# thobotics/geometry_rl

Hardware: NVIDIA B200
Metric: fwd+bwd+TRPL update samples/sec (policy fwd+bwd, TRPL projection, losses, critic, Adam) (higher is better)
Workload: dtype bf16

## Files before the change

### geometry_rl_b200/_lib.py

```python
import ctypes as C
import os

import torch

_HERE = os.path.dirname(os.path.abspath(__file__))
LIB_PATH = os.path.join(_HERE, "libgrl_b200.so")

GRL_OK = 0
BASIS_GRAD_FLOATS = 64 * 16 + 64 + 64 * 64 + 64
NODE_GRAD_FLOATS = 256 * 64 + 256 + 64 * 256 + 64 + 64 + 64 + 64 + 16 * 16 * 64
EDGE_GRAD_FLOATS = 64 * 64
FUSED_EDGE_GRAD_FLOATS = 64 * 64 + 64 * 16 + 64 * 64 + 64

_fp = C.c_void_p
_i32 = C.c_int32


class GrlEmbedDesc(C.Structure):
    _fields_ = [("n_nodes", _i32), ("n_scalars", _i32), ("n_vectors", _i32), ("dim", _i32),
                ("scalars", _fp), ("vectors", _fp), ("ori", _fp), ("weight", _fp), ("x", _fp),
                ("grad_x", _fp), ("grad_weight_partials", _fp), ("n_partials", _i32), ("node_ids", _fp)]


class GrlBasisDesc(C.Structure):
    _fields_ = [("n_edges", _i32), ("dim", _i32), ("edge_src", _fp), ("edge_dst", _fp), ("pos_src", _fp),
                ("pos_dst", _fp), ("ori", _fp), ("w1t", _fp), ("b1", _fp), ("w2t", _fp), ("b2", _fp), ("basis", _fp),
                ("w2", _fp), ("grad_basis", _fp), ("grad_partials", _fp), ("n_partials", _i32),
                ("basis_bf16", _fp), ("grad_basis_bf16", _fp)]


class GrlConvDesc(C.Structure):
    _fields_ = [("n_src", _i32), ("n_dst", _i32), ("n_edges", _i32),
                ("rowptr_dst", _fp), ("edge_src", _fp), ("edge_dst", _fp), ("rowptr_src", _fp), ("src_eid", _fp),
                ("x_src", _fp), ("x_dst", _fp), ("basis", _fp), ("fiber_kernel", _fp), ("wk_t", _fp), ("wk", _fp),
                ("bias", _fp), ("ln_g", _fp), ("ln_b", _fp), ("w1_t", _fp), ("w1", _fp), ("b1", _fp), ("w2_t", _fp),
                ("w2_c", _fp), ("b2", _fp), ("x1", _fp), ("out", _fp), ("accumulate_out", _i32),
                ("grad_out", _fp), ("grad_x1", _fp), ("grad_x_src", _fp), ("grad_x_src_init", _fp),
                ("grad_basis", _fp), ("accumulate_grad_basis", _i32), ("node_grad_partials", _fp),
                ("n_partials_node", _i32), ("edge_grad_partials", _fp), ("n_partials_edge", _i32), ("w2", _fp),
                ("basis_bf16", _fp), ("grad_basis_bf16", _fp), ("grad_x2", _fp), ("x2", _fp), ("grad_amax", _fp),
                ("basis_row", _fp), ("grad_basis_acc_mask", _fp)]


class GrlFusedEdgeDesc(C.Structure):
    _fields_ = [("n_key", _i32), ("n_edges", _i32), ("dim", _i32), ("n_partials", _i32),
                ("rowptr", _fp), ("e_src", _fp), ("e_dst", _fp), ("pos_src", _fp), ("pos_dst", _fp), ("ori", _fp),
                ("w1", _fp), ("b1", _fp), ("w2", _fp), ("b2", _fp), ("wk", _fp), ("x_src", _fp), ("x1", _fp),
                ("grad_x1", _fp), ("grad_x_src", _fp), ("grad_x_src_init", _fp), ("grad_partials", _fp), ("n_other", _i32)]


class GrlEncoderDesc(C.Structure):
    _fields_ = [("n_graphs", _i32), ("n_tokens", _i32), ("n_partials", _i32), ("x", _fp), ("in_proj_weight", _fp),
                ("in_proj_bias", _fp), ("out_proj_weight", _fp), ("out_proj_bias", _fp), ("linear1_weight", _fp),
                ("linear1_bias", _fp), ("linear2_weight", _fp), ("linear2_bias", _fp), ("norm1_weight", _fp),
                ("norm1_bias", _fp), ("norm2_weight", _fp), ("norm2_bias", _fp), ("out", _fp), ("grad_out", _fp),
                ("grad_x", _fp), ("grad_partials", _fp)]


ENCODER_MAX_TOKENS = 56
ENCODER_GRAD_FLOATS = 192 * 64 + 192 + 3 * (64 * 64 + 64) + 4 * 64


class GrlCriticDesc(C.Structure):
    _fields_ = [("n_graphs", _i32), ("n_tokens", _i32), ("n_feat", _i32), ("n_partials", _i32), ("eps", C.c_float),
                ("count", C.c_double), ("x", _fp), ("w1", _fp), ("b1", _fp), ("gamma", _fp), ("beta", _fp), ("stats", _fp),
                ("stat_partials", _fp), ("ysum", _fp), ("grad_ysum", _fp), ("bstats", _fp), ("grad_partials", _fp)]


CRITIC_GRAD_FLOATS = 3 * 64 + 64 * 16


class GrlProjDesc(C.Structure):
    _fields_ = [("batch", _i32), ("k", _i32), ("proj_type", _i32), ("eps_mean", C.c_float), ("eps_cov", C.c_float),
                ("mean", _fp), ("v", _fp), ("old_mean", _fp), ("old_v", _fp), ("proj_mean", _fp), ("proj_v", _fp),
                ("eta", _fp), ("grad_proj_mean", _fp), ("grad_proj_v", _fp), ("grad_mean", _fp), ("grad_v", _fp),
                ("grad_mean_add", _fp), ("grad_v_add", _fp)]


class GrlLossDesc(C.Structure):
    _fields_ = [("batch", _i32), ("k", _i32), ("proj_type", _i32), ("normalize_advantage", _i32),
                ("entropy_coef", C.c_float), ("trust_region_coeff", C.c_float),
                ("mean", _fp), ("v", _fp), ("proj_mean", _fp), ("proj_v", _fp), ("action", _fp), ("prev_log_prob", _fp),
                ("advantage", _fp), ("terms", _fp), ("stats", _fp), ("scalars", _fp), ("grad_losses", _fp),
                ("grad_proj_mean", _fp), ("grad_proj_v", _fp), ("grad_mean_direct", _fp), ("grad_v_direct", _fp),
                ("sums", _fp), ("stage", _i32)]


class GrlReadoutDesc(C.Structure):
    _fields_ = [("n_nodes", _i32), ("od", _i32), ("odv", _i32), ("dim", _i32), ("latent", _fp), ("weight", _fp),
                ("bias", _fp), ("ori", _fp), ("out", _fp), ("hidden", _fp), ("grad_out", _fp), ("grad_hidden", _fp),
                ("grad_latent", _fp), ("grad_partials", _fp), ("n_partials", _i32)]


class GrlActDesc(C.Structure):
    _fields_ = [("batch", _i32), ("num_rows", _i32), ("action_dim", _i32), ("hidden_dim", _i32), ("post_fc", _i32),
                ("contextual_std", _i32), ("use_tanh_mean", _i32), ("deterministic", _i32), ("rank", _i32),
                ("pre_shift", C.c_float), ("minimal_std", C.c_float), ("hidden", _fp), ("mean", _fp),
                ("mean_weight", _fp), ("mean_bias", _fp), ("std_weight", _fp), ("std_bias", _fp), ("state", _fp),
                ("loc", _fp), ("cov", _fp), ("action", _fp), ("log_prob", _fp), ("eps", _fp)]


ACT_MAX_K = 32
READOUT_MAX_OUT = 8
MAX_KNN = 8
LOSS_TERMS = 8
LOSS_SCALARS = 16
LOSS_STATS = 8
LOSS_SUMS = 16
LOSS_SCALAR_INDEX = {"loss_objective": 0, "loss_trust_region": 1, "loss_entropy": 2, "dist_entropy": 3, "ESS": 4, "kl": 5,
                     "constraint": 6, "mean_constraint": 7, "mean_constraint_max": 8, "cov_constraint": 9,
                     "cov_constraint_max": 10, "entropy": 11, "entropy_diff": 12}


SIGNATURES = {
    "grl_abi_version": (C.c_int, []),
    "grl_last_error": (C.c_char_p, []),
    "grl_sm_count": (C.c_int, []),
    "grl_reserve_sms": (C.c_int, [C.c_int]),
    "grl_knn_edge_ptr": (C.c_int, [_fp, C.c_int, C.c_int, C.c_int, _fp, _fp]),
    "grl_knn_graph": (C.c_int, [_fp, _fp, _fp, C.c_int, C.c_int, C.c_int, _fp, C.c_int64, _fp]),
    "grl_radius_neighbors": (C.c_int, [_fp, _fp, C.c_int, C.c_int, C.c_float, C.c_int, _fp, _fp, _fp]),
    "grl_radius_edge_ptr": (C.c_int, [_fp, C.c_int, C.c_int, C.c_int64, _fp, _fp]),
    "grl_radius_graph": (C.c_int, [_fp, _fp, _fp, C.c_int, C.c_int, C.c_int, _fp, C.c_int64, C.c_int64, _fp]),
    "grl_dense_edges": (C.c_int, [C.c_int, _fp, _fp, C.c_int, C.c_int, C.c_int, _fp, C.c_int64, _fp]),
    "grl_csr_build": (C.c_int, [_fp, C.c_int64, _fp, C.c_int, C.c_int, C.c_int, _fp, _fp, _fp, _fp]),
    "grl_embed_fwd": (C.c_int, [C.POINTER(GrlEmbedDesc), _fp]),
    "grl_embed_bwd": (C.c_int, [C.POINTER(GrlEmbedDesc), _fp]),
    "grl_edge_basis_fwd": (C.c_int, [C.POINTER(GrlBasisDesc), _fp]),
    "grl_edge_basis_bwd": (C.c_int, [C.POINTER(GrlBasisDesc), _fp]),
    "grl_fbconv_edge_fwd": (C.c_int, [C.POINTER(GrlConvDesc), _fp]),
    "grl_fbconv_node_fwd": (C.c_int, [C.POINTER(GrlConvDesc), _fp]),
    "grl_fbconv_node_bwd": (C.c_int, [C.POINTER(GrlConvDesc), _fp]),
    "grl_fbconv_edge_bwd": (C.c_int, [C.POINTER(GrlConvDesc), _fp]),
    "grl_fbconv_node_fwd_tc": (C.c_int, [C.POINTER(GrlConvDesc), _fp]),
    "grl_edge_basis_fwd_tc": (C.c_int, [C.POINTER(GrlBasisDesc), _fp]),
    "grl_fbconv_edge_fwd_tc": (C.c_int, [C.POINTER(GrlConvDesc), _fp]),
    "grl_fbconv_edge_bwd_tc": (C.c_int, [C.POINTER(GrlConvDesc), _fp]),
    "grl_edge_basis_bwd_tc": (C.c_int, [C.POINTER(GrlBasisDesc), _fp]),
    "grl_fbconv_node_bwd_tc": (C.c_int, [C.POINTER(GrlConvDesc), _fp]),
    "grl_fbconv_edge_fused_fwd": (C.c_int, [C.POINTER(GrlFusedEdgeDesc), _fp]),
    "grl_fbconv_edge_fused_bwd": (C.c_int, [C.POINTER(GrlFusedEdgeDesc), _fp]),
    "grl_critic_inner_stats": (C.c_int, [C.POINTER(GrlCriticDesc), _fp]),
    "grl_critic_inner_fwd": (C.c_int, [C.POINTER(GrlCriticDesc), _fp]),
    "grl_critic_inner_bwd_stats": (C.c_int, [C.POINTER(GrlCriticDesc), _fp]),
    "grl_critic_inner_bwd": (C.c_int, [C.POINTER(GrlCriticDesc), _fp]),
    "grl_encoder_layer_fwd": (C.c_int, [C.POINTER(GrlEncoderDesc), _fp]),
    "grl_encoder_layer_bwd": (C.c_int, [C.POINTER(GrlEncoderDesc), _fp]),
    "grl_readout_fwd": (C.c_int, [C.POINTER(GrlReadoutDesc), _fp]),
    "grl_readout_bwd": (C.c_int, [C.POINTER(GrlReadoutDesc), _fp]),
    "grl_trpl_loss_fwd": (C.c_int, [C.POINTER(GrlLossDesc), _fp]),
    "grl_trpl_loss_bwd": (C.c_int, [C.POINTER(GrlLossDesc), _fp]),
    "grl_dp_combine": (C.c_int, [_fp, C.c_int, C.c_int, C.c_int, _fp, _fp]),
    "grl_absmax": (C.c_int, [_fp, C.c_int64, _fp, _fp]),
    "grl_reduce_partials": (C.c_int, [_fp, C.c_int, C.c_int64, _fp, C.c_int, _fp]),
    "grl_gae_scan": (C.c_int, [_fp, _fp, _fp, _fp, C.c_float, C.c_float, C.c_int, C.c_int, _fp, _fp, _fp]),
    "grl_gaussian_act": (C.c_int, [C.POINTER(GrlActDesc), _fp]),
    "grl_act_advance": (C.c_int, [_fp, _fp]),
    "grl_trpl_fwd": (C.c_int, [C.POINTER(GrlProjDesc), _fp]),
    "grl_trpl_bwd": (C.c_int, [C.POINTER(GrlProjDesc), _fp]),
    "grl_tc_selftest_gemm": (C.c_int, [_fp, _fp, _fp, C.c_int, C.c_int, _fp]),
    "grl_tc_selftest_gemm_ts": (C.c_int, [_fp, _fp, _fp, C.c_int, _fp]),
    "grl_tc_debug_mma": (C.c_int, [_fp, C.c_int, _fp, C.c_int, _fp, C.c_int, C.c_int] + [C.c_uint32] * 8 + [_fp]),
    "grl_tc_latency_probe": (C.c_int, [_fp, _fp]),
}

_lib = None
launch_count = 0


def load():
    global _lib
    if _lib is None:
        if not os.path.exists(LIB_PATH):
            raise RuntimeError(
                f"{LIB_PATH} not found: build it with `python -c 'import __graft_entry__ as g; g.build()'` "
                "(geometry_rl_b200 has no CPU or eager fallback)")
        lib = C.CDLL(LIB_PATH)
        for name, (res, args) in SIGNATURES.items():
            fn = getattr(lib, name)
            fn.restype = res
            fn.argtypes = args
        _lib = lib
    return _lib


def last_error() -> str:
    return load().grl_last_error().decode()


def check(rc: int, what: str):
    if rc != GRL_OK:
        raise RuntimeError(f"{what} failed with code {rc}: {last_error()}")


def stream_ptr() -> int:
    return torch.cuda.current_stream().cuda_stream


def ptr(t):
    if t is None:
        return None
    if not t.is_cuda:
        raise RuntimeError("geometry_rl_b200 kernels need CUDA tensors (no CPU path exists)")
    if not t.is_contiguous():
        raise RuntimeError("geometry_rl_b200 kernels need contiguous tensors")
    return t.data_ptr()


def ptr_any(t):
    if t is None:
        return None
    if not t.is_cuda:
        raise RuntimeError("geometry_rl_b200 kernels need CUDA tensors (no CPU path exists)")
    return t.data_ptr()


_timing = None


def event_timing(enable: bool):
    global _timing
    if enable:
        _timing = {}
        return None
    rec, _timing = _timing, None
    torch.cuda.synchronize()
    return {k: [(a.elapsed_time(b),) + tuple(shape) for a, b, shape in v] for k, v in (rec or {}).items()}


def call(name: str, *args, shape=(0, 0, 0)):
    global launch_count
    lib = load()
    if _timing is not None:
        a, b = torch.cuda.Event(enable_timing=True), torch.cuda.Event(enable_timing=True)
        a.record()
        rc = getattr(lib, name)(*args, stream_ptr())
        b.record()
        _timing.setdefault(name, []).append((a, b, shape))
    else:
        rc = getattr(lib, name)(*args, stream_ptr())
    launch_count += 1
    check(rc, name)


_sm = None


def sm_count() -> int:
    global _sm
    if _sm is None:
        _sm = load().grl_sm_count()
    return _sm


def reserve_sms(n: int) -> None:
    global _sm
    check(load().grl_reserve_sms(int(n)), "grl_reserve_sms")
    _sm = None
```

### geometry_rl_b200/csrc/grl_common.cuh

```cuda
#pragma once
#include <cuda_runtime.h>
#include <stdint.h>

#include "../../include/grl_b200.h"

namespace grl {

constexpr int kO = GRL_NUM_ORI;
constexpr int kC = GRL_CHANNELS;
constexpr int kH = GRL_HIDDEN;
constexpr int kTE = 8;
constexpr int kTM = kTE * kO;
constexpr int kLDT = 68;
constexpr int kThreads = 256;
constexpr int kRow = kO * kC;
constexpr int kTileFloats = kTM * kLDT;
constexpr int kWFloats = kC * kC;

void set_error(const char* fmt, ...);
int check_launch(const char* what);
int sm_count();
int ensure_dynamic_smem(const void* func, int bytes);
int make_row_tensor_map(void* out_tensor_map_128B, const float* base, long long n_nodes, int box_rows = 16);

#define GRL_REQUIRE(cond, code, ...)  \
  do {                                \
    if (!(cond)) {                    \
      ::grl::set_error(__VA_ARGS__);  \
      return (code);                  \
    }                                 \
  } while (0)

__device__ __forceinline__ float gelu_f(float x) { return 0.5f * x * (1.0f + erff(x * 0.70710678118654752440f)); }
__device__ __forceinline__ float gelu_grad_f(float x) {
  const float cdf = 0.5f * (1.0f + erff(x * 0.70710678118654752440f));
  const float pdf = 0.39894228040143267794f * expf(-0.5f * x * x);
  return cdf + x * pdf;
}

__device__ __forceinline__ float tanh_approx(float x) {
  float y;
  asm("tanh.approx.f32 %0, %1;" : "=f"(y) : "f"(x));
  return y;
}
__device__ __forceinline__ void gelu_fast(float x, float& y, float& dy) {
#ifdef GRL_TC_EXACT_GELU
  const float u = __expf(-0.5f * x * x);
  const float t = __fdividef(1.0f, fmaf(0.23164189f, fabsf(x), 1.0f));
  float poly = fmaf(t, 1.061405429f, -1.453152027f);
  poly = fmaf(t, poly, 1.421413741f);
  poly = fmaf(t, poly, -0.284496736f);
  poly = fmaf(t, poly, 0.254829592f);
  const float tail = 0.5f * (poly * t) * u;
  const float cdf = x >= 0.f ? 1.0f - tail : tail;
  y = x * cdf;
  dy = fmaf(x * u, 0.39894228040143267794f, cdf);
#else
  constexpr float k = 0.7978845608028654f, kc = 0.7978845608028654f * 0.044715f;
  const float t2 = x * x;
  const float th = tanh_approx(x * fmaf(t2, kc, k));
  const float hx = 0.5f * x;
  y = fmaf(hx, th, hx);
  dy = fmaf(hx * fmaf(-th, th, 1.0f), fmaf(t2, 3.0f * kc, k), fmaf(th, 0.5f, 0.5f));
#endif
}
__device__ __forceinline__ float gelu_fast(float x) {
#ifdef GRL_TC_EXACT_GELU
  float y, dy;
  gelu_fast(x, y, dy);
  return y;
#else
  constexpr float k = 0.7978845608028654f, kc = 0.7978845608028654f * 0.044715f;
  const float hx = 0.5f * x;
  return fmaf(hx, tanh_approx(x * fmaf(x * x, kc, k)), hx);
#endif
}

__device__ __forceinline__ void cp_async16(float* smem_dst, const float* gmem_src) {
  const unsigned s = static_cast<unsigned>(__cvta_generic_to_shared(smem_dst));
  asm volatile("cp.async.cg.shared.global [%0], [%1], 16;\n" ::"r"(s), "l"(gmem_src) : "memory");
}
__device__ __forceinline__ void cp_async_commit() { asm volatile("cp.async.commit_group;\n" ::: "memory"); }
__device__ __forceinline__ void cp_async_wait_all() { asm volatile("cp.async.wait_group 0;\n" ::: "memory"); }
template <int N>
__device__ __forceinline__ void cp_async_wait() {
  asm volatile("cp.async.wait_group %0;\n" ::"n"(N) : "memory");
}

__device__ __forceinline__ void stage_w64(float* __restrict__ dst, const float* __restrict__ src) {
#pragma unroll
  for (int i = 0; i < 4; ++i) {
    const int f = threadIdx.x + kThreads * i;
    cp_async16(dst + 4 * f, src + 4 * f);
  }
}

__device__ __forceinline__ void stage_rows_contig(float* __restrict__ tile, const float* __restrict__ src, int cnt) {
#pragma unroll
  for (int i = 0; i < 8; ++i) {
    const int f = threadIdx.x + kThreads * i;
    const int row = f >> 4, c4 = f & 15;
    float* d = tile + row * kLDT + 4 * c4;
    if ((row >> 4) < cnt) {
      cp_async16(d, src + (size_t)row * kC + 4 * c4);
    } else {
      *reinterpret_cast<float4*>(d) = make_float4(0.f, 0.f, 0.f, 0.f);
    }
  }
}

__device__ __forceinline__ void stage_rows_gather(float* __restrict__ tile, const float* __restrict__ base,
                                                  const int* __restrict__ idx, int cnt) {
#pragma unroll
  for (int i = 0; i < 8; ++i) {
    const int f = threadIdx.x + kThreads * i;
    const int row = f >> 4, c4 = f & 15;
    const int j = row >> 4;
    float* d = tile + row * kLDT + 4 * c4;
    if (j < cnt) {
      cp_async16(d, base + (size_t)idx[j] * kRow + (row & 15) * kC + 4 * c4);
    } else {
      *reinterpret_cast<float4*>(d) = make_float4(0.f, 0.f, 0.f, 0.f);
    }
  }
}

template <int K>
__device__ __forceinline__ void gemm_tile(const float* __restrict__ As, int lda, const float* __restrict__ Bs, int o,
                                          int cg, float (&acc)[kTE][4]) {
  const float* a0 = As + o * lda;
  const float* b0 = Bs + 4 * cg;
#pragma unroll 2
  for (int k = 0; k < K; k += 4) {
    const float4 b_0 = *reinterpret_cast<const float4*>(b0 + (k + 0) * kC);
    const float4 b_1 = *reinterpret_cast<const float4*>(b0 + (k + 1) * kC);
    const float4 b_2 = *reinterpret_cast<const float4*>(b0 + (k + 2) * kC);
    const float4 b_3 = *reinterpret_cast<const float4*>(b0 + (k + 3) * kC);
#pragma unroll
    for (int j = 0; j < kTE; ++j) {
      const float4 a = *reinterpret_cast<const float4*>(a0 + j * 16 * lda + k);
      acc[j][0] = fmaf(a.x, b_0.x, acc[j][0]);
      acc[j][1] = fmaf(a.x, b_0.y, acc[j][1]);
      acc[j][2] = fmaf(a.x, b_0.z, acc[j][2]);
      acc[j][3] = fmaf(a.x, b_0.w, acc[j][3]);
      acc[j][0] = fmaf(a.y, b_1.x, acc[j][0]);
      acc[j][1] = fmaf(a.y, b_1.y, acc[j][1]);
      acc[j][2] = fmaf(a.y, b_1.z, acc[j][2]);
      acc[j][3] = fmaf(a.y, b_1.w, acc[j][3]);
      acc[j][0] = fmaf(a.z, b_2.x, acc[j][0]);
      acc[j][1] = fmaf(a.z, b_2.y, acc[j][1]);
      acc[j][2] = fmaf(a.z, b_2.z, acc[j][2]);
      acc[j][3] = fmaf(a.z, b_2.w, acc[j][3]);
      acc[j][0] = fmaf(a.w, b_3.x, acc[j][0]);
      acc[j][1] = fmaf(a.w, b_3.y, acc[j][1]);
      acc[j][2] = fmaf(a.w, b_3.z, acc[j][2]);
      acc[j][3] = fmaf(a.w, b_3.w, acc[j][3]);
    }
  }
}

__device__ __forceinline__ void zero_acc(float (&acc)[kTE][4]) {
#pragma unroll
  for (int j = 0; j < kTE; ++j) acc[j][0] = acc[j][1] = acc[j][2] = acc[j][3] = 0.f;
}

template <bool kColSum>
__device__ __forceinline__ void wgrad_tile(const float* __restrict__ As, int lda, const float* __restrict__ Bs, int ldb,
                                           int ni, int mi, float (&g)[4][4], float (&colsum)[4]) {
  const float* a0 = As + 4 * ni;
  const float* b0 = Bs + 4 * mi;
#pragma unroll 4
  for (int r = 0; r < kTM; ++r) {
    const float4 a = *reinterpret_cast<const float4*>(a0 + r * lda);
    const float4 b = *reinterpret_cast<const float4*>(b0 + r * ldb);
    g[0][0] = fmaf(a.x, b.x, g[0][0]); g[0][1] = fmaf(a.x, b.y, g[0][1]);
    g[0][2] = fmaf(a.x, b.z, g[0][2]); g[0][3] = fmaf(a.x, b.w, g[0][3]);
    g[1][0] = fmaf(a.y, b.x, g[1][0]); g[1][1] = fmaf(a.y, b.y, g[1][1]);
    g[1][2] = fmaf(a.y, b.z, g[1][2]); g[1][3] = fmaf(a.y, b.w, g[1][3]);
    g[2][0] = fmaf(a.z, b.x, g[2][0]); g[2][1] = fmaf(a.z, b.y, g[2][1]);
    g[2][2] = fmaf(a.z, b.z, g[2][2]); g[2][3] = fmaf(a.z, b.w, g[2][3]);
    g[3][0] = fmaf(a.w, b.x, g[3][0]); g[3][1] = fmaf(a.w, b.y, g[3][1]);
    g[3][2] = fmaf(a.w, b.z, g[3][2]); g[3][3] = fmaf(a.w, b.w, g[3][3]);
    if (kColSum && mi == 0) {
      colsum[0] += a.x; colsum[1] += a.y; colsum[2] += a.z; colsum[3] += a.w;
// ... 32 lines not shown
```

### geometry_rl_b200/csrc/grl_conv_node_bwd_tc.cu

```cuda
#include "grl_common.cuh"
#include "grl_tc.cuh"

namespace grl {

constexpr int kPGW1 = 0;
constexpr int kPGB1 = kPGW1 + kH * kC;
constexpr int kPGW2 = kPGB1 + kH;
constexpr int kPGB2 = kPGW2 + kC * kH;
constexpr int kPGLNG = kPGB2 + kC;
constexpr int kPGLNB = kPGLNG + kC;
constexpr int kPGBIAS = kPGLNB + kC;
constexpr int kPGFK = kPGBIAS + kC;
static_assert(kPGFK + kO * kO * kC == GRL_NODE_GRAD_FLOATS, "partial layout");

constexpr int kKb = 80;
constexpr int kLDX2 = 68;

__device__ __forceinline__ void warp_colsum16(float (&v)[16], int lane) {
#pragma unroll
  for (int step = 0; step < 4; ++step) {
    const int half = 8 >> step;
    const int bit = 16 >> step;
    const bool upper = (lane & bit) != 0;
#pragma unroll
    for (int i = 0; i < half; ++i) {
      const float keep = upper ? v[i + half] : v[i];
      const float send = upper ? v[i] : v[i + half];
      v[i] = keep + __shfl_xor_sync(0xffffffffu, send, bit);
    }
  }
  v[0] += __shfl_xor_sync(0xffffffffu, v[0], 1);
}

constexpr int kNB3Epi = 512;
constexpr int kNB3Threads = kNB3Epi + 32;
constexpr uint32_t kCol3D0 = 0, kCol3D1 = 64, kCol3GY = 128, kCol3DW1 = 192, kCol3DW2 = 352;

struct NodeBwd3Smem {
  __half W1h[kH * kKb];
  __half W2h[kC * kH];
  __half A1[kTM * kKb];
  __half GZh[kTM * kC];
  union {
    struct {
      float X2[kTM * kLDX2];
      float GZf[kTM * kLDX2];
    } in;
    struct {
      __half A2h[kTM * 128];
      __half AP[kTM * 128];
    } h;
  } u;
  float bias[kC], lng[kC], lnb[kC];
  float rs[2][4][kTM];
  float acc_gb2[4][kC], acc_glng[4][kC], acc_glnb[4][kC];
  uint64_t full[2], edone[2], lnready, gyfull, dwdone;
  uint32_t tmem_base;
};

__global__ void __launch_bounds__(kNB3Threads, 1) fbconv_node_bwd_tc3_kernel(const GrlConvDesc d) {
  extern __shared__ __align__(128) unsigned char smem_raw[];
  NodeBwd3Smem& s = *reinterpret_cast<NodeBwd3Smem*>(smem_raw);
  const int tid = threadIdx.x, warp = tid >> 5, lane = tid & 31;
  const bool is_epi = warp < 16;
  const int q = warp & 3, cg = (warp >> 2) & 3;
  const int row = 32 * q + lane;

  if (tid == 0) {
    tc::mbar_init(&s.full[0], 1);
    tc::mbar_init(&s.full[1], 1);
    tc::mbar_init(&s.edone[0], 16);
    tc::mbar_init(&s.edone[1], 16);
    tc::mbar_init(&s.lnready, 16);
    tc::mbar_init(&s.gyfull, 1);
    tc::mbar_init(&s.dwdone, 1);
    tc::fence_mbar_init();
  }
  if (warp == 16) tc::tmem_alloc(&s.tmem_base, 512);
  tc::stage_weight_f16(s.W1h, d.w1, kH, kC, kC);
  tc::stage_weight_f16(s.W2h, d.w2, kC, kH, kH);
  for (int n = tid; n < kH; n += kNB3Threads) {
    const float b = d.b1[n];
    const __half hi = __float2half_rn(b);
    const __half lo = __float2half_rn(b - __half2float(hi));
    const __half2 p0 = __halves2half2(hi, lo);
    *reinterpret_cast<uint4*>(s.W1h + ((size_t)8 * kH + n) * 8) = make_uint4(*reinterpret_cast<const uint32_t*>(&p0), 0u, 0u, 0u);
    *reinterpret_cast<uint4*>(s.W1h + ((size_t)9 * kH + n) * 8) = make_uint4(0u, 0u, 0u, 0u);
  }
  if (tid < kTM) {
    *reinterpret_cast<uint4*>(s.A1 + ((size_t)8 * kTM + tid) * 8) = make_uint4(0x3C003C00u, 0u, 0u, 0u);
    *reinterpret_cast<uint4*>(s.A1 + ((size_t)9 * kTM + tid) * 8) = make_uint4(0u, 0u, 0u, 0u);
  }
  if (tid < kC) { s.bias[tid] = d.bias[tid]; s.lng[tid] = d.ln_g[tid]; s.lnb[tid] = d.ln_b[tid]; }
  for (int i = tid; i < 4 * kC; i += kNB3Threads) {
    (&s.acc_gb2[0][0])[i] = 0.f; (&s.acc_glng[0][0])[i] = 0.f; (&s.acc_glnb[0][0])[i] = 0.f;
  }
  const float gscale = d.grad_amax ? tc::grad_scale_from_amax(__ldg(d.grad_amax)) : 1.0f;
  const float inv_gscale = 1.0f / gscale;
  const int n_tiles = (d.n_dst + kTE - 1) / kTE;
  int tile = blockIdx.x;
  auto stage_x2 = [&](int t) {
    const int cnt = min(kTE, d.n_dst - t * kTE);
    const float* src = d.x2 + (size_t)t * kTE * kRow;
    const float* gsrc = d.grad_out + (size_t)t * kTE * kRow;
#pragma unroll
    for (int i = 0; i < 4; ++i) {
      const int f = tid + kNB3Epi * i;
      const int so = (f >> 4) * kLDX2 + 4 * (f & 15);
      if ((f >> 8) < cnt) {
        cp_async16(s.u.in.X2 + so, src + 4 * f);
        cp_async16(s.u.in.GZf + so, gsrc + 4 * f);
      } else {
        *reinterpret_cast<float4*>(s.u.in.X2 + so) = make_float4(0.f, 0.f, 0.f, 0.f);
        *reinterpret_cast<float4*>(s.u.in.GZf + so) = make_float4(0.f, 0.f, 0.f, 0.f);
      }
    }
  };
  if (is_epi && tile < n_tiles) {
    stage_x2(tile);
    cp_async_commit();
  }
  tc::fence_async_smem();
  tc::tc_fence_before();
  __syncthreads();
  tc::tc_fence_after();
  const uint32_t tmem = s.tmem_base;
  const uint32_t lane_addr = tmem + ((uint32_t)(32 * q) << 16);
  const uint32_t a1 = tc::smem_u32(s.A1), gz = tc::smem_u32(s.GZh), a2 = tc::smem_u32(s.u.h.A2h), ap = tc::smem_u32(s.u.h.AP);
  const uint32_t w1 = tc::smem_u32(s.W1h), w2 = tc::smem_u32(s.W2h);
  bool first_tile = true;

  if (!is_epi) {
    uint32_t p_ln = 0, p_e0 = 0, p_e1 = 0;
    constexpr uint32_t id_pre = tc::idesc_f16_ex(128, 64, 0, 0, 0, 0);
    constexpr uint32_t id_gh = tc::idesc_f16_ex(128, 64, 0, 1, 0, 0);
    constexpr uint32_t id_dw2 = tc::idesc_f16_ex(128, 64, 1, 1, 0, 0);
    constexpr uint32_t id_dw1 = tc::idesc_f16_ex(128, kKb, 1, 1, 0, 0);
    const tc::Op a1_k = tc::op_k(a1, kTM), a1_mn = tc::op_mn(a1, kTM);
    const tc::Op gz_k = tc::op_k(gz, kTM), gz_mn = tc::op_mn(gz, kTM);
    const tc::Op a2_mn = tc::op_mn(a2, kTM), ap_k = tc::op_k(ap, kTM), ap_mn = tc::op_mn(ap, kTM);
    const tc::Op w1_k = tc::op_k(w1, kH), w1_mn = tc::op_mn(w1, kH), w2_mn = tc::op_mn(w2, kC);
    auto shifted = [](tc::Op o, uint32_t bytes) { o.lo += bytes >> 4; return o; };
    auto pre = [&](int qq, uint32_t col) { tc::issue_mma_fast<kKb / 16>(tmem + col, a1_k, shifted(w1_k, 64u * qq * 16u), id_pre, false); };
    auto gh = [&](int qq, uint32_t col) { tc::issue_mma_fast<kC / 16>(tmem + col, gz_k, shifted(w2_mn, 8u * qq * (kC * 16u)), id_gh, false); };
    for (; tile < n_tiles; tile += gridDim.x) {
      tc::mbar_wait(&s.lnready, p_ln);
      p_ln ^= 1u;
      tc::tc_fence_after();
      if (tc::elect_one()) {
        pre(0, kCol3D0);
        tc::mma_commit(&s.full[0]);
        pre(1, kCol3D1);
        tc::mma_commit(&s.full[1]);
      }
      __syncwarp();
#pragma unroll
      for (int hh = 0; hh < 2; ++hh) {
        tc::mbar_wait(&s.edone[0], p_e0);
        p_e0 ^= 1u;
        tc::tc_fence_after();
        if (tc::elect_one()) {
          gh(2 * hh, kCol3D0);
          tc::mma_commit(&s.full[0]);
        }
        __syncwarp();
        tc::mbar_wait(&s.edone[1], p_e1);
        p_e1 ^= 1u;
        tc::tc_fence_after();
        if (tc::elect_one()) {
          gh(2 * hh + 1, kCol3D1);
          tc::mma_commit(&s.full[1]);
          tc::issue_mma_fast<kTM / 16>(tmem + kCol3DW2 + 64 * hh, a2_mn, gz_mn, id_dw2, !first_tile);
        }
        __syncwarp();
        tc::mbar_wait(&s.edone[0], p_e0);
        p_e0 ^= 1u;
        tc::tc_fence_after();
        if (hh == 0) {
          if (tc::elect_one()) {
            pre(2, kCol3D0);
            tc::mma_commit(&s.full[0]);
          }
          __syncwarp();
        }
        tc::mbar_wait(&s.edone[1], p_e1);
        p_e1 ^= 1u;
        tc::tc_fence_after();
        if (tc::elect_one()) {
          if (hh == 0) {
            pre(3, kCol3D1);
            tc::mma_commit(&s.full[1]);
          }
          tc::issue_mma_fast<128 / 16>(tmem + kCol3GY, ap_k, shifted(w1_mn, 128u * hh * 16u), id_gh, hh > 0);
          if (hh == 1) tc::mma_commit(&s.gyfull);
          tc::issue_mma_fast<kTM / 16>(tmem + kCol3DW1 + kKb * hh, ap_mn, a1_mn, id_dw1, !first_tile);
          if (hh == 1) tc::mma_commit(&s.dwdone);
        }
        __syncwarp();
      }
      first_tile = false;
    }
  } else {
    uint32_t pf0 = 0, pf1 = 0, pgy = 0;
    for (; tile < n_tiles; tile += gridDim.x) {
      const int n0 = tile * kTE;
      const int node = n0 + (row >> 4);
      const bool live = node < d.n_dst;
      const size_t roff = (size_t)(live ? node : 0) * kRow + (row & 15) * kC + 16 * cg;
      if (tid == 0) {
        const int nt = tile + gridDim.x;
        if (nt < n_tiles) {
          const uint32_t bytes = (uint32_t)min(kTE, d.n_dst - nt * kTE) * kRow * 4u;
          tc::prefetch_l2(d.x2 + (size_t)nt * kTE * kRow, bytes);
          tc::prefetch_l2(d.grad_out + (size_t)nt * kTE * kRow, bytes);
        }
      }
      cp_async_wait_all();
      tc::group_sync(5, kNB3Epi);

      float xh[16];
      float rstd;
      {
        float sum = 0.f;
#pragma unroll
        for (int i = 0; i < 4; ++i) {
          const float4 v = ld4(s.u.in.X2 + row * kLDX2 + 16 * cg + 4 * i);
          xh[4 * i] = v.x; xh[4 * i + 1] = v.y; xh[4 * i + 2] = v.z; xh[4 * i + 3] = v.w;
          sum += (v.x + v.y) + (v.z + v.w);
        }
        float g16[16];
#pragma unroll
        for (int i = 0; i < 4; ++i) {
          const float4 gv = ld4(s.u.in.GZf + row * kLDX2 + 16 * cg + 4 * i);
          g16[4 * i] = gv.x; g16[4 * i + 1] = gv.y; g16[4 * i + 2] = gv.z; g16[4 * i + 3] = gv.w;
        }
        s.rs[0][cg][row] = sum;
        tc::group_sync(1 + q, 128);
        const float mean = ((s.rs[0][0][row] + s.rs[0][1][row]) + (s.rs[0][2][row] + s.rs[0][3][row])) * (1.0f / 64.0f);
        float sq = 0.f;
#pragma unroll
        for (int i = 0; i < 16; ++i) { xh[i] -= mean; sq = fmaf(xh[i], xh[i], sq); }
        s.rs[1][cg][row] = sq;
        {
          float gs[16];
#pragma unroll
          for (int i = 0; i < 16; ++i) gs[i] = g16[i] * gscale;
          *reinterpret_cast<uint4*>(s.GZh + ((size_t)(2 * cg) * kTM + row) * 8) = tc::pack8_h(gs);
          *reinterpret_cast<uint4*>(s.GZh + ((size_t)(2 * cg + 1) * kTM + row) * 8) = tc::pack8_h(gs + 8);
        }
        warp_colsum16(g16, lane);
        if ((lane & 1) == 0) s.acc_gb2[q][16 * cg + (lane >> 1)] += g16[0];
        tc::group_sync(1 + q, 128);
        rstd = rsqrtf(((s.rs[1][0][row] + s.rs[1][1][row]) + (s.rs[1][2][row] + s.rs[1][3][row])) * (1.0f / 64.0f) + 1e-5f);
#pragma unroll
        for (int i = 0; i < 2; ++i) {
          float y[8];
#pragma unroll
          for (int e = 0; e < 8; ++e) {
            const int c = 16 * cg + 8 * i + e;
            xh[8 * i + e] *= rstd;
            y[e] = xh[8 * i + e] * s.lng[c] + s.lnb[c];
          }
          *reinterpret_cast<uint4*>(s.A1 + ((size_t)(2 * cg + i) * kTM + row) * 8) = tc::pack8_h(y);
        }
      }
      tc::fence_async_smem();
      tc::tc_fence_before();
      __syncwarp();
      if (lane == 0) tc::mbar_arrive(&s.lnready);

      __half2 dG0[8], dG1[8];
      auto e1 = [&](uint32_t col, uint64_t* fullb, uint32_t& pf, uint64_t* doneb, __half2 (&dG)[8], int chunk) {
        tc::mbar_wait(fullb, pf);
        pf ^= 1u;
        tc::tc_fence_after();
        float v[16];
        tc::tmem_ld16(lane_addr + col + 16 * cg, v);
        __half2 h0[4], h1[4];
#pragma unroll
        for (int e = 0; e < 4; ++e) {
          tc::gelu_h2(__floats2half2_rn(v[2 * e], v[2 * e + 1]), h0[e], dG[e]);
          tc::gelu_h2(__floats2half2_rn(v[8 + 2 * e], v[8 + 2 * e + 1]), h1[e], dG[4 + e]);
        }
        *reinterpret_cast<uint4*>(s.u.h.A2h + ((size_t)chunk * kTM + row) * 8) = tc::pack_h8(h0);
        *reinterpret_cast<uint4*>(s.u.h.A2h + ((size_t)(chunk + 1) * kTM + row) * 8) = tc::pack_h8(h1);
        tc::fence_async_smem();
        tc::tc_fence_before();
        __syncwarp();
        if (lane == 0) tc::mbar_arrive(doneb);
      };
      auto e2 = [&](uint32_t col, uint64_t* fullb, uint32_t& pf, uint64_t* doneb, const __half2 (&dG)[8], int chunk) {
        tc::mbar_wait(fullb, pf);
        pf ^= 1u;
        tc::tc_fence_after();
        float v[16];
        tc::tmem_ld16(lane_addr + col + 16 * cg, v);
        __half2 p0[4], p1[4];
#pragma unroll
        for (int e = 0; e < 4; ++e) {
          p0[e] = __hmul2(__floats2half2_rn(v[2 * e], v[2 * e + 1]), dG[e]);
          p1[e] = __hmul2(__floats2half2_rn(v[8 + 2 * e], v[8 + 2 * e + 1]), dG[4 + e]);
        }
        *reinterpret_cast<uint4*>(s.u.h.AP + ((size_t)chunk * kTM + row) * 8) = tc::pack_h8(p0);
        *reinterpret_cast<uint4*>(s.u.h.AP + ((size_t)(chunk + 1) * kTM + row) * 8) = tc::pack_h8(p1);
        tc::fence_async_smem();
        tc::tc_fence_before();
        __syncwarp();
        if (lane == 0) tc::mbar_arrive(doneb);
      };
#pragma unroll 1
      for (int hh = 0; hh < 2; ++hh) {
        e1(kCol3D0, &s.full[0], pf0, &s.edone[0], dG0, 2 * cg);
        e1(kCol3D1, &s.full[1], pf1, &s.edone[1], dG1, 8 + 2 * cg);
        e2(kCol3D0, &s.full[0], pf0, &s.edone[0], dG0, 2 * cg);
        e2(kCol3D1, &s.full[1], pf1, &s.edone[1], dG1, 8 + 2 * cg);
      }
      tc::mbar_wait(&s.gyfull, pgy);
      tc::tc_fence_after();

      {
        float gy[32];
        {
          float v[16];
          tc::tmem_ld16(lane_addr + kCol3GY + 16 * cg, v);
#pragma unroll
          for (int e = 0; e < 16; ++e) gy[e] = v[e] * inv_gscale;
        }
        tc::mbar_wait(&s.dwdone, pgy);
        pgy ^= 1u;
        {
          const int nt = tile + gridDim.x;
          if (nt < n_tiles) {
            stage_x2(nt);
            cp_async_commit();
          }
        }
        float s1 = 0.f, s2 = 0.f;
#pragma unroll
        for (int i = 0; i < 16; ++i) {
          const float hx = gy[i] * s.lng[16 * cg + i];
          s1 += hx;
          s2 = fmaf(hx, xh[i], s2);
        }
        s.rs[0][cg][row] = s1;
        s.rs[1][cg][row] = s2;
        tc::group_sync(1 + q, 128);
        const float m1 = ((s.rs[0][0][row] + s.rs[0][1][row]) + (s.rs[0][2][row] + s.rs[0][3][row])) * (1.0f / 64.0f);
        const float m2 = ((s.rs[1][0][row] + s.rs[1][1][row]) + (s.rs[1][2][row] + s.rs[1][3][row])) * (1.0f / 64.0f);
        float* gdst = d.grad_x2 + roff;
#pragma unroll
        for (int i = 0; i < 4; ++i) {
          float o[4];
#pragma unroll
          for (int e = 0; e < 4; ++e) {
            const int c = 4 * i + e;
            const float hx = gy[c] * s.lng[16 * cg + c];
            o[e] = rstd * (hx - m1 - xh[c] * m2);
          }
          if (live) st4(gdst + 4 * i, make_float4(o[0], o[1], o[2], o[3]));
        }
#pragma unroll
        for (int i = 0; i < 16; ++i) gy[16 + i] = gy[i] * xh[i];
        tc::warp_colsum<32>(gy, lane);
        if (lane < 16) s.acc_glnb[q][16 * cg + lane] += gy[0];
        else s.acc_glng[q][16 * cg + lane - 16] += gy[0];
      }
      tc::tc_fence_before();
      first_tile = false;
    }
    cp_async_wait_all();
  }

  __syncthreads();
  tc::tc_fence_after();
  float* P = d.node_grad_partials + (size_t)blockIdx.x * GRL_NODE_GRAD_FLOATS;
  if (is_epi) {
#pragma unroll 1
    for (int h2 = 0; h2 < 2; ++h2) {
      const int c0 = 16 * cg;
      float v[16];
#pragma unroll
      for (int e = 0; e < 16; ++e) v[e] = 0.f;
      if (!first_tile) tc::tmem_ld16(lane_addr + kCol3DW1 + kKb * h2 + c0, v);
      float* p1 = P + kPGW1 + (size_t)(128 * h2 + row) * kC + c0;
#pragma unroll
      for (int e = 0; e < 16; e += 4)
        st4(p1 + e, make_float4(v[e] * inv_gscale, v[e + 1] * inv_gscale, v[e + 2] * inv_gscale, v[e + 3] * inv_gscale));
      if (cg == 0) {
        float b[16];
#pragma unroll
        for (int e = 0; e < 16; ++e) b[e] = 0.f;
        if (!first_tile) tc::tmem_ld16(lane_addr + kCol3DW1 + kKb * h2 + 64, b);
        P[kPGB1 + 128 * h2 + row] = b[0] * inv_gscale;
      }
      if (!first_tile) tc::tmem_ld16(lane_addr + kCol3DW2 + 64 * h2 + c0, v);
#pragma unroll
      for (int e = 0; e < 16; ++e) P[kPGW2 + (size_t)(c0 + e) * kH + 128 * h2 + row] = v[e] * inv_gscale;
    }
  }
  if (tid < kC) {
    P[kPGB2 + tid] = ((s.acc_gb2[0][tid] + s.acc_gb2[1][tid]) + s.acc_gb2[2][tid]) + s.acc_gb2[3][tid];
    P[kPGLNG + tid] = ((s.acc_glng[0][tid] + s.acc_glng[1][tid]) + s.acc_glng[2][tid]) + s.acc_glng[3][tid];
    P[kPGLNB + tid] = ((s.acc_glnb[0][tid] + s.acc_glnb[1][tid]) + s.acc_glnb[2][tid]) + s.acc_glnb[3][tid];
  }
  tc::tc_fence_before();
  __syncthreads();
  if (warp == 16) tc::tmem_dealloc(tmem, 512);
}

constexpr int kFiberThreads = 512;
constexpr int kFibTile = 4;
struct FiberBwdSmem {
  float G[2][kFibTile * kRow];
  float X[2][kFibTile * kRow];
};

__device__ __forceinline__ void fiber_stage(FiberBwdSmem& s, int buf, const GrlConvDesc& d, int tile) {
  const int n0 = tile * kFibTile;
#pragma unroll
  for (int i = 0; i < 4; ++i) {
    const int f = threadIdx.x + kFiberThreads * i;
    const int arr = f >> 10, idx = f & 1023, node = n0 + (idx >> 8);
    float* dst = (arr ? s.X[buf] : s.G[buf]) + 4 * idx;
    if (node < d.n_dst) cp_async16(dst, (arr ? d.x1 : d.grad_x2) + (size_t)n0 * kRow + 4 * idx);
    else *reinterpret_cast<float4*>(dst) = make_float4(0.f, 0.f, 0.f, 0.f);
  }
}

__global__ void __launch_bounds__(kFiberThreads, 1) fbconv_fiber_bwd_kernel(const GrlConvDesc d) {
  extern __shared__ __align__(128) unsigned char smem_raw[];
  FiberBwdSmem& s = *reinterpret_cast<FiberBwdSmem*>(smem_raw);
  const int tid = threadIdx.x, c = tid & 63, op = tid >> 6;
  unsigned long long fk2[kO], gfk2[kO];
#pragma unroll
  for (int p = 0; p < kO; ++p) {
    fk2[p] = pack2(__ldg(d.fiber_kernel + ((size_t)((2 * op) * kO + p)) * kC + c) * 0.0625f,
                   __ldg(d.fiber_kernel + ((size_t)((2 * op + 1) * kO + p)) * kC + c) * 0.0625f);
    gfk2[p] = pack2(0.f, 0.f);
  }
  float gbias = 0.f;
  const int n_tiles = (d.n_dst + kFibTile - 1) / kFibTile;
  int tile = blockIdx.x, buf = 0;
  if (tile < n_tiles) fiber_stage(s, 0, d, tile);
  cp_async_commit();
  for (; tile < n_tiles; tile += gridDim.x, buf ^= 1) {
    const int nt = tile + gridDim.x;
    if (nt < n_tiles) fiber_stage(s, buf ^ 1, d, nt);
    cp_async_commit();
    cp_async_wait<1>();
    __syncthreads();
#pragma unroll
    for (int j = 0; j < kFibTile; ++j) {
      const int node = tile * kFibTile + j;
      const float* G = s.G[buf] + j * kRow + c;
      const float* X = s.X[buf] + j * kRow + c;
      const unsigned long long xv = pack2(X[(2 * op) * kC], X[(2 * op + 1) * kC]);
      unsigned long long a2 = pack2(0.f, 0.f);
      float gsum = 0.f;
#pragma unroll
      for (int p = 0; p < kO; ++p) {
        const float g = G[p * kC];
        const unsigned long long gg = pack2(g, g);
        a2 = ffma2(gg, fk2[p], a2);
        gfk2[p] = ffma2(xv, gg, gfk2[p]);
        gsum += g;
      }
      if (node < d.n_dst) {
        float a0, a1;
        unpack2(a2, a0, a1);
        d.grad_x1[(size_t)node * kRow + (2 * op) * kC + c] = a0;
        d.grad_x1[(size_t)node * kRow + (2 * op + 1) * kC + c] = a1;
      }
      if (op == 0) gbias += gsum;
    }
    __syncthreads();
  }
  float* P = d.node_grad_partials + (size_t)blockIdx.x * GRL_NODE_GRAD_FLOATS;
#pragma unroll
  for (int p = 0; p < kO; ++p) {
    float g0, g1;
    unpack2(gfk2[p], g0, g1);
    P[kPGFK + ((size_t)((2 * op) * kO + p)) * kC + c] = g0 * 0.0625f;
    P[kPGFK + ((size_t)((2 * op + 1) * kO + p)) * kC + c] = g1 * 0.0625f;
  }
  if (op == 0) P[kPGBIAS + c] = gbias;
}

}

extern "C" int grl_fbconv_node_bwd_tc(const GrlConvDesc* d, grl_stream_t stream) {
  GRL_REQUIRE(d && d->n_dst > 0, GRL_EINVAL, "grl_fbconv_node_bwd_tc: bad descriptor");
  GRL_REQUIRE(d->x1 && d->fiber_kernel && d->bias && d->ln_g && d->ln_b && d->w1 && d->b1 && d->w2 && d->grad_out &&
                  d->grad_x1 && d->grad_x2 && d->node_grad_partials && d->n_partials_node > 0, GRL_EINVAL,
              "grl_fbconv_node_bwd_tc: null pointer");
  {
    GRL_REQUIRE(d->x2, GRL_EINVAL, "grl_fbconv_node_bwd_tc: x2 (saved by grl_fbconv_node_fwd_tc) is required");
    const int smem = (int)sizeof(grl::NodeBwd3Smem);
    if (grl::ensure_dynamic_smem((const void*)grl::fbconv_node_bwd_tc3_kernel, smem) != GRL_OK) return GRL_ECUDA;
    grl::fbconv_node_bwd_tc3_kernel<<<d->n_partials_node, grl::kNB3Threads, smem, (cudaStream_t)stream>>>(*d);
  }
  int rc = grl::check_launch("grl_fbconv_node_bwd_tc (mlp)");
  if (rc != GRL_OK) return rc;
  const int smem2 = (int)sizeof(grl::FiberBwdSmem);
  if (grl::ensure_dynamic_smem((const void*)grl::fbconv_fiber_bwd_kernel, smem2) != GRL_OK) return GRL_ECUDA;
  grl::fbconv_fiber_bwd_kernel<<<d->n_partials_node, grl::kFiberThreads, smem2, (cudaStream_t)stream>>>(*d);
  return grl::check_launch("grl_fbconv_node_bwd_tc (fibre)");
}
```

### geometry_rl_b200/csrc/grl_conv_node_tc.cu

```cuda
#include <cuda.h>

#include "grl_common.cuh"
#include "grl_tc.cuh"

namespace grl {

constexpr int kLDX = 72;

constexpr int kNF2Threads = 512;
constexpr int kK1 = 80;

struct NodeFwd2Group {
  union {
    struct {
      float X1[kTM * kC];
      float X2[kTM * kLDX];
    } x;
    __half A1[kTM * kK1];
  } u;
};

struct NodeFwd2Smem {
  __half W1h[kH * kK1];
  __half W2h[kC * kH];
  NodeFwd2Group g[2];
  float b2[kC], bias[kC], lng[kC], lnb[kC];
  uint64_t bar[2][2];
  uint64_t bar_x[2];
  uint64_t bar_d[2];
  uint32_t tmem_base;
};

__device__ __forceinline__ void stage_x1_dense(float* __restrict__ X1, const float* __restrict__ src, int cnt, int gt,
                                               uint64_t* bar) {
  if (gt == 0) {
    tc::mbar_expect_tx(bar, (uint32_t)cnt * kRow * 4u);
    tc::bulk_g2s(X1, src, (uint32_t)cnt * kRow * 4u, bar);
  }
  if (cnt < kTE) {
#pragma unroll
    for (int i = 0; i < 8; ++i) {
      const int f = gt + 256 * i;
      if ((f >> 8) >= cnt) *reinterpret_cast<float4*>(X1 + 4 * f) = make_float4(0.f, 0.f, 0.f, 0.f);
    }
  }
}

template <bool kAcc>
__global__ void __launch_bounds__(kNF2Threads, 1) fbconv_node_fwd_tc2_kernel(const GrlConvDesc d, const __grid_constant__ CUtensorMap tm_xd) {
  extern __shared__ unsigned char smem_raw[];
  NodeFwd2Smem& s = *reinterpret_cast<NodeFwd2Smem*>(
      smem_raw + ((1024u - (tc::smem_u32(smem_raw) & 1023u)) & 1023u));
  const int tid = threadIdx.x;
  const int grp = tid >> 8, gt = tid & 255, gw = gt >> 5, lane = tid & 31;
  NodeFwd2Group& G = s.g[grp];
  const int bar_id = 1 + grp;

  if (tid == 0) {
    tc::mbar_init(&s.bar[0][0], 1);
    tc::mbar_init(&s.bar[0][1], 1);
    tc::mbar_init(&s.bar[1][0], 1);
    tc::mbar_init(&s.bar[1][1], 1);
    tc::mbar_init(&s.bar_x[0], 1);
    tc::mbar_init(&s.bar_x[1], 1);
    tc::mbar_init(&s.bar_d[0], 1);
    tc::mbar_init(&s.bar_d[1], 1);
    tc::fence_mbar_init();
  }
  if (tid < 32) tc::tmem_alloc(&s.tmem_base, 512);
  tc::stage_weight_f16(s.W1h, d.w1, kH, kC, kC);
  tc::stage_weight_f16(s.W2h, d.w2, kC, kH, kH);
  for (int n = tid; n < kH; n += kNF2Threads) {
    const float b = d.b1[n];
    const __half hi = __float2half_rn(b);
    const __half lo = __float2half_rn(b - __half2float(hi));
    const __half z = __float2half_rn(0.f);
    const __half2 h[4] = {__halves2half2(hi, lo), __halves2half2(z, z), __halves2half2(z, z), __halves2half2(z, z)};
    *reinterpret_cast<uint4*>(s.W1h + ((size_t)8 * kH + n) * 8) = tc::pack_h8(h);
    *reinterpret_cast<uint4*>(s.W1h + ((size_t)9 * kH + n) * 8) = make_uint4(0u, 0u, 0u, 0u);
  }
  if (tid < kC) { s.b2[tid] = d.b2[tid]; s.bias[tid] = d.bias[tid]; s.lng[tid] = d.ln_g[tid]; s.lnb[tid] = d.ln_b[tid]; }
  const int fc = gt & 63, pq = gt >> 6;
  unsigned long long fk2[kO][2];
#pragma unroll
  for (int o = 0; o < kO; ++o)
#pragma unroll
    for (int pi = 0; pi < 2; ++pi)
      fk2[o][pi] = pack2(__ldg(d.fiber_kernel + ((size_t)(o * kO + 4 * pq + 2 * pi)) * kC + fc) * 0.0625f,
                         __ldg(d.fiber_kernel + ((size_t)(o * kO + 4 * pq + 2 * pi + 1)) * kC + fc) * 0.0625f);

  const int n_tiles = (d.n_dst + kTE - 1) / kTE;
  const int tile_stride = 2 * gridDim.x;
  int tile = 2 * blockIdx.x + grp;
  tc::fence_async_smem();
  tc::tc_fence_before();
  __syncthreads();
  tc::tc_fence_after();
  if (tile < n_tiles)
    stage_x1_dense(G.u.x.X1, d.x1 + (size_t)tile * kTE * kRow, min(kTE, d.n_dst - tile * kTE), gt, &s.bar_x[grp]);
  const uint32_t tmem = s.tmem_base + 256u * grp;
  const uint32_t a1_addr = tc::smem_u32(G.u.A1);
  const uint32_t w1_addr = tc::smem_u32(s.W1h), w2_addr = tc::smem_u32(s.W2h);
  const int q = gw & 3, hh = gw >> 2;
  const int row = 32 * q + lane;
  const uint32_t lane_addr = tmem + ((uint32_t)(32 * q) << 16);
  uint32_t parity = 0;

  for (; tile < n_tiles; tile += tile_stride) {
    const int n0 = tile * kTE;
    if (gt == 0) {
      tc::prefetch_l2(d.x_dst + (size_t)n0 * kRow, (uint32_t)min(kTE, d.n_dst - n0) * kRow * 4u);
      const int nt = tile + tile_stride;
      if (nt < n_tiles) tc::prefetch_l2(d.x1 + (size_t)nt * kTE * kRow, (uint32_t)min(kTE, d.n_dst - nt * kTE) * kRow * 4u);
    }
    tc::mbar_wait(&s.bar_x[grp], parity);
    tc::group_sync(bar_id, 256);

    {
      const float bias_c = s.bias[fc];
#pragma unroll 2
      for (int j = 0; j < kTE; ++j) {
        unsigned long long a01 = pack2(0.f, 0.f), a23 = a01;
#pragma unroll
        for (int o = 0; o < kO; ++o) {
          const float x = G.u.x.X1[(16 * j + o) * kC + fc];
          const unsigned long long xx = pack2(x, x);
          a01 = ffma2(xx, fk2[o][0], a01);
          a23 = ffma2(xx, fk2[o][1], a23);
        }
        float a0, a1, a2, a3;
        unpack2(a01, a0, a1);
        unpack2(a23, a2, a3);
        float* o2 = G.u.x.X2 + (16 * j + 4 * pq) * kLDX + fc;
        o2[0 * kLDX] = a0 + bias_c;
        o2[1 * kLDX] = a1 + bias_c;
        o2[2 * kLDX] = a2 + bias_c;
        o2[3 * kLDX] = a3 + bias_c;
      }
    }
    tc::group_sync(bar_id, 256);

    {
      const int r = gt >> 1, h = gt & 1;
      float4 v[8];
      float sum = 0.f;
#pragma unroll
      for (int i = 0; i < 8; ++i) {
        v[i] = ld4(G.u.x.X2 + r * kLDX + 4 * (2 * i + h));
        sum += (v[i].x + v[i].y) + (v[i].z + v[i].w);
      }
      if (d.x2 && n0 + (r >> 4) < d.n_dst) {
        float* xo = d.x2 + (size_t)(n0 + (r >> 4)) * kRow + (r & 15) * kC + 4 * h;
#pragma unroll
        for (int i = 0; i < 8; ++i) st4(xo + 8 * i, v[i]);
      }
      sum += __shfl_xor_sync(0xffffffffu, sum, 1);
      const float mean = sum * (1.0f / 64.0f);
      float sq = 0.f;
#pragma unroll
      for (int i = 0; i < 8; ++i) {
        v[i].x -= mean; v[i].y -= mean; v[i].z -= mean; v[i].w -= mean;
        sq += (v[i].x * v[i].x + v[i].y * v[i].y) + (v[i].z * v[i].z + v[i].w * v[i].w);
      }
      sq += __shfl_xor_sync(0xffffffffu, sq, 1);
      const float rstd = rsqrtf(sq * (1.0f / 64.0f) + 1e-5f);
#pragma unroll
      for (int i = 0; i < 8; ++i) {
        const int c = 4 * (2 * i + h);
        const float4 g = ld4(s.lng + c), b = ld4(s.lnb + c);
        const __half2 p0 = __floats2half2_rn(v[i].x * rstd * g.x + b.x, v[i].y * rstd * g.y + b.y);
        const __half2 p1 = __floats2half2_rn(v[i].z * rstd * g.z + b.z, v[i].w * rstd * g.w + b.w);
        uint2 pk;
        pk.x = *reinterpret_cast<const uint32_t*>(&p0);
        pk.y = *reinterpret_cast<const uint32_t*>(&p1);
        *reinterpret_cast<uint2*>(G.u.A1 + ((size_t)i * kTM + r) * 8 + 4 * h) = pk;
      }
      *reinterpret_cast<uint4*>(G.u.A1 + ((size_t)(8 + h) * kTM + r) * 8) = make_uint4(h == 0 ? 0x3C003C00u : 0u, 0u, 0u, 0u);
    }
    tc::fence_async_smem();
    tc::tc_fence_before();
    tc::group_sync(bar_id, 256);
    if (gt == 0) {
      tc::tc_fence_after();
      tc::issue_mma_rolled(tmem, tc::view_k(a1_addr, kTM), tc::view_k(w1_addr, kH), tc::idesc_f16_ex(128, kH, 0, 0, 0, 0), kK1 / 16, false);
      tc::mma_commit(&s.bar[grp][0]);
      tc::mbar_expect_tx(&s.bar_d[grp], 2u * kTM * 32u * 4u);
      tc::tma_load_2d(G.u.x.X2, &tm_xd, 0, n0 * kO, &s.bar_d[grp]);
      tc::tma_load_2d(G.u.x.X2 + kTM * 32, &tm_xd, 32, n0 * kO, &s.bar_d[grp]);
    }
    tc::mbar_wait(&s.bar[grp][0], parity);
    tc::tc_fence_after();
    {
      const int nt = tile + tile_stride;
      if (nt < n_tiles) {
        tc::fence_async_smem();
        stage_x1_dense(G.u.x.X1, d.x1 + (size_t)nt * kTE * kRow, min(kTE, d.n_dst - nt * kTE), gt, &s.bar_x[grp]);
      }
    }
    {
#pragma unroll 2
      for (int i = 0; i < 8; ++i) {
        const int c0 = 128 * hh + 16 * i;
        float v[16];
        tc::tmem_ld16(lane_addr + c0, v);
        uint32_t r[8];
#pragma unroll
        for (int e = 0; e < 4; ++e) {
          const __half2 a = tc::gelu_h2(__floats2half2_rn(v[2 * e], v[2 * e + 1]));
          const __half2 b = tc::gelu_h2(__floats2half2_rn(v[8 + 2 * e], v[8 + 2 * e + 1]));
          r[e] = *reinterpret_cast<const uint32_t*>(&a);
          r[4 + e] = *reinterpret_cast<const uint32_t*>(&b);
        }
        tc::tmem_st8(lane_addr + 128 * hh + 8 * i, r);
      }
      tc::tmem_st_wait();
    }
    tc::tc_fence_before();
    tc::group_sync(bar_id, 256);
    if (gt == 0) {
      tc::tc_fence_after();
      const tc::OpView w2v = tc::view_k(w2_addr, kC);
      tc::OpView w2hi = w2v;
      w2hi.addr += 8 * w2v.adv;
      tc::issue_mma_ts(tmem + 64, tmem, w2v, tc::idesc_f16_ex(128, kC, 0, 0, 0, 0), 8, false);
      tc::issue_mma_ts(tmem + 64, tmem + 128, w2hi, tc::idesc_f16_ex(128, kC, 0, 0, 0, 0), 8, true);
      tc::mma_commit(&s.bar[grp][1]);
    }
    const int node = n0 + (row >> 4);
    const bool live = node < d.n_dst;
    const size_t off = (size_t)(live ? node : 0) * kRow + (row & 15) * kC + 32 * hh;
    tc::mbar_wait(&s.bar[grp][1], parity);
    tc::tc_fence_after();
    tc::mbar_wait(&s.bar_d[grp], parity);
    const float* xrow = G.u.x.X2 + hh * (kTM * 32) + row * 32;
#pragma unroll
    for (int i = 0; i < 2; ++i) {
      float v[16];
      tc::tmem_ld16(lane_addr + 64 + 32 * hh + 16 * i, v);
      if (live) {
#pragma unroll
        for (int e = 0; e < 4; ++e) {
          const float4 bb = ld4(s.b2 + 32 * hh + 16 * i + 4 * e);
          float4 x = ld4(xrow + (((4 * i + e) ^ (row & 7)) << 2));
          if (kAcc) {
            const float4 old = ldg4(d.out + off + 16 * i + 4 * e);
            x.x += old.x; x.y += old.y; x.z += old.z; x.w += old.w;
          }
          st4(d.out + off + 16 * i + 4 * e, make_float4(x.x + (v[4 * e] + bb.x), x.y + (v[4 * e + 1] + bb.y),
                                                       x.z + (v[4 * e + 2] + bb.z), x.w + (v[4 * e + 3] + bb.w)));
        }
      }
    }
    tc::tc_fence_before();
    parity ^= 1u;
  }
  cp_async_wait_all();
  tc::tc_fence_before();
  __syncthreads();
  if (tid < 32) tc::tmem_dealloc(s.tmem_base, 512);
}

}

extern "C" int grl_fbconv_node_fwd_tc(const GrlConvDesc* d, grl_stream_t stream) {
  GRL_REQUIRE(d && d->n_dst > 0, GRL_EINVAL, "grl_fbconv_node_fwd_tc: bad descriptor");
  GRL_REQUIRE(d->x1 && d->fiber_kernel && d->bias && d->ln_g && d->ln_b && d->w1 && d->b1 && d->w2 && d->b2 && d->x_dst &&
                  d->out, GRL_EINVAL, "grl_fbconv_node_fwd_tc: null pointer");
  const int n_tiles = (d->n_dst + grl::kTE - 1) / grl::kTE;
  const int smem2 = (int)sizeof(grl::NodeFwd2Smem) + 1024;
  if (grl::ensure_dynamic_smem((const void*)grl::fbconv_node_fwd_tc2_kernel<false>, smem2) != GRL_OK) return GRL_ECUDA;
  if (grl::ensure_dynamic_smem((const void*)grl::fbconv_node_fwd_tc2_kernel<true>, smem2) != GRL_OK) return GRL_ECUDA;
  alignas(64) CUtensorMap tm_xd;
  if (grl::make_row_tensor_map(&tm_xd, d->x_dst, d->n_dst, grl::kTM) != GRL_OK) return GRL_ECUDA;
  int grid = grl::sm_count();
  if (2 * grid > n_tiles) grid = (n_tiles + 1) / 2;
  if (d->accumulate_out) grl::fbconv_node_fwd_tc2_kernel<true><<<grid, grl::kNF2Threads, smem2, (cudaStream_t)stream>>>(*d, tm_xd);
  else grl::fbconv_node_fwd_tc2_kernel<false><<<grid, grl::kNF2Threads, smem2, (cudaStream_t)stream>>>(*d, tm_xd);
  return grl::check_launch("grl_fbconv_node_fwd_tc");
}
```

### geometry_rl_b200/csrc/grl_critic.cu

```cuda
#include "grl_common.cuh"

namespace grl {

constexpr int kCrThreads = 256;
constexpr int kCrMaxTokens = 256;

struct CriticSmem {
  float x[kCrMaxTokens * 16];
  float w1[16 * kC];
  float red[16 * kC];
  double dred[kCrThreads / 32 * 4];
};

__device__ __forceinline__ void critic_stage_w1(float* __restrict__ w1s, const GrlCriticDesc& d) {
  for (int i = threadIdx.x; i < 16 * kC; i += kCrThreads) {
    const int f = i >> 6, c = i & 63;
    w1s[i] = f < d.n_feat ? __ldg(d.w1 + c * d.n_feat + f) : 0.f;
  }
}

__device__ __forceinline__ void critic_stage_x(float* __restrict__ xs, const GrlCriticDesc& d, int b, int t0, int cnt) {
  const float* src = d.x + ((size_t)b * d.n_tokens + t0) * d.n_feat;
  for (int i = threadIdx.x; i < cnt * 16; i += kCrThreads) {
    const int t = i >> 4, f = i & 15;
    xs[i] = f < d.n_feat ? __ldg(src + t * d.n_feat + f) : 0.f;
  }
}

__device__ __forceinline__ float4 critic_h(const float* __restrict__ xrow, const float* __restrict__ w1s, int cg, float4 b1) {
  float4 h = b1;
#pragma unroll
  for (int f = 0; f < 16; ++f) {
    const float xv = xrow[f];
    const float4 w = *reinterpret_cast<const float4*>(w1s + f * kC + 4 * cg);
    h.x = fmaf(xv, w.x, h.x); h.y = fmaf(xv, w.y, h.y); h.z = fmaf(xv, w.z, h.z); h.w = fmaf(xv, w.w, h.w);
  }
  return h;
}

template <int NV>
__device__ __forceinline__ void block_sum_d(double (&v)[NV], double* __restrict__ scratch) {
#pragma unroll
  for (int i = 0; i < NV; ++i) {
#pragma unroll
    for (int o = 16; o > 0; o >>= 1) v[i] += __shfl_xor_sync(0xffffffffu, v[i], o);
  }
  const int warp = threadIdx.x >> 5, lane = threadIdx.x & 31;
  __syncthreads();
  if (lane == 0) {
#pragma unroll
    for (int i = 0; i < NV; ++i) scratch[warp * 4 + i] = v[i];
  }
  __syncthreads();
  if (threadIdx.x == 0) {
#pragma unroll
    for (int i = 0; i < NV; ++i) {
      double s = 0.0;
      for (int w = 0; w < kCrThreads / 32; ++w) s += scratch[w * 4 + i];
      v[i] = s;
    }
  }
}

__device__ __forceinline__ void critic_range(const GrlCriticDesc& d, int& g_lo, int& g_hi) {
  g_lo = (int)((long long)d.n_graphs * blockIdx.x / gridDim.x);
  g_hi = (int)((long long)d.n_graphs * (blockIdx.x + 1) / gridDim.x);
}

__global__ void __launch_bounds__(kCrThreads) critic_stats_kernel(const GrlCriticDesc d) {
  extern __shared__ __align__(16) unsigned char smem_raw[];
  CriticSmem& s = *reinterpret_cast<CriticSmem*>(smem_raw);
  const int p = threadIdx.x >> 4, cg = threadIdx.x & 15;
  critic_stage_w1(s.w1, d);
  const float4 b1 = __ldg(reinterpret_cast<const float4*>(d.b1) + cg);
  int g_lo, g_hi;
  critic_range(d, g_lo, g_hi);
  double acc[2] = {0.0, 0.0};
  for (int b = g_lo; b < g_hi; ++b) {
    for (int t0 = 0; t0 < d.n_tokens; t0 += kCrMaxTokens) {
      const int cnt = min(kCrMaxTokens, d.n_tokens - t0);
      __syncthreads();
      critic_stage_x(s.x, d, b, t0, cnt);
      __syncthreads();
      float sm = 0.f, sq = 0.f;
      for (int t = p; t < cnt; t += 16) {
        const float4 h = critic_h(s.x + t * 16, s.w1, cg, b1);
        sm += (h.x + h.y) + (h.z + h.w);
        sq += (h.x * h.x + h.y * h.y) + (h.z * h.z + h.w * h.w);
      }
      acc[0] += (double)sm;
      acc[1] += (double)sq;
    }
  }
  block_sum_d<2>(acc, s.dred);
  if (threadIdx.x == 0) {
    d.stat_partials[2 * blockIdx.x] = acc[0];
    d.stat_partials[2 * blockIdx.x + 1] = acc[1];
  }
}

__global__ void critic_combine_kernel(const double* __restrict__ partials, int n_slots, int n, double* __restrict__ out) {
  const int i = threadIdx.x;
  if (i >= n) return;
  double s = 0.0;
  for (int k = 0; k < n_slots; ++k) s += partials[(size_t)k * n + i];
  out[i] = s;
}

struct CriticNorm {
  float mean, inv, r;
};
__device__ __forceinline__ CriticNorm critic_norm(const GrlCriticDesc& d) {
  const double n = d.count;
  const double mean = d.stats[0] / n;
  double var = d.stats[1] / n - mean * mean;
  var = var > 0.0 ? var : 0.0;
  const double sd = sqrt(var);
  CriticNorm c;
  c.mean = (float)mean;
  c.inv = (float)(1.0 / (sd + (double)d.eps));
  c.r = (float)(sd / (sd + (double)d.eps));
  return c;
}

__global__ void __launch_bounds__(kCrThreads) critic_fwd_kernel(const GrlCriticDesc d) {
  extern __shared__ __align__(16) unsigned char smem_raw[];
  CriticSmem& s = *reinterpret_cast<CriticSmem*>(smem_raw);
  const int p = threadIdx.x >> 4, cg = threadIdx.x & 15;
  critic_stage_w1(s.w1, d);
  const float4 b1 = __ldg(reinterpret_cast<const float4*>(d.b1) + cg);
  const float4 ga = __ldg(reinterpret_cast<const float4*>(d.gamma) + cg);
  const float4 be = __ldg(reinterpret_cast<const float4*>(d.beta) + cg);
  const CriticNorm nm = critic_norm(d);
  int g_lo, g_hi;
  critic_range(d, g_lo, g_hi);
  for (int b = g_lo; b < g_hi; ++b) {
    float4 ys = make_float4(0.f, 0.f, 0.f, 0.f);
    for (int t0 = 0; t0 < d.n_tokens; t0 += kCrMaxTokens) {
      const int cnt = min(kCrMaxTokens, d.n_tokens - t0);
      __syncthreads();
      critic_stage_x(s.x, d, b, t0, cnt);
      __syncthreads();
      for (int t = p; t < cnt; t += 16) {
        const float4 h = critic_h(s.x + t * 16, s.w1, cg, b1);
        ys.x += fmaxf(fmaf((h.x - nm.mean) * nm.inv, ga.x, be.x), 0.f);
        ys.y += fmaxf(fmaf((h.y - nm.mean) * nm.inv, ga.y, be.y), 0.f);
        ys.z += fmaxf(fmaf((h.z - nm.mean) * nm.inv, ga.z, be.z), 0.f);
        ys.w += fmaxf(fmaf((h.w - nm.mean) * nm.inv, ga.w, be.w), 0.f);
      }
    }
    __syncthreads();
    *reinterpret_cast<float4*>(s.red + p * kC + 4 * cg) = ys;
    __syncthreads();
    if (threadIdx.x < kC) {
      float a = 0.f;
#pragma unroll
      for (int k = 0; k < 16; ++k) a += s.red[k * kC + threadIdx.x];
      d.ysum[(size_t)b * kC + threadIdx.x] = a;
    }
  }
}

__global__ void __launch_bounds__(kCrThreads) critic_bwd_stats_kernel(const GrlCriticDesc d) {
  extern __shared__ __align__(16) unsigned char smem_raw[];
  CriticSmem& s = *reinterpret_cast<CriticSmem*>(smem_raw);
  const int p = threadIdx.x >> 4, cg = threadIdx.x & 15;
  critic_stage_w1(s.w1, d);
  const float4 b1 = __ldg(reinterpret_cast<const float4*>(d.b1) + cg);
  const float4 ga = __ldg(reinterpret_cast<const float4*>(d.gamma) + cg);
  const float4 be = __ldg(reinterpret_cast<const float4*>(d.beta) + cg);
  const CriticNorm nm = critic_norm(d);
  int g_lo, g_hi;
  critic_range(d, g_lo, g_hi);
  double acc[2] = {0.0, 0.0};
  float4 gg = make_float4(0.f, 0.f, 0.f, 0.f), gb = make_float4(0.f, 0.f, 0.f, 0.f);
  for (int b = g_lo; b < g_hi; ++b) {
    const float4 gy = __ldg(reinterpret_cast<const float4*>(d.grad_ysum + (size_t)b * kC) + cg);
    for (int t0 = 0; t0 < d.n_tokens; t0 += kCrMaxTokens) {
      const int cnt = min(kCrMaxTokens, d.n_tokens - t0);
      __syncthreads();
      critic_stage_x(s.x, d, b, t0, cnt);
      __syncthreads();
      float s1 = 0.f, s2 = 0.f;
      for (int t = p; t < cnt; t += 16) {
        const float4 h = critic_h(s.x + t * 16, s.w1, cg, b1);
        const float xh[4] = {(h.x - nm.mean) * nm.inv, (h.y - nm.mean) * nm.inv, (h.z - nm.mean) * nm.inv, (h.w - nm.mean) * nm.inv};
        const float g[4] = {gy.x, gy.y, gy.z, gy.w}, gam[4] = {ga.x, ga.y, ga.z, ga.w}, bet[4] = {be.x, be.y, be.z, be.w};
        float* ggp = &gg.x;
        float* gbp = &gb.x;
#pragma unroll
        for (int k = 0; k < 4; ++k) {
          const float go = fmaf(xh[k], gam[k], bet[k]) > 0.f ? g[k] : 0.f;
          ggp[k] += go * xh[k];
          gbp[k] += go;
          const float gx = go * gam[k];
          s1 += gx;
          s2 += gx * xh[k];
        }
      }
      acc[0] += (double)s1;
      acc[1] += (double)s2;
    }
  }
  block_sum_d<2>(acc, s.dred);
  if (threadIdx.x == 0) {
    d.stat_partials[2 * blockIdx.x] = acc[0];
    d.stat_partials[2 * blockIdx.x + 1] = acc[1];
  }
  float* P = d.grad_partials + (size_t)blockIdx.x * GRL_CRITIC_GRAD_FLOATS;
  __syncthreads();
  *reinterpret_cast<float4*>(s.red + p * kC + 4 * cg) = gg;
  __syncthreads();
  if (threadIdx.x < kC) {
    float a = 0.f;
#pragma unroll
    for (int k = 0; k < 16; ++k) a += s.red[k * kC + threadIdx.x];
    P[threadIdx.x] = a;
  }
  __syncthreads();
  *reinterpret_cast<float4*>(s.red + p * kC + 4 * cg) = gb;
  __syncthreads();
  if (threadIdx.x < kC) {
    float a = 0.f;
#pragma unroll
    for (int k = 0; k < 16; ++k) a += s.red[k * kC + threadIdx.x];
    P[kC + threadIdx.x] = a;
  }
}

__global__ void __launch_bounds__(kCrThreads) critic_bwd_kernel(const GrlCriticDesc d) {
  extern __shared__ __align__(16) unsigned char smem_raw[];
  CriticSmem& s = *reinterpret_cast<CriticSmem*>(smem_raw);
  const int p = threadIdx.x >> 4, cg = threadIdx.x & 15;
  critic_stage_w1(s.w1, d);
  const float4 b1 = __ldg(reinterpret_cast<const float4*>(d.b1) + cg);
  const float4 ga = __ldg(reinterpret_cast<const float4*>(d.gamma) + cg);
  const float4 be = __ldg(reinterpret_cast<const float4*>(d.beta) + cg);
  const CriticNorm nm = critic_norm(d);
  const float c1 = (float)(d.bstats[0] / d.count);
  const float c2 = (float)(d.bstats[1] / (d.count * (double)nm.r));
  int g_lo, g_hi;
  critic_range(d, g_lo, g_hi);
  float gw[4][16];
  float gb1[4] = {0.f, 0.f, 0.f, 0.f};
#pragma unroll
  for (int k = 0; k < 4; ++k)
#pragma unroll
    for (int f = 0; f < 16; ++f) gw[k][f] = 0.f;
  for (int b = g_lo; b < g_hi; ++b) {
    const float4 gy = __ldg(reinterpret_cast<const float4*>(d.grad_ysum + (size_t)b * kC) + cg);
    for (int t0 = 0; t0 < d.n_tokens; t0 += kCrMaxTokens) {
      const int cnt = min(kCrMaxTokens, d.n_tokens - t0);
      __syncthreads();
      critic_stage_x(s.x, d, b, t0, cnt);
      __syncthreads();
      for (int t = p; t < cnt; t += 16) {
        const float* xr = s.x + t * 16;
        const float4 h = critic_h(xr, s.w1, cg, b1);
        const float hv[4] = {h.x, h.y, h.z, h.w}, g[4] = {gy.x, gy.y, gy.z, gy.w};
        const float gam[4] = {ga.x, ga.y, ga.z, ga.w}, bet[4] = {be.x, be.y, be.z, be.w};
        float gh[4];
#pragma unroll
        for (int k = 0; k < 4; ++k) {
          const float xh = (hv[k] - nm.mean) * nm.inv;
          const float gx = fmaf(xh, gam[k], bet[k]) > 0.f ? g[k] * gam[k] : 0.f;
          gh[k] = nm.inv * (gx - c1 - xh * c2);
          gb1[k] += gh[k];
        }
#pragma unroll
        for (int f = 0; f < 16; ++f) {
          const float xv = xr[f];
#pragma unroll
          for (int k = 0; k < 4; ++k) gw[k][f] = fmaf(gh[k], xv, gw[k][f]);
        }
      }
    }
  }
  float* P = d.grad_partials + (size_t)blockIdx.x * GRL_CRITIC_GRAD_FLOATS;
  auto combine = [&](float v0, float v1, float v2, float v3, float* dst, int stride) {
    __syncthreads();
    *reinterpret_cast<float4*>(s.red + p * kC + 4 * cg) = make_float4(v0, v1, v2, v3);
    __syncthreads();
    if (threadIdx.x < kC) {
      float a = 0.f;
#pragma unroll
      for (int k = 0; k < 16; ++k) a += s.red[k * kC + threadIdx.x];
      dst[(size_t)threadIdx.x * stride] = a;
    }
  };
  combine(gb1[0], gb1[1], gb1[2], gb1[3], P + 2 * kC, 1);
#pragma unroll
  for (int f = 0; f < 16; ++f) combine(gw[0][f], gw[1][f], gw[2][f], gw[3][f], P + 3 * kC + f, 16);
}

}

extern "C" {

static int critic_check(const GrlCriticDesc* d, const char* who) {
  GRL_REQUIRE(d, GRL_EINVAL, "%s: null descriptor", who);
  GRL_REQUIRE(d->n_graphs > 0 && d->n_tokens > 0 && d->n_feat > 0 && d->n_feat <= 16, GRL_EINVAL,
              "%s: n_graphs=%d n_tokens=%d n_feat=%d (n_feat <= 16)", who, d->n_graphs, d->n_tokens, d->n_feat);
  GRL_REQUIRE(d->x && d->w1 && d->b1 && d->gamma && d->beta && d->stats && d->stat_partials, GRL_EINVAL, "%s: null pointer", who);
  GRL_REQUIRE(d->n_partials > 0 && d->n_partials <= d->n_graphs, GRL_EINVAL, "%s: n_partials=%d must be in [1, n_graphs]", who,
              d->n_partials);
  return GRL_OK;
}

static int critic_grid(const GrlCriticDesc* d) { return d->n_partials; }

int grl_critic_inner_stats(const GrlCriticDesc* d, grl_stream_t stream) {
  const int rc = critic_check(d, "grl_critic_inner_stats");
  if (rc != GRL_OK) return rc;
  const int smem = (int)sizeof(grl::CriticSmem);
  if (grl::ensure_dynamic_smem((const void*)grl::critic_stats_kernel, smem) != GRL_OK) return GRL_ECUDA;
  const int grid = critic_grid(d);
  grl::critic_stats_kernel<<<grid, grl::kCrThreads, smem, (cudaStream_t)stream>>>(*d);
  grl::critic_combine_kernel<<<1, 32, 0, (cudaStream_t)stream>>>(d->stat_partials, grid, 2, d->stats);
  return grl::check_launch("grl_critic_inner_stats");
}

int grl_critic_inner_fwd(const GrlCriticDesc* d, grl_stream_t stream) {
  const int rc = critic_check(d, "grl_critic_inner_fwd");
  if (rc != GRL_OK) return rc;
  GRL_REQUIRE(d->ysum && d->count > 0, GRL_EINVAL, "grl_critic_inner_fwd: ysum / count");
  const int smem = (int)sizeof(grl::CriticSmem);
  if (grl::ensure_dynamic_smem((const void*)grl::critic_fwd_kernel, smem) != GRL_OK) return GRL_ECUDA;
  grl::critic_fwd_kernel<<<critic_grid(d), grl::kCrThreads, smem, (cudaStream_t)stream>>>(*d);
  return grl::check_launch("grl_critic_inner_fwd");
}

int grl_critic_inner_bwd_stats(const GrlCriticDesc* d, grl_stream_t stream) {
  const int rc = critic_check(d, "grl_critic_inner_bwd_stats");
  if (rc != GRL_OK) return rc;
  GRL_REQUIRE(d->grad_ysum && d->bstats && d->grad_partials && d->count > 0, GRL_EINVAL, "grl_critic_inner_bwd_stats: null pointer");
  const int smem = (int)sizeof(grl::CriticSmem);
  if (grl::ensure_dynamic_smem((const void*)grl::critic_bwd_stats_kernel, smem) != GRL_OK) return GRL_ECUDA;
  const int grid = critic_grid(d);
  grl::critic_bwd_stats_kernel<<<grid, grl::kCrThreads, smem, (cudaStream_t)stream>>>(*d);
  grl::critic_combine_kernel<<<1, 32, 0, (cudaStream_t)stream>>>(d->stat_partials, grid, 2, d->bstats);
  return grl::check_launch("grl_critic_inner_bwd_stats");
}

int grl_critic_inner_bwd(const GrlCriticDesc* d, grl_stream_t stream) {
  const int rc = critic_check(d, "grl_critic_inner_bwd");
  if (rc != GRL_OK) return rc;
  GRL_REQUIRE(d->grad_ysum && d->bstats && d->grad_partials && d->count > 0, GRL_EINVAL, "grl_critic_inner_bwd: null pointer");
  const int smem = (int)sizeof(grl::CriticSmem);
  if (grl::ensure_dynamic_smem((const void*)grl::critic_bwd_kernel, smem) != GRL_OK) return GRL_ECUDA;
  grl::critic_bwd_kernel<<<critic_grid(d), grl::kCrThreads, smem, (cudaStream_t)stream>>>(*d);
  return grl::check_launch("grl_critic_inner_bwd");
}

}
```

### geometry_rl_b200/csrc/grl_edge_fused.cu

```cuda
#include <cuda.h>

#include <cstdlib>

#include "grl_common.cuh"
#include "grl_tc.cuh"

namespace grl {


__device__ __forceinline__ int fused_lower_bound(const int32_t* __restrict__ rowptr, int n_nodes, long long target) {
  int lo = 0, hi = n_nodes;
  while (lo < hi) {
    const int mid = (lo + hi) >> 1;
    if (8ll * __ldg(rowptr + mid) + mid < target) lo = mid + 1; else hi = mid;
  }
  return lo;
}

struct RowPos {
  float p[6];
  bool valid;
  __device__ __forceinline__ void load(const GrlFusedEdgeDesc& d, int es, int ed, bool v) {
    valid = v;
    if (v) {
      const float* ps = d.pos_src + 3 * (size_t)es;
      const float* pd = d.pos_dst + 3 * (size_t)ed;
      p[0] = __ldg(ps); p[1] = __ldg(ps + 1); p[2] = __ldg(ps + 2);
      p[3] = __ldg(pd); p[4] = __ldg(pd + 1); p[5] = __ldg(pd + 2);
    }
  }
  __device__ __forceinline__ void emit(const GrlFusedEdgeDesc& d, __nv_bfloat16* __restrict__ F, int r) const {
    const int o = r & 15;
    float f[16];
#pragma unroll
    for (int i = 0; i < 16; ++i) f[i] = 0.f;
    if (valid) {
      const float rx = p[0] - p[3], ry = p[1] - p[4], rz = (d.dim == 3) ? p[2] - p[5] : 0.f;
      const float ox = __ldg(d.ori + 3 * o), oy = __ldg(d.ori + 3 * o + 1), oz = (d.dim == 3) ? __ldg(d.ori + 3 * o + 2) : 0.f;
      const float i1 = (rx * ox + ry * oy) + rz * oz;
      const float tx = rx - i1 * ox, ty = ry - i1 * oy, tz = rz - i1 * oz;
      const float i2 = sqrtf((tx * tx + ty * ty) + tz * tz);
      f[0] = i1; f[1] = i2;
      f[2] = i1 * i1; f[3] = i1 * i2; f[4] = i2 * i1; f[5] = i2 * i2;
      f[6] = f[2] * i1; f[7] = f[2] * i2; f[8] = f[3] * i1; f[9] = f[3] * i2;
      f[10] = f[4] * i1; f[11] = f[4] * i2; f[12] = f[5] * i1; f[13] = f[5] * i2;
      f[14] = 1.0f; f[15] = 1.0f;
    }
    *reinterpret_cast<uint4*>(F + ((size_t)0 * kTM + r) * 8) = tc::pack8(f);
    *reinterpret_cast<uint4*>(F + ((size_t)1 * kTM + r) * 8) = tc::pack8(f + 8);
  }
};

__device__ __forceinline__ void stage_w1_bias(__nv_bfloat16* __restrict__ img, const float* __restrict__ w1,
                                              const float* __restrict__ b1) {
  for (int i = threadIdx.x; i < kC * 16; i += blockDim.x) {
    const int n = i >> 4, f = i & 15;
    float w;
    if (f < GRL_BASIS_FEATS) {
      w = __ldg(w1 + n * GRL_BASIS_FEATS + f);
    } else {
      const float b = __ldg(b1 + n);
      const float hi = __bfloat162float(__float2bfloat16_rn(b));
      w = f == GRL_BASIS_FEATS ? hi : b - hi;
    }
    img[tc::op_index(kC, n, f)] = __float2bfloat16_rn(w);
  }
}

__device__ __forceinline__ void stage_w1_b1_b2(__nv_bfloat16* __restrict__ img, const float* __restrict__ w1,
                                               const float* __restrict__ b1, const float* __restrict__ b2) {
  for (int i = threadIdx.x; i < 2 * kC * 16; i += blockDim.x) {
    const int n = i >> 4, f = i & 15;
    float w = 0.f;
    if (f < GRL_BASIS_FEATS) {
      if (n < kC) w = __ldg(w1 + n * GRL_BASIS_FEATS + f);
    } else {
      const float b = n < kC ? __ldg(b1 + n) : __ldg(b2 + n - kC);
      const float hi = __bfloat162float(__float2bfloat16_rn(b));
      w = f == GRL_BASIS_FEATS ? hi : b - hi;
    }
    img[tc::op_index(2 * kC, n, f)] = __float2bfloat16_rn(w);
  }
}

__device__ __forceinline__ int swz_off(int j, int half, int o, int k) {
  return (((j * 2 + half) * kO + o) << 5) + ((k ^ (o & 7)) << 2);
}

struct FusedFwdSmem {
  __nv_bfloat16 F[kTM * 16];
  __half HB[kTM * kC];
  float XS[kTM * kC];
  __nv_bfloat16 W1b[2 * kC * 16];
  __half W2h[kC * kC];
  __half Wkh[kC * kC];
  int src[4][kTE], dst[4][kTE];
  uint64_t bar[3];
  uint64_t bar_x;
  uint32_t tmem_base;
};

__global__ void __launch_bounds__(kThreads, 3) edge_fused_fwd_kernel(const GrlFusedEdgeDesc d, const __grid_constant__ CUtensorMap tm_xs) {
  extern __shared__ unsigned char smem_raw[];
  FusedFwdSmem& s = *reinterpret_cast<FusedFwdSmem*>(
      smem_raw + ((1024u - (tc::smem_u32(smem_raw) & 1023u)) & 1023u));
  const int tid = threadIdx.x, warp = tid >> 5, lane = tid & 31;
  const int q = warp & 3, ch = warp >> 2, row = 32 * q + lane;
  const int o = tid >> 4, cg = tid & 15;
  if (tid == 0) {
    tc::mbar_init(&s.bar[0], 1);
    tc::mbar_init(&s.bar[1], 1);
    tc::mbar_init(&s.bar[2], 1);
    tc::mbar_init(&s.bar_x, 1);
    tc::fence_mbar_init();
  }
  if (warp == 0) tc::tmem_alloc(&s.tmem_base, 128);
  stage_w1_b1_b2(s.W1b, d.w1, d.b1, d.b2);
  tc::stage_weight_f16(s.W2h, d.w2, kC, kC, kC);
  tc::stage_weight_f16(s.Wkh, d.wk, kC, kC, kC);
  const long long W = 8ll * __ldg(d.rowptr + d.n_key) + d.n_key;
  const int n_lo = blockIdx.x == 0 ? 0 : fused_lower_bound(d.rowptr, d.n_key, W * blockIdx.x / gridDim.x);
  const int n_hi = blockIdx.x + 1 == gridDim.x ? d.n_key : fused_lower_bound(d.rowptr, d.n_key, W * (blockIdx.x + 1) / gridDim.x);
  const int p0 = d.rowptr[n_lo], p1 = d.rowptr[n_hi];
  const int n_tiles = (p1 - p0 + kTE - 1) / kTE;

  auto load_idx = [&](int t, int& es, int& ed) {
    es = 0; ed = 0;
    const int e = p0 + t * kTE + tid;
    if (tid < kTE && t < n_tiles && e < p1) { es = __ldg(d.e_src + e); ed = __ldg(d.e_dst + e); }
  };
  int es_a, ed_a, es_b, ed_b;
  load_idx(0, es_a, ed_a);
  if (tid < kTE) { s.src[0][tid] = es_a; s.dst[0][tid] = ed_a; }
  load_idx(1, es_a, ed_a);
  if (tid < kTE) { s.src[1][tid] = es_a; s.dst[1][tid] = ed_a; }
  load_idx(2, es_a, ed_a);
  load_idx(3, es_b, ed_b);
  tc::fence_async_smem();
  tc::tc_fence_before();
  __syncthreads();
  tc::tc_fence_after();
  const uint32_t tmem = s.tmem_base, lane_addr = tmem + ((uint32_t)(32 * q) << 16);
  const uint32_t fa = tc::smem_u32(s.F), hb = tc::smem_u32(s.HB);
  const uint32_t w1 = tc::smem_u32(s.W1b), w2 = tc::smem_u32(s.W2h), wk = tc::smem_u32(s.Wkh);
  constexpr uint32_t kIdF16 = tc::idesc_f16_ex(128, kC, 0, 0, 0, 0);

  RowPos pos;
  pos.valid = false;
  if (tid < kTM && n_tiles > 0) {
    const int j = tid >> 4;
    pos.load(d, s.src[0][j], s.dst[0][j], p0 + j < p1);
  }

  int cur = n_lo;
  float4 sum = make_float4(0.f, 0.f, 0.f, 0.f);
  for (int t = 0; t < n_tiles; ++t) {
    const int slot = t & 3;
    const uint32_t par = (uint32_t)t & 1u;
    const int cnt = min(kTE, p1 - (p0 + t * kTE));
    if (tid < kTE) { s.src[(t + 2) & 3][tid] = es_a; s.dst[(t + 2) & 3][tid] = ed_a; }
    es_a = es_b; ed_a = ed_b;
    load_idx(t + 4, es_b, ed_b);
    tc::fence_async_smem();
    __syncthreads();
    if (tid >= kTM && tid < kTM + kTE) {
      const int j = tid - kTM;
      if (j < cnt) {
        const int srow = s.src[slot][j] * kO;
        tc::tma_load_2d(s.XS + (j * 2 + 0) * 512, &tm_xs, 0, srow, &s.bar_x);
        tc::tma_load_2d(s.XS + (j * 2 + 1) * 512, &tm_xs, 32, srow, &s.bar_x);
      }
      if (j == 0) tc::mbar_expect_tx(&s.bar_x, (uint32_t)cnt * kO * kC * 4u);
    }
    if (cnt < kTE) {
      for (int i = tid; i < (kTE - cnt) * kRow / 4; i += kThreads)
        reinterpret_cast<float4*>(s.XS + cnt * kRow)[i] = make_float4(0.f, 0.f, 0.f, 0.f);
    }
    if (tid < kTM) {
      const int j = tid >> 4;
      pos.emit(d, s.F, tid);
      const int nb = p0 + (t + 1) * kTE + j;
      pos.load(d, s.src[(t + 1) & 3][j], s.dst[(t + 1) & 3][j], t + 1 < n_tiles && nb < p1);
    }
    if (tid >= kTM && tid < kTM + kTE && t + 1 < n_tiles) {
      const int j = tid - kTM;
      if (p0 + (t + 1) * kTE + j < p1) tc::prefetch_l2(d.x_src + (size_t)s.src[(t + 1) & 3][j] * kRow, kRow * 4u);
    }
    tc::fence_async_smem();
    tc::tc_fence_before();
    __syncthreads();
    if (tid == 0) {
      tc::tc_fence_after();
      tc::issue_mma(tmem, tc::view_k(fa, kTM), tc::view_k(w1, 2 * kC), tc::idesc_bf16(128, 2 * kC), 1, false);
      tc::mma_commit(&s.bar[0]);
    }
    tc::mbar_wait(&s.bar[0], par);
    tc::tc_fence_after();
#pragma unroll
    for (int i = 0; i < 2; ++i) {
      const int c0 = 32 * ch + 16 * i;
      float v[16];
      tc::tmem_ld16(lane_addr + c0, v);
      __half2 h0[4], h1[4];
#pragma unroll
      for (int e = 0; e < 4; ++e) {
        h0[e] = tc::gelu_h2(__floats2half2_rn(v[2 * e], v[2 * e + 1]));
        h1[e] = tc::gelu_h2(__floats2half2_rn(v[8 + 2 * e], v[8 + 2 * e + 1]));
      }
      *reinterpret_cast<uint4*>(s.HB + ((size_t)(c0 >> 3) * kTM + row) * 8) = tc::pack_h8(h0);
      *reinterpret_cast<uint4*>(s.HB + ((size_t)((c0 >> 3) + 1) * kTM + row) * 8) = tc::pack_h8(h1);
    }
    tc::fence_async_smem();
    tc::tc_fence_before();
    __syncthreads();
    if (tid == 0) {
      tc::tc_fence_after();
      tc::issue_mma(tmem + kC, tc::view_k(hb, kTM), tc::view_k(w2, kC), kIdF16, kC / 16, true);
      tc::mma_commit(&s.bar[1]);
    }
    tc::mbar_wait(&s.bar[1], par);
    tc::tc_fence_after();
#pragma unroll
    for (int i = 0; i < 2; ++i) {
      const int c0 = 32 * ch + 16 * i;
      float v[16];
      tc::tmem_ld16(lane_addr + kC + c0, v);
      __half2 h0[4], h1[4];
#pragma unroll
      for (int e = 0; e < 4; ++e) {
        h0[e] = tc::gelu_h2(__floats2half2_rn(v[2 * e], v[2 * e + 1]));
        h1[e] = tc::gelu_h2(__floats2half2_rn(v[8 + 2 * e], v[8 + 2 * e + 1]));
      }
      *reinterpret_cast<uint4*>(s.HB + ((size_t)(c0 >> 3) * kTM + row) * 8) = tc::pack_h8(h0);
      *reinterpret_cast<uint4*>(s.HB + ((size_t)((c0 >> 3) + 1) * kTM + row) * 8) = tc::pack_h8(h1);
    }
    tc::fence_async_smem();
    tc::tc_fence_before();
    __syncthreads();
    if (tid == 0) {
      tc::tc_fence_after();
      tc::issue_mma(tmem, tc::view_k(hb, kTM), tc::view_k(wk, kC), kIdF16, kC / 16, false);
      tc::mma_commit(&s.bar[2]);
    }
    tc::mbar_wait(&s.bar_x, par);
    tc::mbar_wait(&s.bar[2], par);
    tc::tc_fence_after();
#pragma unroll
    for (int i = 0; i < 2; ++i) {
      const int c0 = 32 * ch + 16 * i;
      float v[16];
      tc::tmem_ld16(lane_addr + c0, v);
      float* xs = s.XS + ((((row >> 4) * 2 + ch) * kO + (row & 15)) << 5);
#pragma unroll
      for (int e4 = 0; e4 < 4; ++e4) {
        float* px = xs + (((4 * i + e4) ^ (row & 7)) << 2);
        const int e = 4 * e4;
        float4 x = ld4(px);
        x.x *= v[e]; x.y *= v[e + 1]; x.z *= v[e + 2]; x.w *= v[e + 3];
        st4(px, x);
      }
    }
    tc::tc_fence_before();
    __syncthreads();
#pragma unroll
    for (int j = 0; j < kTE; ++j) {
      if (j < cnt) {
        const int dn = s.dst[slot][j];
        while (cur < dn) {
          st4(d.x1 + (size_t)cur * kRow + o * kC + 4 * cg, sum);
          sum = make_float4(0.f, 0.f, 0.f, 0.f);
          ++cur;
        }
        const float4 m = ld4(s.XS + swz_off(j, cg >> 3, o, cg & 7));
        sum.x += m.x; sum.y += m.y; sum.z += m.z; sum.w += m.w;
      }
    }
  }
  while (cur < n_hi) {
    st4(d.x1 + (size_t)cur * kRow + o * kC + 4 * cg, sum);
    sum = make_float4(0.f, 0.f, 0.f, 0.f);
    ++cur;
  }
  tc::tc_fence_before();
  __syncthreads();
  if (warp == 0) tc::tmem_dealloc(tmem, 128);
}

__device__ __forceinline__ void warp_colsum16(float (&v)[16], int lane) {
#pragma unroll
  for (int step = 0; step < 4; ++step) {
    const int half = 8 >> step;
    const int bit = 16 >> step;
    const bool upper = (lane & bit) != 0;
#pragma unroll
    for (int i = 0; i < half; ++i) {
      const float keep = upper ? v[i + half] : v[i];
      const float send = upper ? v[i] : v[i + half];
      v[i] = keep + __shfl_xor_sync(0xffffffffu, send, bit);
    }
  }
  v[0] += __shfl_xor_sync(0xffffffffu, v[0], 1);
}


constexpr int kWs3Threads = 800;

struct FusedBwdWs3Smem {
  float GX[kTM * kC];
  float XS[kTM * kC];
  float IN[kTM * kC];
  __nv_bfloat16 F[2][kTM * 16];
  __nv_bfloat16 H1[2][kTM * kC];
  __nv_bfloat16 BZ[2][kTM * kC];
  __nv_bfloat16 W1b[kC * 16];
  __nv_bfloat16 Wkb[kC * kC];
  __nv_bfloat16 W2b[kC * kC];
  __nv_bfloat16 G[2][kTM * kC];
  float b2[kC];
  float acc_gb2[4][kC];
  int src[4][kTE], dst[4][kTE], lead[4][kTE];
  int adv[4][kTE];
  uint64_t bar_r[2], bar_c[3], full[2], empty[2];
  uint64_t bar_g, xs_free, gx_free, b2_free;
  uint32_t tmem_base;
};

__global__ void __launch_bounds__(kWs3Threads, 1)
edge_fused_bwd_ws3_kernel(const GrlFusedEdgeDesc d, const __grid_constant__ CUtensorMap tm_gx, const __grid_constant__ CUtensorMap tm_xs,
                          const __grid_constant__ CUtensorMap tm_in) {
  extern __shared__ unsigned char smem_dyn[];
  FusedBwdWs3Smem& s = *reinterpret_cast<FusedBwdWs3Smem*>(
      smem_dyn + ((1024u - (tc::smem_u32(smem_dyn) & 1023u)) & 1023u));
  const int tid = threadIdx.x, warp = tid >> 5, lane = tid & 31;
  const int role = warp < 8 ? 0 : (warp < 16 ? 1 : (warp < 24 ? 2 : 3));
  const int rw = warp & 7;
  const int rt = rw * 32 + lane;
  const int q = rw & 3, ch = rw >> 2, row = 32 * q + lane;
  if (tid == 0) {
    tc::mbar_init(&s.bar_r[0], 1);
    tc::mbar_init(&s.bar_r[1], 1);
    for (int i = 0; i < 3; ++i) tc::mbar_init(&s.bar_c[i], 1);
    tc::mbar_init(&s.full[0], 256);
    tc::mbar_init(&s.full[1], 256);
    tc::mbar_init(&s.empty[0], 1);
    tc::mbar_init(&s.empty[1], 1);
    tc::mbar_init(&s.bar_g, 1);
    tc::mbar_init(&s.xs_free, 256);
    tc::mbar_init(&s.gx_free, 256);
    tc::mbar_init(&s.b2_free, 1);
    tc::fence_mbar_init();
  }
  if (warp == 0) tc::tmem_alloc(&s.tmem_base, 512);
  stage_w1_bias(s.W1b, d.w1, d.b1);
  tc::stage_weight_bf16(s.W2b, d.w2, kC, kC, kC);
  tc::stage_weight_bf16(s.Wkb, d.wk, kC, kC, kC);
  if (tid < kC) s.b2[tid] = __ldg(d.b2 + tid);
  if (tid < 4 * kC) (&s.acc_gb2[0][0])[tid] = 0.f;
  const long long W = 8ll * __ldg(d.rowptr + d.n_key) + d.n_key;
  const int n_lo = blockIdx.x == 0 ? 0 : fused_lower_bound(d.rowptr, d.n_key, W * blockIdx.x / gridDim.x);
  const int n_hi = blockIdx.x + 1 == gridDim.x ? d.n_key : fused_lower_bound(d.rowptr, d.n_key, W * (blockIdx.x + 1) / gridDim.x);
  const int p0 = d.rowptr[n_lo], p1 = d.rowptr[n_hi];
  const int n_tiles = (p1 - p0 + kTE - 1) / kTE;
  tc::fence_async_smem();
  tc::tc_fence_before();
  __syncthreads();
  tc::tc_fence_after();
  const uint32_t tmem = s.tmem_base, lane_addr = tmem + ((uint32_t)(32 * q) << 16);
  const uint32_t w1 = tc::smem_u32(s.W1b), w2 = tc::smem_u32(s.W2b), wk = tc::smem_u32(s.Wkb);
  constexpr uint32_t kScr = 0, kKern = 192, kGB = 256, kGWk = 320, kGW2 = 384, kGW1 = 448;

  if (role == 3) {
    if (lane == 0) {
      tc::tma_prefetch_desc(&tm_gx);
      tc::tma_prefetch_desc(&tm_xs);
    }
    if (lane == 0) tc::tma_prefetch_desc(&tm_in);
    int es = 0, ed = 0, es_n = 0, ed_n = 0;
    int last_key = n_lo;
    auto load_idx = [&](int t_, int& a, int& b_) {
      a = 0; b_ = 0;
      const int e = p0 + t_ * kTE + lane;
      if (lane < kTE && t_ < n_tiles && e < p1) { a = __ldg(d.e_src + e); b_ = __ldg(d.e_dst + e); }
    };
    load_idx(0, es, ed);
    for (int t = 0; t < n_tiles; ++t) {
      const int slot = t & 3;
      const int cnt = min(kTE, p1 - (p0 + t * kTE));
      load_idx(t + 1, es_n, ed_n);
      int prev = __shfl_up_sync(0xffffffffu, es, 1);
      const bool valid = lane < cnt;
      const bool starts = lane == 0 || !valid || es != prev;
      const unsigned heads = __ballot_sync(0xffffffffu, starts);
      const int ld = 31 - __clz(heads & ((2u << lane) - 1u));
      const unsigned leaders = __ballot_sync(0xffffffffu, valid && ld == lane);
      if (lane == 0) prev = last_key;
      const int adv = valid ? es - prev : 0;
      const unsigned run_starts = d.grad_x_src_init ? __ballot_sync(0xffffffffu, adv > 0) : 0u;
      last_key = __shfl_sync(0xffffffffu, es, cnt - 1);
      if (lane < kTE) { s.src[slot][lane] = es; s.dst[slot][lane] = ed; s.lead[slot][lane] = ld; s.adv[slot][lane] = adv; }
      if (lane < kTE && t + 1 < n_tiles && p0 + (t + 1) * kTE + lane < p1) {
        tc::prefetch_l2(d.grad_x1 + (size_t)ed_n * kRow, kRow * 4u);
        tc::prefetch_l2(d.x_src + (size_t)es_n * kRow, kRow * 4u);
        if (d.grad_x_src_init) tc::prefetch_l2(d.grad_x_src_init + (size_t)es_n * kRow, kRow * 4u);
      }
      if (t > 0) tc::mbar_wait(&s.xs_free, (uint32_t)(t - 1) & 1u);
      if (cnt < kTE) {
        for (int i = lane; i < (kTE - cnt) * kRow / 4; i += 32) {
          reinterpret_cast<float4*>(s.XS + cnt * kRow)[i] = make_float4(0.f, 0.f, 0.f, 0.f);
        }
      }
      if (valid && ld == lane) {
        tc::tma_load_2d(s.XS + (lane * 2 + 0) * 512, &tm_xs, 0, es * kO, &s.bar_g);
        tc::tma_load_2d(s.XS + (lane * 2 + 1) * 512, &tm_xs, 32, es * kO, &s.bar_g);
      }
      if (t > 0) tc::mbar_wait(&s.gx_free, (uint32_t)(t - 1) & 1u);
      if (cnt < kTE) {
        for (int i = lane; i < (kTE - cnt) * kRow / 4; i += 32) {
          reinterpret_cast<float4*>(s.GX + cnt * kRow)[i] = make_float4(0.f, 0.f, 0.f, 0.f);
        }
      }
      if (valid) {
        tc::tma_load_2d(s.GX + (lane * 2 + 0) * 512, &tm_gx, 0, ed * kO, &s.bar_g);
        tc::tma_load_2d(s.GX + (lane * 2 + 1) * 512, &tm_gx, 32, ed * kO, &s.bar_g);
      }
      if ((run_starts >> lane) & 1u) {
        tc::tma_load_2d(s.IN + (lane * 2 + 0) * 512, &tm_in, 0, es * kO, &s.bar_g);
        tc::tma_load_2d(s.IN + (lane * 2 + 1) * 512, &tm_in, 32, es * kO, &s.bar_g);
      }
      __syncwarp();
      if (lane == 0) tc::mbar_expect_tx(&s.bar_g, (uint32_t)(cnt + __popc(leaders) + __popc(run_starts)) * kRow * 4u);
      es = es_n; ed = ed_n;
    }
  } else if (role == 0) {
    RowPos pos;
    int es_n = 0, ed_n = 0;
    bool v_n = false;
    auto load_ids = [&](int t_) {
      const int e = p0 + t_ * kTE + (rt >> 4);
      v_n = rt < kTM && t_ < n_tiles && e < p1;
      if (v_n) { es_n = __ldg(d.e_src + e); ed_n = __ldg(d.e_dst + e); }
    };
    pos.valid = false;
    load_ids(0);
    pos.load(d, es_n, ed_n, v_n);
    load_ids(1);
    for (int t = 0; t < n_tiles; ++t) {
      const int b = t & 1;
      const uint32_t par = (uint32_t)t & 1u, parb = (uint32_t)(t >> 1) & 1u;
      const uint32_t fa = tc::smem_u32(s.F[b]), ha = tc::smem_u32(s.H1[b]);
      const uint32_t kSet = 64u + 64u * b;
      tc::mbar_wait(&s.empty[b], parb ^ 1u);
      tc::tc_fence_after();
      if (rt < kTM) {
        pos.emit(d, s.F[b], rt);
        pos.load(d, es_n, ed_n, v_n);
        load_ids(t + 2);
      }
      tc::fence_async_smem();
      tc::tc_fence_before();
      tc::group_sync(1, 256);
      if (rt == 0) {
        tc::tc_fence_after();
        tc::issue_mma(tmem + kScr, tc::view_k(fa, kTM), tc::view_k(w1, kC), tc::idesc_bf16(128, kC), 1, false);
        tc::mma_commit(&s.bar_r[0]);
      }
      tc::mbar_wait(&s.bar_r[0], par);
      tc::tc_fence_after();
#pragma unroll
      for (int layer = 0; layer < 2; ++layer) {
        __nv_bfloat16* img = layer == 0 ? s.H1[b] : s.BZ[b];
        if (layer == 1) {
          tc::fence_async_smem();
          tc::tc_fence_before();
          tc::group_sync(1, 256);
          if (rt == 0) {
            tc::tc_fence_after();
            tc::issue_mma(tmem + kScr, tc::view_k(ha, kTM), tc::view_k(w2, kC), tc::idesc_bf16(128, kC), kC / 16, false);
            tc::mma_commit(&s.bar_r[1]);
          }
          tc::mbar_wait(&s.bar_r[1], par);
          tc::tc_fence_after();
        }
        uint32_t dpk[16];
#pragma unroll
        for (int i = 0; i < 2; ++i) {
          const int c0 = 32 * ch + 16 * i;
          float v[16];
          tc::tmem_ld16(lane_addr + kScr + c0, v);
#pragma unroll
          for (int e = 0; e < 8; ++e) {
            float x0 = v[2 * e], x1 = v[2 * e + 1];
            if (layer == 1) { x0 += s.b2[c0 + 2 * e]; x1 += s.b2[c0 + 2 * e + 1]; }
            __half2 y, dy;
            tc::gelu_h2(__floats2half2_rn(x0, x1), y, dy);
            const float2 yf = __half22float2(y);
            v[2 * e] = yf.x; v[2 * e + 1] = yf.y;
            dpk[8 * i + e] = *reinterpret_cast<const uint32_t*>(&dy);
          }
          *reinterpret_cast<uint4*>(img + ((size_t)(c0 >> 3) * kTM + row) * 8) = tc::pack8(v);
          *reinterpret_cast<uint4*>(img + ((size_t)((c0 >> 3) + 1) * kTM + row) * 8) = tc::pack8(v + 8);
        }
        tc::tmem_st16(lane_addr + kSet + 32 * layer + 16 * ch, dpk);
      }
      tc::tmem_st_wait();
      tc::fence_async_smem();
      tc::tc_fence_before();
      tc::mbar_arrive(&s.full[b]);
    }
  } else if (role == 1) {
    const int o = rt >> 4, cg = rt & 15;
    int cur = n_lo;
    const size_t toff = (size_t)o * kC + 4 * cg;
    const bool has_init = d.grad_x_src_init != nullptr;
    float4 sum = make_float4(0.f, 0.f, 0.f, 0.f);
    float4 init = has_init && cur < n_hi ? ldg4(d.grad_x_src_init + (size_t)cur * kRow + toff) : make_float4(0.f, 0.f, 0.f, 0.f);
    auto fill_gap = [&](int lo, int hi) {
      for (int n = lo; n < hi; ++n)
        st4(d.grad_x_src + (size_t)n * kRow + toff,
            has_init ? ldg4(d.grad_x_src_init + (size_t)n * kRow + toff) : make_float4(0.f, 0.f, 0.f, 0.f));
    };
    const int rj = row >> 4, ro = row & 15;

    for (int t = 0; t < n_tiles; ++t) {
      const int slot = t & 3, b = t & 1;
      const uint32_t par = (uint32_t)t & 1u, parb = (uint32_t)(t >> 1) & 1u;
      const int cnt = min(kTE, p1 - (p0 + t * kTE));
      const bool acc = t > 0;
      const uint32_t bz = tc::smem_u32(s.BZ[b]);
      const uint32_t ga = tc::smem_u32(s.G[b]), xa = ga - kTM * kC * 2;
      __nv_bfloat16* G = s.G[b];
      if (t >= 2) {
        tc::mbar_wait(&s.empty[b], parb ^ 1u);
        tc::tc_fence_after();
      }
      tc::mbar_wait(&s.full[b], parb);
      tc::tc_fence_after();
      if (rt == 0) {
        tc::issue_mma(tmem + kKern, tc::view_k(bz, kTM), tc::view_k(wk, kC), tc::idesc_bf16(128, kC), kC / 16, false);
// ... 54 lines not shown
      }
      tc::fence_async_smem();
      tc::mbar_arrive(&s.gx_free);
    }
    if (cur < n_hi) {
      st4(d.grad_x_src + (size_t)cur * kRow + toff, make_float4(sum.x + init.x, sum.y + init.y, sum.z + init.z, sum.w + init.w));
      fill_gap(cur + 1, n_hi);
    }
  } else {
    for (int t = 0; t < n_tiles; ++t) {
      const int b = t & 1;
      const uint32_t par = (uint32_t)t & 1u, parb = (uint32_t)(t >> 1) & 1u;
      const bool acc = t > 0;
      const uint32_t fa = tc::smem_u32(s.F[b]), ha = tc::smem_u32(s.H1[b]);
      const uint32_t ga = tc::smem_u32(s.G[b]), xa = ga - kTM * kC * 2;
      __nv_bfloat16* G = s.G[b];
      const uint32_t kSet = 64u + 64u * b;
      tc::mbar_wait(&s.full[b], parb);
      tc::mbar_wait(&s.bar_c[1], par);
      tc::tc_fence_after();
      {
        const int h = ch;
        uint32_t dpk[16];
        tc::tmem_ld16_raw(lane_addr + kSet + 32 + 16 * h, dpk);
        float gp2[32];
#pragma unroll
        for (int i = 0; i < 2; ++i) {
          const int c0 = 32 * h + 16 * i;
          float v[16];
          tc::tmem_ld16(lane_addr + kGB + c0, v);
#pragma unroll
          for (int e = 0; e < 8; ++e) {
            const float2 dg = __half22float2(*reinterpret_cast<const __half2*>(&dpk[8 * i + e]));
            gp2[16 * i + 2 * e] = v[2 * e] * dg.x;
            gp2[16 * i + 2 * e + 1] = v[2 * e + 1] * dg.y;
          }
          *reinterpret_cast<uint4*>(G + ((size_t)(c0 >> 3) * kTM + row) * 8) = tc::pack8(gp2 + 16 * i);
          *reinterpret_cast<uint4*>(G + ((size_t)((c0 >> 3) + 1) * kTM + row) * 8) = tc::pack8(gp2 + 16 * i + 8);
        }
        tc::warp_colsum<32>(gp2, lane);
        s.acc_gb2[q][32 * h + lane] += gp2[0];
      }
      tc::fence_async_smem();
      tc::tc_fence_before();
      tc::group_sync(3, 256);
      if (rt == 0) {
        tc::tc_fence_after();
        tc::issue_mma(tmem + kGB, tc::view_k(ga, kTM), tc::view_mn(w2, kC), tc::idesc_bf16_ex(128, 64, 0, 1), kC / 16, false);
        tc::issue_mma(tmem + kGW2, tc::view_mn(xa, kTM), tc::view_mn(ha, kTM), tc::idesc_bf16_ex(128, 64, 1, 1), kTM / 16, acc);
        tc::mma_commit(&s.bar_c[2]);
      }
      tc::mbar_wait(&s.bar_c[2], par);
      tc::tc_fence_after();
      {
        const int h = ch;
        uint32_t dpk[16];
        tc::tmem_ld16_raw(lane_addr + kSet + 16 * h, dpk);
#pragma unroll
        for (int i = 0; i < 2; ++i) {
          const int c0 = 32 * h + 16 * i;
          float v[16];
          tc::tmem_ld16(lane_addr + kGB + c0, v);
#pragma unroll
          for (int e = 0; e < 8; ++e) {
            const float2 dg = __half22float2(*reinterpret_cast<const __half2*>(&dpk[8 * i + e]));
            v[2 * e] *= dg.x;
            v[2 * e + 1] *= dg.y;
          }
          *reinterpret_cast<uint4*>(G + ((size_t)(c0 >> 3) * kTM + row) * 8) = tc::pack8(v);
          *reinterpret_cast<uint4*>(G + ((size_t)((c0 >> 3) + 1) * kTM + row) * 8) = tc::pack8(v + 8);
        }
      }
      tc::fence_async_smem();
      tc::tc_fence_before();
      tc::group_sync(3, 256);
      if (rt == 0) {
        tc::mbar_arrive(&s.b2_free);
        tc::tc_fence_after();
        tc::issue_mma(tmem + kGW1, tc::view_mn(xa, kTM), tc::view_mn(fa, kTM), tc::idesc_bf16_ex(128, 16, 1, 1), kTM / 16, acc);
        tc::mma_commit(&s.empty[b]);
      }
    }
    for (int t = max(0, n_tiles - 2); t < n_tiles; ++t) {
      tc::mbar_wait(&s.empty[t & 1], (uint32_t)(t >> 1) & 1u);
    }
    tc::tc_fence_after();
  }
  tc::tc_fence_before();
  __syncthreads();
  tc::tc_fence_after();
  float* P = d.grad_partials + (size_t)blockIdx.x * GRL_FUSED_EDGE_GRAD_FLOATS;
  if (warp < 16) {
    const int q4 = warp & 3, cq = warp >> 2, row4 = 32 * q4 + lane, c0 = 16 * cq;
    const uint32_t la = tmem + ((uint32_t)(32 * q4) << 16);
    float v[16];
    auto read = [&](uint32_t col) {
      if (n_tiles > 0) {
        tc::tmem_ld16(la + col, v);
      } else {
#pragma unroll
        for (int e = 0; e < 16; ++e) v[e] = 0.f;
      }
    };
    read(kGWk + c0);
    if (row4 >= 64) {
      float* p = P + (size_t)(row4 - 64) * kC + c0;
#pragma unroll
      for (int e = 0; e < 16; e += 4) st4(p + e, make_float4(v[e], v[e + 1], v[e + 2], v[e + 3]));
    }
    read(kGW2 + c0);
    if (row4 >= 64) {
      float* p = P + kWFloats + 64 * 16 + (size_t)(row4 - 64) * kC + c0;
#pragma unroll
      for (int e = 0; e < 16; e += 4) st4(p + e, make_float4(v[e], v[e + 1], v[e + 2], v[e + 3]));
    }
    read(kGW1);
    if (row4 >= 64 && cq == 0) {
      float* p = P + kWFloats + (size_t)(row4 - 64) * 16;
#pragma unroll
      for (int e = 0; e < 16; e += 4) st4(p + e, make_float4(v[e], v[e + 1], v[e + 2], v[e + 3]));
    }
  }
  if (tid < kC)
    P[2 * kWFloats + 64 * 16 + tid] = ((s.acc_gb2[0][tid] + s.acc_gb2[1][tid]) + s.acc_gb2[2][tid]) + s.acc_gb2[3][tid];
  tc::tc_fence_before();
  __syncthreads();
  if (warp == 0) tc::tmem_dealloc(tmem, 512);
}

}

extern "C" {

static int fused_check(const GrlFusedEdgeDesc* d, const char* what) {
  GRL_REQUIRE(d, GRL_EINVAL, "%s: null descriptor", what);
  GRL_REQUIRE(d->n_key > 0 && d->n_edges >= 0 && (d->dim == 2 || d->dim == 3), GRL_EINVAL, "%s: n_key=%d n_edges=%d dim=%d",
              what, d->n_key, d->n_edges, d->dim);
  GRL_REQUIRE(d->rowptr && d->pos_src && d->pos_dst && d->ori && d->w1 && d->b1 && d->w2 && d->b2 && d->wk && d->x_src &&
                  (d->n_edges == 0 || (d->e_src && d->e_dst)), GRL_EINVAL, "%s: null pointer", what);
  return GRL_OK;
}

int grl_fbconv_edge_fused_fwd(const GrlFusedEdgeDesc* d, grl_stream_t stream) {
  const int rc = fused_check(d, "grl_fbconv_edge_fused_fwd");
  if (rc != GRL_OK) return rc;
  GRL_REQUIRE(d->x1, GRL_EINVAL, "grl_fbconv_edge_fused_fwd: x1 is null");
  GRL_REQUIRE(d->n_other > 0, GRL_EINVAL, "grl_fbconv_edge_fused_fwd: n_other=%d (rows of x_src) must be set", d->n_other);
  alignas(64) CUtensorMap tm_xs;
  if (grl::make_row_tensor_map(&tm_xs, d->x_src, d->n_other) != GRL_OK) return GRL_ECUDA;
  const int smem = (int)sizeof(grl::FusedFwdSmem) + 1024;
  if (grl::ensure_dynamic_smem((const void*)grl::edge_fused_fwd_kernel, smem) != GRL_OK) return GRL_ECUDA;
  int grid = 3 * grl::sm_count();
  if (grid > d->n_key) grid = d->n_key;
  grl::edge_fused_fwd_kernel<<<grid, grl::kThreads, smem, (cudaStream_t)stream>>>(*d, tm_xs);
  return grl::check_launch("grl_fbconv_edge_fused_fwd");
}

int grl_fbconv_edge_fused_bwd(const GrlFusedEdgeDesc* d, grl_stream_t stream) {
  const int rc = fused_check(d, "grl_fbconv_edge_fused_bwd");
  if (rc != GRL_OK) return rc;
  GRL_REQUIRE(d->grad_x1 && d->grad_x_src && d->grad_partials, GRL_EINVAL, "grl_fbconv_edge_fused_bwd: null pointer");
  GRL_REQUIRE(d->n_partials > 0 && d->n_partials <= d->n_key, GRL_EINVAL,
              "grl_fbconv_edge_fused_bwd: n_partials=%d must be in [1, n_key]", d->n_partials);
  GRL_REQUIRE(d->n_other > 0, GRL_EINVAL, "grl_fbconv_edge_fused_bwd: n_other=%d (rows of grad_x1) must be set", d->n_other);
  alignas(64) CUtensorMap tm_gx, tm_xs, tm_in;
  if (grl::make_row_tensor_map(&tm_gx, d->grad_x1, d->n_other) != GRL_OK) return GRL_ECUDA;
  if (grl::make_row_tensor_map(&tm_xs, d->x_src, d->n_key) != GRL_OK) return GRL_ECUDA;
  if (grl::make_row_tensor_map(&tm_in, d->grad_x_src_init ? d->grad_x_src_init : d->x_src, d->n_key) != GRL_OK) return GRL_ECUDA;
  const int smem = (int)sizeof(grl::FusedBwdWs3Smem) + 1024;
  if (grl::ensure_dynamic_smem((const void*)grl::edge_fused_bwd_ws3_kernel, smem) != GRL_OK) return GRL_ECUDA;
  grl::edge_fused_bwd_ws3_kernel<<<d->n_partials, grl::kWs3Threads, smem, (cudaStream_t)stream>>>(*d, tm_gx, tm_xs, tm_in);
  return grl::check_launch("grl_fbconv_edge_fused_bwd");
}

}
```

### geometry_rl_b200/csrc/grl_embed.cu

```cuda
#include "grl_common.cuh"

namespace grl {

constexpr int kMaxF = 16;

constexpr int kEmbTile = 16;

__device__ __forceinline__ void embed_stage(const GrlEmbedDesc& d, int n0, int cnt, float* __restrict__ sc, float* __restrict__ vc) {
  const int S = d.n_scalars, V3 = 3 * d.n_vectors;
  if (d.node_ids == nullptr) {
    for (int i = threadIdx.x; i < cnt * S; i += kThreads) sc[i] = d.scalars[(size_t)n0 * S + i];
    for (int i = threadIdx.x; i < cnt * V3; i += kThreads) vc[i] = d.vectors[(size_t)n0 * V3 + i];
  } else {
    for (int i = threadIdx.x; i < cnt * S; i += kThreads) sc[i] = d.scalars[(size_t)__ldg(d.node_ids + n0 + i / S) * S + i % S];
    for (int i = threadIdx.x; i < cnt * V3; i += kThreads) vc[i] = d.vectors[(size_t)__ldg(d.node_ids + n0 + i / V3) * V3 + i % V3];
  }
}

__device__ __forceinline__ void embed_features(const GrlEmbedDesc& d, const float* __restrict__ sc, const float* __restrict__ vc,
                                               int cnt, float* __restrict__ feat) {
  const int S = d.n_scalars, V = d.n_vectors;
  const int j = threadIdx.x >> 4, o = threadIdx.x & 15;
  const float ox = d.ori[3 * o], oy = d.ori[3 * o + 1], oz = (d.dim == 3) ? d.ori[3 * o + 2] : 0.f;
  float f[kMaxF];
#pragma unroll
  for (int i = 0; i < kMaxF; ++i) {
    float v = 0.f;
    if (j < cnt) {
      if (i < S) {
        v = sc[j * S + i];
      } else if (i < S + V) {
        const float* p = vc + (j * V + (i - S)) * 3;
        v = (p[0] * ox + p[1] * oy) + ((d.dim == 3) ? p[2] * oz : 0.f);
      }
    }
    f[i] = v;
  }
  float* dst = feat + (j * kO + o) * kMaxF;
#pragma unroll
  for (int i = 0; i < kMaxF; i += 4) st4(dst + i, make_float4(f[i], f[i + 1], f[i + 2], f[i + 3]));
}

template <int FQ>
__global__ void __launch_bounds__(kThreads, FQ <= 2 ? 4 : 2) embed_fwd_kernel(const GrlEmbedDesc d) {
  __shared__ __align__(16) float feat[kEmbTile * kO * kMaxF];
  __shared__ float sc[kEmbTile * kMaxF], vc[kEmbTile * kMaxF * 3];
  const int tid = threadIdx.x, o = tid >> 4, cg = tid & 15;
  const int F = d.n_scalars + d.n_vectors;
  unsigned long long w01[4 * FQ], w23[4 * FQ];
#pragma unroll
  for (int f = 0; f < 4 * FQ; ++f) {
    float w[4];
#pragma unroll
    for (int i = 0; i < 4; ++i) w[i] = (f < F) ? __ldg(d.weight + (size_t)(4 * cg + i) * F + f) : 0.f;
    w01[f] = pack2(w[0], w[1]);
    w23[f] = pack2(w[2], w[3]);
  }
  const int n_tiles = (d.n_nodes + kEmbTile - 1) / kEmbTile;
  for (int t = blockIdx.x; t < n_tiles; t += gridDim.x) {
    const int n0 = t * kEmbTile, cnt = min(kEmbTile, d.n_nodes - n0);
    __syncthreads();
    embed_stage(d, n0, cnt, sc, vc);
    __syncthreads();
    embed_features(d, sc, vc, cnt, feat);
    __syncthreads();
#pragma unroll 4
    for (int j = 0; j < cnt; ++j) {
      const float* fr = feat + (j * kO + o) * kMaxF;
      unsigned long long a01 = pack2(0.f, 0.f), a23 = a01;
#pragma unroll
      for (int qd = 0; qd < FQ; ++qd) {
        const float4 fv = ld4(fr + 4 * qd);
        const float fe[4] = {fv.x, fv.y, fv.z, fv.w};
#pragma unroll
        for (int e = 0; e < 4; ++e) {
          const unsigned long long ff = pack2(fe[e], fe[e]);
          a01 = ffma2(ff, w01[4 * qd + e], a01);
          a23 = ffma2(ff, w23[4 * qd + e], a23);
        }
      }
      float4 a;
      unpack2(a01, a.x, a.y);
      unpack2(a23, a.z, a.w);
      st4(d.x + (size_t)(n0 + j) * kRow + o * kC + 4 * cg, a);
    }
  }
}

template <int FQ>
__global__ void __launch_bounds__(kThreads, FQ <= 2 ? 4 : 2) embed_bwd_kernel(const GrlEmbedDesc d) {
  __shared__ __align__(16) float feat[kEmbTile * kO * kMaxF];
  __shared__ float sc[kEmbTile * kMaxF], vc[kEmbTile * kMaxF * 3];
  const int tid = threadIdx.x, o = tid >> 4, cg = tid & 15;
  const int F = d.n_scalars + d.n_vectors;
  unsigned long long g01[4 * FQ], g23[4 * FQ];
#pragma unroll
  for (int f = 0; f < 4 * FQ; ++f) g01[f] = g23[f] = pack2(0.f, 0.f);
  const int n_tiles = (d.n_nodes + kEmbTile - 1) / kEmbTile;
  for (int t = blockIdx.x; t < n_tiles; t += gridDim.x) {
    const int n0 = t * kEmbTile, cnt = min(kEmbTile, d.n_nodes - n0);
    __syncthreads();
    embed_stage(d, n0, cnt, sc, vc);
    __syncthreads();
    embed_features(d, sc, vc, cnt, feat);
    __syncthreads();
#pragma unroll 8
    for (int j = 0; j < cnt; ++j) {
      const float4 gx = ldg4(d.grad_x + (size_t)(n0 + j) * kRow + o * kC + 4 * cg);
      const unsigned long long gx01 = pack2(gx.x, gx.y), gx23 = pack2(gx.z, gx.w);
      const float* fr = feat + (j * kO + o) * kMaxF;
#pragma unroll
      for (int qd = 0; qd < FQ; ++qd) {
        const float4 fv = ld4(fr + 4 * qd);
        const float fe[4] = {fv.x, fv.y, fv.z, fv.w};
#pragma unroll
        for (int e = 0; e < 4; ++e) {
          const unsigned long long ff = pack2(fe[e], fe[e]);
          g01[4 * qd + e] = ffma2(gx01, ff, g01[4 * qd + e]);
          g23[4 * qd + e] = ffma2(gx23, ff, g23[4 * qd + e]);
        }
      }
    }
  }
  float* P = d.grad_weight_partials + (size_t)blockIdx.x * kC * F;
  float* red = feat;
#pragma unroll
  for (int f = 0; f < 4 * FQ; ++f) {
    if (f < F) {
      float4 g;
      unpack2(g01[f], g.x, g.y);
      unpack2(g23[f], g.z, g.w);
      __syncthreads();
      st4(red + o * kC + 4 * cg, g);
      __syncthreads();
      if (tid < kC) {
        float t = 0.f;
#pragma unroll
        for (int oo = 0; oo < kO; ++oo) t += red[oo * kC + tid];
        P[tid * F + f] = t;
      }
    }
  }
}

}

extern "C" {

static int check_embed(const GrlEmbedDesc* d, const char* who) {
  GRL_REQUIRE(d, GRL_EINVAL, "%s: null descriptor", who);
  GRL_REQUIRE(d->n_nodes > 0 && (d->dim == 2 || d->dim == 3), GRL_EINVAL, "%s: n_nodes=%d dim=%d", who, d->n_nodes, d->dim);
  GRL_REQUIRE(d->n_scalars >= 0 && d->n_vectors >= 0 && d->n_scalars + d->n_vectors >= 1 &&
                  d->n_scalars + d->n_vectors <= grl::kMaxF, GRL_EUNSUPPORTED, "%s: S+V=%d not in [1,16]", who,
              d->n_scalars + d->n_vectors);
  GRL_REQUIRE((d->n_scalars == 0 || d->scalars) && (d->n_vectors == 0 || d->vectors) && d->ori, GRL_EINVAL,
              "%s: null pointer", who);
  return GRL_OK;
}

int grl_embed_fwd(const GrlEmbedDesc* d, grl_stream_t stream) {
  const int rc = check_embed(d, "grl_embed_fwd");
  if (rc != GRL_OK) return rc;
  GRL_REQUIRE(d->weight && d->x, GRL_EINVAL, "grl_embed_fwd: null pointer");
  const int n_tiles = (d->n_nodes + grl::kEmbTile - 1) / grl::kEmbTile;
  const int fq = (d->n_scalars + d->n_vectors + 3) / 4;
  int grid = (fq <= 2 ? 8 : 6) * grl::sm_count();
  if (grid > n_tiles) grid = n_tiles;
  cudaStream_t st = (cudaStream_t)stream;
  if (fq == 1) grl::embed_fwd_kernel<1><<<grid, grl::kThreads, 0, st>>>(*d);
  else if (fq == 2) grl::embed_fwd_kernel<2><<<grid, grl::kThreads, 0, st>>>(*d);
  else if (fq == 3) grl::embed_fwd_kernel<3><<<grid, grl::kThreads, 0, st>>>(*d);
  else grl::embed_fwd_kernel<4><<<grid, grl::kThreads, 0, st>>>(*d);
  return grl::check_launch("grl_embed_fwd");
}

int grl_embed_bwd(const GrlEmbedDesc* d, grl_stream_t stream) {
  const int rc = check_embed(d, "grl_embed_bwd");
  if (rc != GRL_OK) return rc;
  GRL_REQUIRE(d->grad_x && d->grad_weight_partials && d->n_partials > 0, GRL_EINVAL, "grl_embed_bwd: null pointer");
  const int fq = (d->n_scalars + d->n_vectors + 3) / 4;
  cudaStream_t st = (cudaStream_t)stream;
  if (fq == 1) grl::embed_bwd_kernel<1><<<d->n_partials, grl::kThreads, 0, st>>>(*d);
  else if (fq == 2) grl::embed_bwd_kernel<2><<<d->n_partials, grl::kThreads, 0, st>>>(*d);
  else if (fq == 3) grl::embed_bwd_kernel<3><<<d->n_partials, grl::kThreads, 0, st>>>(*d);
  else grl::embed_bwd_kernel<4><<<d->n_partials, grl::kThreads, 0, st>>>(*d);
  return grl::check_launch("grl_embed_bwd");
}

}
```

### geometry_rl_b200/csrc/grl_readout.cu

```cuda
#include "grl_common.cuh"

namespace grl {

constexpr int kMaxJ = GRL_READOUT_MAX_OUT;

__device__ __forceinline__ float warp_sum(float v) {
#pragma unroll
  for (int o = 16; o > 0; o >>= 1) v += __shfl_xor_sync(0xffffffffu, v, o);
  return v;
}

struct ReadoutRow {
  float2 hid;
  float2 V[3];
};

__device__ __forceinline__ ReadoutRow reduce_row(const float* __restrict__ row, const float (&ori)[kO][3], int lane) {
  ReadoutRow r;
  r.hid = make_float2(0.f, 0.f);
  r.V[0] = r.V[1] = r.V[2] = make_float2(0.f, 0.f);
#pragma unroll
  for (int o = 0; o < kO; ++o) {
    const float2 x = __ldg(reinterpret_cast<const float2*>(row + o * kC) + lane);
    r.hid.x += x.x; r.hid.y += x.y;
#pragma unroll
    for (int dd = 0; dd < 3; ++dd) { r.V[dd].x = fmaf(x.x, ori[o][dd], r.V[dd].x); r.V[dd].y = fmaf(x.y, ori[o][dd], r.V[dd].y); }
  }
  const float s = 1.0f / kO;
  r.hid.x *= s; r.hid.y *= s;
#pragma unroll
  for (int dd = 0; dd < 3; ++dd) { r.V[dd].x *= s; r.V[dd].y *= s; }
  return r;
}

__global__ void __launch_bounds__(256) readout_fwd_kernel(const GrlReadoutDesc d) {
  __shared__ float s_ori[kO][3];
  __shared__ float s_obar[3];
  if (threadIdx.x < kO * 3) s_ori[threadIdx.x / 3][threadIdx.x % 3] = d.ori[threadIdx.x];
  __syncthreads();
  if (threadIdx.x < 3) {
    float a = 0.f;
    for (int o = 0; o < kO; ++o) a += s_ori[o][threadIdx.x];
    s_obar[threadIdx.x] = a / kO;
  }
  __syncthreads();
  float ori[kO][3];
#pragma unroll
  for (int o = 0; o < kO; ++o) { ori[o][0] = s_ori[o][0]; ori[o][1] = s_ori[o][1]; ori[o][2] = s_ori[o][2]; }
  const int lane = threadIdx.x & 31, od = d.od, odv = d.odv;
  const int warps_per_grid = gridDim.x * (blockDim.x >> 5);
  for (int n = blockIdx.x * (blockDim.x >> 5) + (threadIdx.x >> 5); n < d.n_nodes; n += warps_per_grid) {
    const ReadoutRow r = reduce_row(d.latent + (size_t)n * kRow, ori, lane);
    reinterpret_cast<float2*>(d.hidden + (size_t)n * kC)[lane] = r.hid;
    float os[kMaxJ];
#pragma unroll
    for (int s = 0; s < kMaxJ; ++s) {
      os[s] = 0.f;
      if (s < od) {
        const float2 w = __ldg(reinterpret_cast<const float2*>(d.weight + s * kC) + lane);
        os[s] = warp_sum(w.x * r.hid.x + w.y * r.hid.y) + __ldg(d.bias + s);
      }
    }
#pragma unroll
    for (int v = 0; v < kMaxJ; ++v) {
      if (v < odv) {
        const float2 w = __ldg(reinterpret_cast<const float2*>(d.weight + (od + v) * kC) + lane);
        const float bj = __ldg(d.bias + od + v);
        const float gate = os[od == 1 ? 0 : v];
#pragma unroll
        for (int dd = 0; dd < 3; ++dd) {
          const float ov = warp_sum(w.x * r.V[dd].x + w.y * r.V[dd].y) + bj * s_obar[dd];
          if (lane == 0) d.out[((size_t)n * odv + v) * 3 + dd] = dd < d.dim ? ov * gate : 0.f;
        }
      }
    }
  }
}

__global__ void __launch_bounds__(256) readout_bwd_kernel(const GrlReadoutDesc d) {
  __shared__ float s_ori[kO][3];
  __shared__ float s_obar[3];
  __shared__ float s_gw[8][kMaxJ * kC + kMaxJ];
  if (threadIdx.x < kO * 3) s_ori[threadIdx.x / 3][threadIdx.x % 3] = d.ori[threadIdx.x];
  for (int i = threadIdx.x; i < 8 * (kMaxJ * kC + kMaxJ); i += blockDim.x) (&s_gw[0][0])[i] = 0.f;
  __syncthreads();
  if (threadIdx.x < 3) {
    float a = 0.f;
    for (int o = 0; o < kO; ++o) a += s_ori[o][threadIdx.x];
    s_obar[threadIdx.x] = a / kO;
  }
  __syncthreads();
  float ori[kO][3];
#pragma unroll
  for (int o = 0; o < kO; ++o) { ori[o][0] = s_ori[o][0]; ori[o][1] = s_ori[o][1]; ori[o][2] = s_ori[o][2]; }
  const int lane = threadIdx.x & 31, warp = threadIdx.x >> 5, od = d.od, odv = d.odv, J = od + odv;
  float* gw = s_gw[warp];
  const int warps_per_grid = gridDim.x * (blockDim.x >> 5);
  for (int n = blockIdx.x * (blockDim.x >> 5) + warp; n < d.n_nodes; n += warps_per_grid) {
    const ReadoutRow r = reduce_row(d.latent + (size_t)n * kRow, ori, lane);
    float os[kMaxJ], g_os[kMaxJ];
#pragma unroll
    for (int s = 0; s < kMaxJ; ++s) {
      os[s] = 0.f; g_os[s] = 0.f;
      if (s < od) {
        const float2 w = __ldg(reinterpret_cast<const float2*>(d.weight + s * kC) + lane);
        os[s] = warp_sum(w.x * r.hid.x + w.y * r.hid.y) + __ldg(d.bias + s);
      }
    }
    float2 g_hid = d.grad_hidden ? reinterpret_cast<const float2*>(d.grad_hidden + (size_t)n * kC)[lane] : make_float2(0.f, 0.f);
    float2 gV[3] = {make_float2(0.f, 0.f), make_float2(0.f, 0.f), make_float2(0.f, 0.f)};
#pragma unroll
    for (int v = 0; v < kMaxJ; ++v) {
      if (v < odv) {
        const int j = od + v, sidx = od == 1 ? 0 : v;
        const float2 w = __ldg(reinterpret_cast<const float2*>(d.weight + j * kC) + lane);
        const float bj = __ldg(d.bias + j);
        float gb = 0.f;
        float2 gwj = make_float2(0.f, 0.f);
#pragma unroll
        for (int dd = 0; dd < 3; ++dd) {
          if (dd < d.dim) {
            const float go = __ldg(d.grad_out + ((size_t)n * odv + v) * 3 + dd);
            const float ov = warp_sum(w.x * r.V[dd].x + w.y * r.V[dd].y) + bj * s_obar[dd];
            const float g_ov = go * os[sidx];
            g_os[sidx] += go * ov;
            gV[dd].x = fmaf(g_ov, w.x, gV[dd].x); gV[dd].y = fmaf(g_ov, w.y, gV[dd].y);
            gwj.x = fmaf(g_ov, r.V[dd].x, gwj.x); gwj.y = fmaf(g_ov, r.V[dd].y, gwj.y);
            gb = fmaf(g_ov, s_obar[dd], gb);
          }
        }
        gw[j * kC + 2 * lane] += gwj.x;
        gw[j * kC + 2 * lane + 1] += gwj.y;
        if (lane == 0) gw[J * kC + j] += gb;
      }
    }
#pragma unroll
    for (int s = 0; s < kMaxJ; ++s) {
      if (s < od) {
        const float2 w = __ldg(reinterpret_cast<const float2*>(d.weight + s * kC) + lane);
        g_hid.x = fmaf(g_os[s], w.x, g_hid.x); g_hid.y = fmaf(g_os[s], w.y, g_hid.y);
        gw[s * kC + 2 * lane] += g_os[s] * r.hid.x;
        gw[s * kC + 2 * lane + 1] += g_os[s] * r.hid.y;
        if (lane == 0) gw[J * kC + s] += g_os[s];
      }
    }
    const float sc = 1.0f / kO;
    float* gl = d.grad_latent + (size_t)n * kRow;
#pragma unroll
    for (int o = 0; o < kO; ++o) {
      float2 g;
      g.x = sc * (g_hid.x + gV[0].x * ori[o][0] + gV[1].x * ori[o][1] + gV[2].x * ori[o][2]);
      g.y = sc * (g_hid.y + gV[0].y * ori[o][0] + gV[1].y * ori[o][1] + gV[2].y * ori[o][2]);
      reinterpret_cast<float2*>(gl + o * kC)[lane] = g;
    }
  }
  __syncthreads();
  float* P = d.grad_partials + (size_t)blockIdx.x * (J * kC + J);
  for (int i = threadIdx.x; i < J * kC + J; i += blockDim.x) {
    float a = 0.f;
#pragma unroll
    for (int w = 0; w < 8; ++w) a += s_gw[w][i];
    P[i] = a;
  }
}

}

extern "C" {

static int check_readout(const GrlReadoutDesc* d, const char* who, bool bwd) {
  GRL_REQUIRE(d, GRL_EINVAL, "%s: null descriptor", who);
  GRL_REQUIRE(d->n_nodes > 0 && (d->dim == 2 || d->dim == 3), GRL_EINVAL, "%s: n_nodes=%d dim=%d", who, d->n_nodes, d->dim);
  GRL_REQUIRE(d->od >= 1 && d->odv >= 1 && d->od + d->odv <= GRL_READOUT_MAX_OUT && (d->od == d->odv || d->od == 1),
              GRL_EUNSUPPORTED, "%s: od=%d odv=%d (need od == odv or od == 1, od + odv <= %d)", who, d->od, d->odv,
              GRL_READOUT_MAX_OUT);
  GRL_REQUIRE(d->latent && d->weight && d->bias && d->ori, GRL_EINVAL, "%s: null pointer", who);
  if (bwd) GRL_REQUIRE(d->grad_out && d->grad_latent && d->grad_partials && d->n_partials > 0, GRL_EINVAL, "%s: null grad pointer", who);
  else GRL_REQUIRE(d->out && d->hidden, GRL_EINVAL, "%s: null output pointer", who);
  return GRL_OK;
}

int grl_readout_fwd(const GrlReadoutDesc* d, grl_stream_t stream) {
  const int rc = check_readout(d, "grl_readout_fwd", false);
  if (rc != GRL_OK) return rc;
  int grid = (d->n_nodes + 7) / 8;
  const int cap = 4 * grl::sm_count();
  if (grid > cap) grid = cap;
  grl::readout_fwd_kernel<<<grid, 256, 0, (cudaStream_t)stream>>>(*d);
  return grl::check_launch("grl_readout_fwd");
}

int grl_readout_bwd(const GrlReadoutDesc* d, grl_stream_t stream) {
  const int rc = check_readout(d, "grl_readout_bwd", true);
  if (rc != GRL_OK) return rc;
  grl::readout_bwd_kernel<<<d->n_partials, 256, 0, (cudaStream_t)stream>>>(*d);
  return grl::check_launch("grl_readout_bwd");
}

}
```

### geometry_rl_b200/csrc/grl_trpl.cu

```cuda
#include "grl_common.cuh"

namespace grl {

constexpr int kMaxK = GRL_MAX_ACTION_DIM;

struct KlEval {
  double kl, dkl;
};

struct KlInv {
  double io[kMaxK], ic[kMaxK], lo[kMaxK];
};
__device__ __forceinline__ KlEval kl_eval(const KlInv& q, int k, double eta) {
  KlEval r{0.0, 0.0};
  const double e1 = eta + 1.0, ie1 = 1.0 / e1;
#pragma unroll
  for (int i = 0; i < kMaxK; ++i) {
    if (i < k) {
      const double D = fma(eta, q.io[i], q.ic[i]);
      const double rD = 1.0 / D;
      const double ct = e1 * rD;
      r.kl += fma(ct, q.io[i], -1.0) + q.lo[i] - log(ct);
      const double dct = (q.ic[i] - q.io[i]) * rD * rD;
      r.dkl += (q.io[i] - D * ie1) * dct;
    }
  }
  r.kl *= 0.5;
  r.dkl *= 0.5;
  return r;
}

__global__ void __launch_bounds__(128) trpl_fwd_kernel(const GrlProjDesc d) {
  const int b = blockIdx.x * blockDim.x + threadIdx.x;
  if (b >= d.batch) return;
  const int k = d.k;
  float m[kMaxK], v[kMaxK], mo[kMaxK], vo[kMaxK];
#pragma unroll
  for (int i = 0; i < kMaxK; ++i) {
    if (i < k) {
      m[i] = d.mean[(size_t)b * k + i];
      v[i] = d.v[(size_t)b * k + i];
      mo[i] = d.old_mean[(size_t)b * k + i];
      vo[i] = d.old_v[(size_t)b * k + i];
    } else {
      m[i] = mo[i] = 0.f;
      v[i] = vo[i] = 1.f;
    }
  }
  float maha = 0.f;
#pragma unroll
  for (int i = 0; i < kMaxK; ++i)
    if (i < k) { const float t = (m[i] - mo[i]) / vo[i]; maha += t * t; }
  const float mean_part = d.proj_type == 0 ? 0.5f * maha : maha;
  float omega = 0.f;
  const bool mean_active = mean_part > d.eps_mean;
  if (mean_active) omega = fabsf(sqrtf(mean_part / d.eps_mean) - 1.0f);
#pragma unroll
  for (int i = 0; i < kMaxK; ++i)
    if (i < k) d.proj_mean[(size_t)b * k + i] = mean_active ? (m[i] + omega * mo[i]) / (1.0f + omega + 1e-16f) : m[i];

  d.eta[2 * (size_t)b + 1] = mean_active ? (double)omega : 0.0;

  if (d.proj_type == 0) {
    double c[kMaxK], o[kMaxK];
    KlInv q;
#pragma unroll
    for (int i = 0; i < kMaxK; ++i) {
      c[i] = (double)(v[i] * v[i]);
      o[i] = (double)(vo[i] * vo[i]);
      q.io[i] = 1.0 / o[i];
      q.ic[i] = 1.0 / c[i];
      q.lo[i] = i < k ? log(o[i]) : 0.0;
    }
    const double eps = (double)d.eps_cov;
    double eta = 0.0;
    KlEval f = kl_eval(q, k, 0.0);
    if (f.kl > eps) {
      double lo = 0.0, hi = 1.0;
      for (int it = 0; it < 200; ++it) {
        if (kl_eval(q, k, hi).kl <= eps) break;
        lo = hi;
        hi *= 2.0;
      }
      eta = 0.5 * (lo + hi);
      for (int it = 0; it < 100; ++it) {
        f = kl_eval(q, k, eta);
        const double res = f.kl - eps;
        if (res > 0.0) lo = eta; else hi = eta;
        if (fabs(res) <= 1e-14 * eps || (hi - lo) <= 1e-15 * hi) break;
        double nxt = eta - res / f.dkl;
        if (!(nxt > lo && nxt < hi)) nxt = 0.5 * (lo + hi);
        eta = nxt;
      }
    }
    d.eta[2 * (size_t)b] = eta;
#pragma unroll
    for (int i = 0; i < kMaxK; ++i) {
      if (i < k) {
        const float ct = eta > 0.0 ? (float)((eta + 1.0) / (eta / o[i] + 1.0 / c[i])) : v[i] * v[i];
        d.proj_v[(size_t)b * k + i] = sqrtf(ct);
      }
    }
  } else {
    float cov_part = 0.f;
#pragma unroll
    for (int i = 0; i < kMaxK; ++i)
      if (i < k) { const float inv = 1.0f / vo[i]; cov_part += 1.0f + inv * (v[i] * v[i]) * inv - 2.0f * inv * v[i]; }
    float eta = 0.f;
    const bool active = cov_part > d.eps_cov;
    if (active) eta = fabsf(sqrtf(cov_part / d.eps_cov) - 1.0f);
    d.eta[2 * (size_t)b] = active ? (double)eta : 0.0;
#pragma unroll
    for (int i = 0; i < kMaxK; ++i)
      if (i < k) d.proj_v[(size_t)b * k + i] = active ? (v[i] + eta * vo[i]) / (1.0f + eta + 1e-16f) : v[i];
  }
}

__global__ void __launch_bounds__(128) trpl_bwd_kernel(const GrlProjDesc d) {
  const int b = blockIdx.x * blockDim.x + threadIdx.x;
  if (b >= d.batch) return;
  const int k = d.k;
  double m[kMaxK], v[kMaxK], mo[kMaxK], vo[kMaxK], gm[kMaxK], gv[kMaxK];
  double am[kMaxK], av[kMaxK];
#pragma unroll
  for (int i = 0; i < kMaxK; ++i) {
    am[i] = (i < k && d.grad_mean_add) ? (double)d.grad_mean_add[(size_t)b * k + i] : 0.0;
    av[i] = (i < k && d.grad_v_add) ? (double)d.grad_v_add[(size_t)b * k + i] : 0.0;
  }
#pragma unroll
  for (int i = 0; i < kMaxK; ++i) {
    if (i < k) {
      m[i] = d.mean[(size_t)b * k + i];
      v[i] = d.v[(size_t)b * k + i];
      mo[i] = d.old_mean[(size_t)b * k + i];
      vo[i] = d.old_v[(size_t)b * k + i];
      gm[i] = d.grad_proj_mean[(size_t)b * k + i];
      gv[i] = d.grad_proj_v[(size_t)b * k + i];
    } else {
      m[i] = mo[i] = gm[i] = gv[i] = 0.0;
      v[i] = vo[i] = 1.0;
    }
  }
  const double scale = d.proj_type == 0 ? 0.5 : 1.0;
  double M = 0.0;
#pragma unroll
  for (int i = 0; i < kMaxK; ++i)
    if (i < k) { const double t = (m[i] - mo[i]) / vo[i]; M += t * t; }
  M *= scale;
  const double eps_m = (double)d.eps_mean;
  if (d.eta[2 * (size_t)b + 1] > 0.0) {
    const double w = sqrt(M / eps_m) - 1.0;
    double dot = 0.0;
#pragma unroll
    for (int i = 0; i < kMaxK; ++i)
      if (i < k) dot += gm[i] * (mo[i] - m[i]) / ((1.0 + w) * (1.0 + w));
    const double dw_dM = 1.0 / (2.0 * eps_m * (1.0 + w));
#pragma unroll
    for (int i = 0; i < kMaxK; ++i)
      if (i < k)
        d.grad_mean[(size_t)b * k + i] =
            (float)(gm[i] / (1.0 + w) + dot * dw_dM * scale * 2.0 * (m[i] - mo[i]) / (vo[i] * vo[i]) + am[i]);
  } else {
#pragma unroll
    for (int i = 0; i < kMaxK; ++i)
      if (i < k) d.grad_mean[(size_t)b * k + i] = (float)(gm[i] + am[i]);
  }
  const double eta = d.eta[2 * (size_t)b];
  if (d.proj_type == 0) {
    if (eta > 0.0) {
      double num = 0.0, den = 0.0;
      double gct[kMaxK], dct_dc[kMaxK], dkl_dct[kMaxK];
#pragma unroll
      for (int i = 0; i < kMaxK; ++i) {
        gct[i] = dct_dc[i] = dkl_dct[i] = 0.0;
        if (i < k) {
          const double c = v[i] * v[i], o = vo[i] * vo[i];
          const double D = eta / o + 1.0 / c;
          const double ct = (eta + 1.0) / D;
          gct[i] = gv[i] / (2.0 * sqrt(ct));
          dct_dc[i] = (eta + 1.0) / (D * D * c * c);
          const double dct_deta = (1.0 / c - 1.0 / o) / (D * D);
          dkl_dct[i] = 0.5 * (1.0 / o - 1.0 / ct);
          num += gct[i] * dct_deta;
          den += dkl_dct[i] * dct_deta;
        }
      }
#pragma unroll
      for (int i = 0; i < kMaxK; ++i)
        if (i < k) {
          const double gc = gct[i] * dct_dc[i] - num * (dkl_dct[i] * dct_dc[i]) / den;
          d.grad_v[(size_t)b * k + i] = (float)(gc * 2.0 * v[i] + av[i]);
        }
    } else {
#pragma unroll
      for (int i = 0; i < kMaxK; ++i)
        if (i < k) d.grad_v[(size_t)b * k + i] = (float)(gv[i] + av[i]);
    }
  } else {
    if (eta > 0.0) {
      double dot = 0.0;
#pragma unroll
      for (int i = 0; i < kMaxK; ++i)
        if (i < k) dot += gv[i] * (vo[i] - v[i]) / ((1.0 + eta) * (1.0 + eta));
      const double deta_dS = 1.0 / (2.0 * (double)d.eps_cov * (1.0 + eta));
#pragma unroll
      for (int i = 0; i < kMaxK; ++i)
        if (i < k)
          d.grad_v[(size_t)b * k + i] =
              (float)(gv[i] / (1.0 + eta) + dot * deta_dS * 2.0 * (v[i] / vo[i] - 1.0) / vo[i] + av[i]);
    } else {
#pragma unroll
      for (int i = 0; i < kMaxK; ++i)
        if (i < k) d.grad_v[(size_t)b * k + i] = (float)(gv[i] + av[i]);
    }
  }
}


constexpr double kLog2Pi = 1.8378770664093454835606594728112;

__global__ void __launch_bounds__(128) trpl_loss_terms_kernel(const GrlLossDesc d) {
  const int b = blockIdx.x * blockDim.x + threadIdx.x;
  if (b >= d.batch) return;
  const int k = d.k;
  double maha_a = 0.0, logdet_pv = 0.0, log_pv = 0.0, log_v = 0.0, maha_m = 0.0, trace = 0.0, w2_cov = 0.0;
#pragma unroll
  for (int i = 0; i < kMaxK; ++i) {
    if (i < k) {
      const size_t j = (size_t)b * k + i;
      const double m = d.mean[j], v = d.v[j], pm = d.proj_mean[j], pv = d.proj_v[j], a = d.action[j];
      maha_a += (a - pm) * (a - pm) / pv;
      logdet_pv += log(pv);
      log_pv += log(pv);
      log_v += log(v);
      const double t = (m - pm) / pv;
      maha_m += t * t;
      trace += (v / pv) * (v / pv);
      w2_cov += 1.0 + v * v / (pv * pv) - 2.0 * v / pv;
    }
  }
  const double log_prob = -0.5 * (maha_a + k * kLog2Pi + logdet_pv);
  const double kl_mean = 0.5 * maha_m;
  const double kl_cov = 0.5 * (trace - k + 2.0 * log_pv - 2.0 * log_v);
  const double tr_mean = d.proj_type == 0 ? kl_mean : maha_m;
  const double tr_cov = d.proj_type == 0 ? kl_cov : w2_cov;
  double* T = d.terms + (size_t)b * GRL_LOSS_TERMS;
  T[0] = log_prob - (double)d.prev_log_prob[b];
  T[1] = tr_mean;
  T[2] = tr_cov;
  T[3] = kl_mean + kl_cov;
  T[4] = 0.5 * (k * (1.0 + kLog2Pi) + logdet_pv);
  T[5] = 0.5 * (k * (1.0 + kLog2Pi) + 2.0 * log_v);
  T[6] = 0.5 * (k * (1.0 + kLog2Pi) + 2.0 * log_pv);
  T[7] = (double)d.advantage[b];
}

constexpr int kLossThreads = 1024;

__device__ __forceinline__ double block_sum(double x, double* sh) {
#pragma unroll
  for (int o = 16; o > 0; o >>= 1) x += __shfl_xor_sync(0xffffffffu, x, o);
  __syncthreads();
  if ((threadIdx.x & 31) == 0) sh[threadIdx.x >> 5] = x;
  __syncthreads();
  x = sh[threadIdx.x & 31];
#pragma unroll
  for (int o = 16; o > 0; o >>= 1) x += __shfl_xor_sync(0xffffffffu, x, o);
  return x;
}
__device__ __forceinline__ double block_max(double x, double* sh) {
#pragma unroll
  for (int o = 16; o > 0; o >>= 1) x = fmax(x, __shfl_xor_sync(0xffffffffu, x, o));
  __syncthreads();
  if ((threadIdx.x & 31) == 0) sh[threadIdx.x >> 5] = x;
  __syncthreads();
  x = sh[threadIdx.x & 31];
#pragma unroll
  for (int o = 16; o > 0; o >>= 1) x = fmax(x, __shfl_xor_sync(0xffffffffu, x, o));
  return x;
}

__global__ void dp_combine_kernel(const double* __restrict__ gathered, int world, int n, int n_sum, double* __restrict__ out) {
  const int i = threadIdx.x;
  if (i >= n) return;
  double acc = gathered[i];
  for (int r = 1; r < world; ++r) {
    const double v = gathered[(size_t)r * n + i];
    acc = i < n_sum ? acc + v : fmax(acc, v);
  }
  out[i] = acc;
}

__global__ void __launch_bounds__(kLossThreads) trpl_loss_stats_kernel(const GrlLossDesc d) {
  __shared__ double sh[32];
  const int B = d.batch, tid = threadIdx.x;
  const double* T = d.terms;
  double s = 0.0, q = 0.0, mx = -1e300;
  for (int b = tid; b < B; b += kLossThreads) {
    const double a = T[(size_t)b * GRL_LOSS_TERMS + 7];
    s += a;
    q += a * a;
    mx = fmax(mx, T[(size_t)b * GRL_LOSS_TERMS]);
  }
  s = block_sum(s, sh);
  q = block_sum(q, sh);
  mx = block_max(mx, sh);
  if (tid == 0) { d.stats[0] = s; d.stats[1] = q; d.stats[2] = (double)B; d.stats[3] = mx; }
}

__global__ void __launch_bounds__(kLossThreads) trpl_loss_sums_kernel(const GrlLossDesc d) {
  __shared__ double sh[32];
  const int B = d.batch, tid = threadIdx.x;
  const double* T = d.terms;
  const double n = d.stats[2];
  double loc = 0.0, inv_scale = 1.0;
  if (d.normalize_advantage && n > 1.0) {
    loc = d.stats[0] / n;
    const double var = fmax((d.stats[1] - n * loc * loc) / (n - 1.0), 0.0);
    inv_scale = 1.0 / fmax(sqrt(var), 1e-6);
  }
  const double mx = d.stats[3];
  double s_obj = 0.0, s_e1 = 0.0, s_e2 = 0.0, s_trm = 0.0, s_trc = 0.0, s_kl = 0.0, s_hd = 0.0, s_hp = 0.0, s_hq = 0.0;
  double m_trm = -1e300, m_trc = -1e300;
  for (int b = tid; b < B; b += kLossThreads) {
    const double* t = T + (size_t)b * GRL_LOSS_TERMS;
    const double lw = t[0];
    s_obj += exp(lw) * ((t[7] - loc) * inv_scale);
    const double e = exp(lw - mx);
    s_e1 += e;
    s_e2 += e * e;
    s_trm += t[1]; s_trc += t[2]; s_kl += t[3]; s_hd += t[4]; s_hp += t[5]; s_hq += t[6];
    m_trm = fmax(m_trm, t[1]);
    m_trc = fmax(m_trc, t[2]);
  }
  s_obj = block_sum(s_obj, sh); s_e1 = block_sum(s_e1, sh); s_e2 = block_sum(s_e2, sh);
  s_trm = block_sum(s_trm, sh); s_trc = block_sum(s_trc, sh); s_kl = block_sum(s_kl, sh);
  s_hd = block_sum(s_hd, sh); s_hp = block_sum(s_hp, sh); s_hq = block_sum(s_hq, sh);
  m_trm = block_max(m_trm, sh); m_trc = block_max(m_trc, sh);
  if (tid == 0) {
    double* S = d.sums;
    S[0] = s_obj; S[1] = s_trm + s_trc; S[2] = s_hd;
    S[3] = s_e1; S[4] = s_e2; S[5] = s_trm; S[6] = s_trc; S[7] = s_kl; S[8] = s_hp; S[9] = s_hq - s_hp;
    S[10] = m_trm; S[11] = m_trc;
    d.stats[4] = loc;
    d.stats[5] = inv_scale;
  }
}

__global__ void trpl_loss_finalize_kernel(const GrlLossDesc d) {
  if (threadIdx.x != 0 || blockIdx.x != 0) return;
  const double n = d.stats[2];
  const double* G = d.sums;
  float* S = d.scalars;
  S[GRL_LS_LOSS_OBJECTIVE] = (float)(-G[0] / n);
  S[GRL_LS_LOSS_TRUST_REGION] = (float)(G[1] / n * (double)d.trust_region_coeff);
  S[GRL_LS_LOSS_ENTROPY] = (float)(-(double)d.entropy_coef * G[2] / n);
  S[GRL_LS_DIST_ENTROPY] = (float)(G[2] / n);
  S[GRL_LS_ESS] = (float)(G[3] * G[3] / G[4] / n);
  S[GRL_LS_KL] = (float)(G[7] / n);
  S[GRL_LS_CONSTRAINT] = (float)((G[5] + G[6]) / n);
  S[GRL_LS_MEAN_CONSTRAINT] = (float)(G[5] / n);
  S[GRL_LS_MEAN_CONSTRAINT_MAX] = (float)G[10];
  S[GRL_LS_COV_CONSTRAINT] = (float)(G[6] / n);
  S[GRL_LS_COV_CONSTRAINT_MAX] = (float)G[11];
  S[GRL_LS_ENTROPY] = (float)(G[8] / n);
  S[GRL_LS_ENTROPY_DIFF] = (float)(G[9] / n);
  for (int i = GRL_LS_ENTROPY_DIFF + 1; i < GRL_LOSS_SCALARS; ++i) S[i] = 0.f;
}

__global__ void __launch_bounds__(128) trpl_loss_bwd_kernel(const GrlLossDesc d) {
  const int b = blockIdx.x * blockDim.x + threadIdx.x;
  if (b >= d.batch) return;
  const int k = d.k;
  const double n = d.stats[2];
  const double g_obj = d.grad_losses[0], g_tr = d.grad_losses[1], g_ent = d.grad_losses[2];
  const double* T = d.terms + (size_t)b * GRL_LOSS_TERMS;
  const double adv = (T[7] - d.stats[4]) * d.stats[5];
  const double g_lw = -g_obj / n * exp(T[0]) * adv;
  const double c_ent = -g_ent * (double)d.entropy_coef / n;
  const double c_tr = g_tr * (double)d.trust_region_coeff / n;
#pragma unroll
  for (int i = 0; i < kMaxK; ++i) {
    if (i < k) {
      const size_t j = (size_t)b * k + i;
      const double m = d.mean[j], v = d.v[j], pm = d.proj_mean[j], pv = d.proj_v[j], a = d.action[j];
      const double r = a - pm;
      d.grad_proj_mean[j] = (float)(g_lw * r / pv);
      d.grad_proj_v[j] = (float)(g_lw * 0.5 * (r * r / (pv * pv) - 1.0 / pv) + c_ent * 0.5 / pv);
      double gm, gv;
      if (d.proj_type == 0) {
        gm = (m - pm) / (pv * pv);
        gv = v / (pv * pv) - 1.0 / v;
      } else {
        gm = 2.0 * (m - pm) / (pv * pv);
        gv = 2.0 * v / (pv * pv) - 2.0 / pv;
      }
      d.grad_mean_direct[j] = (float)(c_tr * gm);
      d.grad_v_direct[j] = (float)(c_tr * gv);
    }
  }
}

}

extern "C" {

static int check_proj(const GrlProjDesc* d, const char* who, bool bwd) {
  GRL_REQUIRE(d, GRL_EINVAL, "%s: null descriptor", who);
  GRL_REQUIRE(d->batch > 0 && d->k > 0, GRL_EINVAL, "%s: batch=%d k=%d", who, d->batch, d->k);
  GRL_REQUIRE(d->k <= GRL_MAX_ACTION_DIM, GRL_EUNSUPPORTED, "%s: k=%d > %d", who, d->k, GRL_MAX_ACTION_DIM);
  GRL_REQUIRE(d->proj_type == 0 || d->proj_type == 1, GRL_EUNSUPPORTED, "%s: proj_type=%d", who, d->proj_type);
  GRL_REQUIRE(d->eps_mean > 0.f && d->eps_cov > 0.f, GRL_EINVAL, "%s: bounds must be positive", who);
  GRL_REQUIRE(d->mean && d->v && d->old_mean && d->old_v && d->eta, GRL_EINVAL, "%s: null pointer", who);
  if (bwd) GRL_REQUIRE(d->grad_proj_mean && d->grad_proj_v && d->grad_mean && d->grad_v, GRL_EINVAL, "%s: null grad pointer", who);
  else GRL_REQUIRE(d->proj_mean && d->proj_v, GRL_EINVAL, "%s: null output pointer", who);
  return GRL_OK;
}

int grl_trpl_fwd(const GrlProjDesc* d, grl_stream_t stream) {
  const int rc = check_proj(d, "grl_trpl_fwd", false);
  if (rc != GRL_OK) return rc;
  grl::trpl_fwd_kernel<<<(d->batch + 127) / 128, 128, 0, (cudaStream_t)stream>>>(*d);
  return grl::check_launch("grl_trpl_fwd");
}

int grl_trpl_bwd(const GrlProjDesc* d, grl_stream_t stream) {
  const int rc = check_proj(d, "grl_trpl_bwd", true);
  if (rc != GRL_OK) return rc;
  grl::trpl_bwd_kernel<<<(d->batch + 127) / 128, 128, 0, (cudaStream_t)stream>>>(*d);
  return grl::check_launch("grl_trpl_bwd");
}

static int check_loss(const GrlLossDesc* d, const char* who, bool bwd) {
  GRL_REQUIRE(d, GRL_EINVAL, "%s: null descriptor", who);
  GRL_REQUIRE(d->batch > 0 && d->k > 0, GRL_EINVAL, "%s: batch=%d k=%d", who, d->batch, d->k);
  GRL_REQUIRE(d->k <= GRL_MAX_ACTION_DIM, GRL_EUNSUPPORTED, "%s: k=%d > %d", who, d->k, GRL_MAX_ACTION_DIM);
  GRL_REQUIRE(d->proj_type == 0 || d->proj_type == 1, GRL_EUNSUPPORTED, "%s: proj_type=%d", who, d->proj_type);
  GRL_REQUIRE(d->mean && d->v && d->proj_mean && d->proj_v && d->action && d->terms && d->stats, GRL_EINVAL,
              "%s: null pointer", who);
  if (bwd) GRL_REQUIRE(d->grad_losses && d->grad_proj_mean && d->grad_proj_v && d->grad_mean_direct && d->grad_v_direct,
                       GRL_EINVAL, "%s: null grad pointer", who);
  else GRL_REQUIRE(d->prev_log_prob && d->advantage && d->scalars && d->sums, GRL_EINVAL, "%s: null input / output pointer", who);
  return GRL_OK;
}

int grl_trpl_loss_fwd(const GrlLossDesc* d, grl_stream_t stream) {
  const int rc = check_loss(d, "grl_trpl_loss_fwd", false);
  if (rc != GRL_OK) return rc;
  GRL_REQUIRE(d->stage >= 0 && d->stage <= 3, GRL_EINVAL, "grl_trpl_loss_fwd: stage=%d", d->stage);
  cudaStream_t st = (cudaStream_t)stream;
  if (d->stage == 0 || d->stage == 1) {
    grl::trpl_loss_terms_kernel<<<(d->batch + 127) / 128, 128, 0, st>>>(*d);
    grl::trpl_loss_stats_kernel<<<1, grl::kLossThreads, 0, st>>>(*d);
  }
  if (d->stage == 0 || d->stage == 2) grl::trpl_loss_sums_kernel<<<1, grl::kLossThreads, 0, st>>>(*d);
  if (d->stage == 0 || d->stage == 3) grl::trpl_loss_finalize_kernel<<<1, 32, 0, st>>>(*d);
  return grl::check_launch("grl_trpl_loss_fwd");
}

int grl_dp_combine(const double* gathered, int world, int n, int n_sum, double* out, grl_stream_t stream) {
  GRL_REQUIRE(gathered && out && world > 0 && n > 0 && n <= 32 && n_sum >= 0 && n_sum <= n, GRL_EINVAL,
              "grl_dp_combine: world=%d n=%d n_sum=%d", world, n, n_sum);
  grl::dp_combine_kernel<<<1, 32, 0, (cudaStream_t)stream>>>(gathered, world, n, n_sum, out);
  return grl::check_launch("grl_dp_combine");
}

int grl_trpl_loss_bwd(const GrlLossDesc* d, grl_stream_t stream) {
  const int rc = check_loss(d, "grl_trpl_loss_bwd", true);
  if (rc != GRL_OK) return rc;
  grl::trpl_loss_bwd_kernel<<<(d->batch + 127) / 128, 128, 0, (cudaStream_t)stream>>>(*d);
  return grl::check_launch("grl_trpl_loss_bwd");
}

}
```

### geometry_rl_b200/csrc/grl_util.cu

```cuda
#include <cstdarg>
#include <cstdio>
#include <atomic>
#include <mutex>
#include <utility>
#include <vector>

#include <cuda.h>

#include "grl_common.cuh"

namespace grl {

typedef CUresult (*EncodeTiledFn)(CUtensorMap*, CUtensorMapDataType, cuuint32_t, void*, const cuuint64_t*, const cuuint64_t*,
                                  const cuuint32_t*, const cuuint32_t*, CUtensorMapInterleave, CUtensorMapSwizzle,
                                  CUtensorMapL2promotion, CUtensorMapFloatOOBfill);

static EncodeTiledFn encode_tiled_fn() {
  static EncodeTiledFn fn = [] {
    void* p = nullptr;
    cudaDriverEntryPointQueryResult q;
    if (cudaGetDriverEntryPoint("cuTensorMapEncodeTiled", &p, cudaEnableDefault, &q) != cudaSuccess ||
        q != cudaDriverEntryPointSuccess)
      p = nullptr;
    return reinterpret_cast<EncodeTiledFn>(p);
  }();
  return fn;
}

int make_row_tensor_map(void* out, const float* base, long long n_nodes, int box_rows) {
  EncodeTiledFn fn = encode_tiled_fn();
  if (!fn) {
    set_error("cuTensorMapEncodeTiled is not available from this driver");
    return GRL_ECUDA;
  }
  const cuuint64_t gdim[2] = {(cuuint64_t)kC, (cuuint64_t)n_nodes * kO};
  const cuuint64_t gstride[1] = {(cuuint64_t)kC * sizeof(float)};
  const cuuint32_t box[2] = {32u, (cuuint32_t)box_rows};
  const cuuint32_t estr[2] = {1u, 1u};
  const CUresult r = fn(reinterpret_cast<CUtensorMap*>(out), CU_TENSOR_MAP_DATA_TYPE_FLOAT32, 2, const_cast<float*>(base), gdim,
                        gstride, box, estr, CU_TENSOR_MAP_INTERLEAVE_NONE, CU_TENSOR_MAP_SWIZZLE_128B,
                        CU_TENSOR_MAP_L2_PROMOTION_L2_256B, CU_TENSOR_MAP_FLOAT_OOB_FILL_NONE);
  if (r != CUDA_SUCCESS) {
    set_error("cuTensorMapEncodeTiled failed with CUresult %d (base %p, %lld nodes)", (int)r, (const void*)base, n_nodes);
    return GRL_ECUDA;
  }
  return GRL_OK;
}

static thread_local char g_err[512] = "";

void set_error(const char* fmt, ...) {
  va_list ap;
  va_start(ap, fmt);
  vsnprintf(g_err, sizeof(g_err), fmt, ap);
  va_end(ap);
}

int check_launch(const char* what) {
  const cudaError_t e = cudaGetLastError();
  if (e != cudaSuccess) {
    set_error("%s: %s", what, cudaGetErrorString(e));
    return GRL_ECUDA;
  }
  return GRL_OK;
}

static std::atomic<int> g_reserved_sms{0};

int sm_count() {
  static int cached[64] = {0};
  int dev = 0;
  if (cudaGetDevice(&dev) != cudaSuccess || dev < 0 || dev >= 64) return 148 - g_reserved_sms.load(std::memory_order_relaxed);
  if (cached[dev] == 0) {
    int n = 0;
    if (cudaDeviceGetAttribute(&n, cudaDevAttrMultiProcessorCount, dev) != cudaSuccess || n <= 0) n = 148;
    cached[dev] = n;
  }
  const int usable = cached[dev] - g_reserved_sms.load(std::memory_order_relaxed);
  return usable > 1 ? usable : 1;
}

int ensure_dynamic_smem(const void* func, int bytes) {
  static std::mutex mu;
  static std::vector<std::pair<const void*, int>> done;
  int dev = 0;
  if (cudaGetDevice(&dev) != cudaSuccess) {
    set_error("cudaGetDevice failed");
    return GRL_ECUDA;
  }
  std::lock_guard<std::mutex> lock(mu);
  for (const auto& e : done)
    if (e.first == func && e.second == dev) return GRL_OK;
  const cudaError_t err = cudaFuncSetAttribute(func, cudaFuncAttributeMaxDynamicSharedMemorySize, bytes);
  if (err != cudaSuccess) {
    set_error("cudaFuncSetAttribute(MaxDynamicSharedMemorySize=%d): %s", bytes, cudaGetErrorString(err));
    return GRL_ECUDA;
  }
  done.emplace_back(func, dev);
  return GRL_OK;
}

__global__ void __launch_bounds__(256) reduce_partials_kernel(const float* __restrict__ partials, int n_partials, int64_t n,
                                                              float* __restrict__ out, int accumulate) {
  __shared__ float seg_sum[8][32];
  const int lane = threadIdx.x & 31, seg = threadIdx.x >> 5;
  const int per = (n_partials + 7) / 8;
  const int p0 = seg * per, p1 = min(n_partials, p0 + per);
  for (int64_t base = (int64_t)blockIdx.x * 32; base < n; base += (int64_t)gridDim.x * 32) {
    const int64_t i = base + lane;
    float a0 = 0.f, a1 = 0.f, a2 = 0.f, a3 = 0.f;
    if (i < n) {
      int p = p0;
      for (; p + 3 < p1; p += 4) {
        a0 += partials[(int64_t)p * n + i];
        a1 += partials[(int64_t)(p + 1) * n + i];
        a2 += partials[(int64_t)(p + 2) * n + i];
        a3 += partials[(int64_t)(p + 3) * n + i];
      }
      for (; p < p1; ++p) a0 += partials[(int64_t)p * n + i];
    }
    seg_sum[seg][lane] = (a0 + a1) + (a2 + a3);
    __syncthreads();
    if (seg == 0 && i < n) {
      float s = seg_sum[0][lane];
#pragma unroll
      for (int k = 1; k < 8; ++k) s += seg_sum[k][lane];
      out[i] = accumulate ? out[i] + s : s;
    }
    __syncthreads();
  }
}

__global__ void __launch_bounds__(256) absmax_kernel(const float4* __restrict__ x, int64_t n4, const float* __restrict__ tail,
                                                     int n_tail, unsigned int* __restrict__ out_bits) {
  unsigned int m = 0u;
  for (int64_t i = blockIdx.x * (int64_t)blockDim.x + threadIdx.x; i < n4; i += (int64_t)gridDim.x * blockDim.x) {
    const float4 v = __ldg(x + i);
    const float a = fmaxf(fmaxf(fabsf(v.x), fabsf(v.y)), fmaxf(fabsf(v.z), fabsf(v.w)));
    m = max(m, __float_as_uint(a));
  }
  if (blockIdx.x == 0 && (int)threadIdx.x < n_tail) m = max(m, __float_as_uint(fabsf(tail[threadIdx.x])));
#pragma unroll
  for (int o = 16; o > 0; o >>= 1) m = max(m, __shfl_xor_sync(0xffffffffu, m, o));
  __shared__ unsigned int wm[8];
  if ((threadIdx.x & 31) == 0) wm[threadIdx.x >> 5] = m;
  __syncthreads();
  if (threadIdx.x == 0) {
#pragma unroll
    for (int w = 1; w < 8; ++w) m = max(m, wm[w]);
    atomicMax(out_bits, m);
  }
}

}

extern "C" {

int grl_abi_version(void) { return 1; }
const char* grl_last_error(void) { return grl::g_err; }
int grl_sm_count(void) { return grl::sm_count(); }
int grl_reserve_sms(int n) {
  GRL_REQUIRE(n >= 0 && n <= 64, GRL_EINVAL, "grl_reserve_sms: n=%d outside [0, 64]", n);
  grl::g_reserved_sms.store(n, std::memory_order_relaxed);
  return GRL_OK;
}

int grl_reduce_partials(const float* partials, int n_partials, int64_t n_floats, float* out, int accumulate,
                        grl_stream_t stream) {
  GRL_REQUIRE(partials && out && n_partials > 0 && n_floats > 0, GRL_EINVAL, "grl_reduce_partials: bad arguments");
  int64_t blocks = (n_floats + 31) / 32;
  if (blocks > 16 * grl::sm_count()) blocks = 16 * grl::sm_count();
  grl::reduce_partials_kernel<<<(int)blocks, 256, 0, (cudaStream_t)stream>>>(partials, n_partials, n_floats, out, accumulate);
  return grl::check_launch("grl_reduce_partials");
}

int grl_absmax(const float* x, int64_t n, uint32_t* out_bits, grl_stream_t stream) {
  GRL_REQUIRE(x && out_bits && n > 0, GRL_EINVAL, "grl_absmax: bad arguments");
  GRL_REQUIRE((reinterpret_cast<uintptr_t>(x) & 15) == 0, GRL_EINVAL, "grl_absmax: x must be 16-byte aligned");
  cudaStream_t s = (cudaStream_t)stream;
  if (cudaMemsetAsync(out_bits, 0, sizeof(uint32_t), s) != cudaSuccess) return grl::check_launch("grl_absmax (memset)");
  const int64_t n4 = n / 4;
  int64_t blocks = (n4 + 255) / 256;
  if (blocks > 8 * grl::sm_count()) blocks = 8 * grl::sm_count();
  if (blocks < 1) blocks = 1;
  grl::absmax_kernel<<<(int)blocks, 256, 0, s>>>(reinterpret_cast<const float4*>(x), n4, x + 4 * n4, (int)(n - 4 * n4), out_bits);
  return grl::check_launch("grl_absmax");
}

}
```

### include/grl_b200.h

```cpp
#ifndef GRL_B200_H_
#define GRL_B200_H_

#include <stdint.h>

#ifdef __cplusplus
extern "C" {
#endif

#define GRL_OK 0
#define GRL_EINVAL (-1)
#define GRL_EUNSUPPORTED (-2)
#define GRL_ECUDA (-3)

#define GRL_NUM_ORI 16
#define GRL_CHANNELS 64
#define GRL_HIDDEN 256
#define GRL_BASIS_FEATS 14
#define GRL_MAX_ACTION_DIM 16
#define GRL_MAX_KNN 8

typedef void* grl_stream_t;

int grl_abi_version(void);
const char* grl_last_error(void);
int grl_sm_count(void);
int grl_reserve_sms(int n);


int grl_knn_edge_ptr(const int32_t* num_valid, int B, int P, int k, int64_t* edge_ptr, grl_stream_t stream);

int grl_knn_graph(const float* pos, const int32_t* num_valid, const int64_t* edge_ptr, int B, int P, int k,
                  int64_t* coo, int64_t coo_row_stride, grl_stream_t stream);

int grl_radius_neighbors(const float* pos, const int32_t* num_valid, int B, int P, float radius, int max_neighbors,
                         int32_t* nbr, int32_t* cnt, grl_stream_t stream);

int grl_radius_edge_ptr(const int32_t* cnt, int B, int P, int64_t capacity, int64_t* edge_ptr, grl_stream_t stream);

int grl_radius_graph(const int32_t* nbr, const int32_t* cnt, const int64_t* edge_ptr, int B, int P, int max_neighbors,
                     int64_t* coo, int64_t coo_row_stride, int64_t capacity, grl_stream_t stream);

int grl_dense_edges(int mode, const int32_t* num_valid, const int64_t* edge_ptr, int B, int n_src, int n_dst,
                    int64_t* coo, int64_t coo_row_stride, grl_stream_t stream);

int grl_csr_build(const int64_t* coo, int64_t coo_row_stride, const int64_t* edge_ptr, int B, int n_key, int key_row,
                  int32_t* rowptr, int32_t* other, int32_t* eid, grl_stream_t stream);


typedef struct {
  int32_t n_nodes, n_scalars, n_vectors, dim;
  const float* scalars;
  const float* vectors;
  const float* ori;
  const float* weight;
  float* x;
  const float* grad_x;
  float* grad_weight_partials;
  int32_t n_partials;
  const int32_t* node_ids;
} GrlEmbedDesc;
int grl_embed_fwd(const GrlEmbedDesc* d, grl_stream_t stream);
int grl_embed_bwd(const GrlEmbedDesc* d, grl_stream_t stream);

typedef struct {
  int32_t n_edges, dim;
  const int32_t* edge_src;
  const int32_t* edge_dst;
  const float* pos_src;
  const float* pos_dst;
  const float* ori;
  const float* w1t;
  const float* b1;
  const float* w2t;
  const float* b2;
  float* basis;
  const float* w2;
  const float* grad_basis;
  float* grad_partials;
  int32_t n_partials;
  void* basis_bf16;
  const void* grad_basis_bf16;
} GrlBasisDesc;
#define GRL_BASIS_GRAD_FLOATS (64 * 16 + 64 + 64 * 64 + 64)
int grl_edge_basis_fwd(const GrlBasisDesc* d, grl_stream_t stream);
int grl_edge_basis_bwd(const GrlBasisDesc* d, grl_stream_t stream);

typedef struct {
  int32_t n_src, n_dst, n_edges;
  const int32_t* rowptr_dst;
  const int32_t* edge_src;
  const int32_t* edge_dst;
  const int32_t* rowptr_src;
  const int32_t* src_eid;
  const float* x_src;
  const float* x_dst;
  const float* basis;
  const float* fiber_kernel;
  const float* wk_t;
  const float* wk;
  const float* bias;
  const float* ln_g;
  const float* ln_b;
  const float* w1_t;
  const float* w1;
  const float* b1;
  const float* w2_t;
  const float* w2_c;
  const float* b2;
  float* x1;
  float* out;
  int32_t accumulate_out;
  const float* grad_out;
  float* grad_x1;
  float* grad_x_src;
  const float* grad_x_src_init;
  float* grad_basis;
  int32_t accumulate_grad_basis;
  float* node_grad_partials;
  int32_t n_partials_node;
  float* edge_grad_partials;
  int32_t n_partials_edge;
  const float* w2;
  const void* basis_bf16;
  void* grad_basis_bf16;
  float* grad_x2;
  float* x2;
  const uint32_t* grad_amax;
  const int32_t* basis_row;
  const int32_t* grad_basis_acc_mask;
} GrlConvDesc;
#define GRL_NODE_GRAD_FLOATS (256 * 64 + 256 + 64 * 256 + 64 + 64 + 64 + 64 + 16 * 16 * 64)
int grl_fbconv_edge_fwd(const GrlConvDesc* d, grl_stream_t stream);
int grl_fbconv_node_fwd(const GrlConvDesc* d, grl_stream_t stream);
int grl_fbconv_node_bwd(const GrlConvDesc* d, grl_stream_t stream);
int grl_fbconv_edge_bwd(const GrlConvDesc* d, grl_stream_t stream);
int grl_edge_basis_fwd_tc(const GrlBasisDesc* d, grl_stream_t stream);
int grl_fbconv_edge_fwd_tc(const GrlConvDesc* d, grl_stream_t stream);
int grl_fbconv_node_fwd_tc(const GrlConvDesc* d, grl_stream_t stream);
int grl_fbconv_edge_bwd_tc(const GrlConvDesc* d, grl_stream_t stream);
int grl_edge_basis_bwd_tc(const GrlBasisDesc* d, grl_stream_t stream);
int grl_fbconv_node_bwd_tc(const GrlConvDesc* d, grl_stream_t stream);

typedef struct {
  int32_t n_key, n_edges, dim, n_partials;
  const int32_t* rowptr;
  const int32_t* e_src;
  const int32_t* e_dst;
  const float* pos_src;
  const float* pos_dst;
  const float* ori;
  const float* w1;
  const float* b1;
  const float* w2;
  const float* b2;
  const float* wk;
  const float* x_src;
  float* x1;
  const float* grad_x1;
  float* grad_x_src;
  const float* grad_x_src_init;
  float* grad_partials;
  int32_t n_other;
} GrlFusedEdgeDesc;
#define GRL_FUSED_EDGE_GRAD_FLOATS (64 * 64 + 64 * 16 + 64 * 64 + 64)
int grl_fbconv_edge_fused_fwd(const GrlFusedEdgeDesc* d, grl_stream_t stream);
int grl_fbconv_edge_fused_bwd(const GrlFusedEdgeDesc* d, grl_stream_t stream);

int grl_absmax(const float* x, int64_t n, uint32_t* out_bits, grl_stream_t stream);

int grl_reduce_partials(const float* partials, int n_partials, int64_t n_floats, float* out, int accumulate,
                        grl_stream_t stream);

typedef struct {
  int32_t n_graphs, n_tokens, n_feat, n_partials;
  float eps;
  double count;
  const float* x;
  const float* w1;
  const float* b1;
// ... 166 lines not shown
```

Before: 973,500.

## Enable programmatic dependent launch across kernels and deepen fiber bwd pipeline

Launches most kernels with the programmatic stream serialization attribute. Each kernel calls griddepcontrol.wait before touching dependent data and signals launch_dependents on its last tile, so the next kernel's prologue (weight staging, smem init) can overlap the tail of the previous one. The fiber backward kernel moves from a 2-stage to a 4-stage cp.async pipeline, and the absmax loop is unrolled 4x. PDL is on by default and can be switched off with an env var; the cost is extra shared memory in the fiber kernel, and any kernel that reads producer data before its wait would be a correctness hazard.

Result: no change. 978,600, median of 6 (+0.5%).

```diff
diff --git a/geometry_rl_b200/_lib.py b/geometry_rl_b200/_lib.py
--- a/geometry_rl_b200/_lib.py
+++ b/geometry_rl_b200/_lib.py
@@ -117,6 +117,8 @@
     "grl_last_error": (C.c_char_p, []),
     "grl_sm_count": (C.c_int, []),
     "grl_reserve_sms": (C.c_int, [C.c_int]),
+    "grl_set_pdl": (C.c_int, [C.c_int]),
+    "grl_pdl_enabled": (C.c_int, []),
     "grl_knn_edge_ptr": (C.c_int, [_fp, C.c_int, C.c_int, C.c_int, _fp, _fp]),
     "grl_knn_graph": (C.c_int, [_fp, _fp, _fp, C.c_int, C.c_int, C.c_int, _fp, C.c_int64, _fp]),
     "grl_radius_neighbors": (C.c_int, [_fp, _fp, C.c_int, C.c_int, C.c_float, C.c_int, _fp, _fp, _fp]),
@@ -257,3 +259,11 @@
     global _sm
     check(load().grl_reserve_sms(int(n)), "grl_reserve_sms")
     _sm = None
+
+
+def set_pdl(on: bool) -> None:
+    check(load().grl_set_pdl(1 if on else 0), "grl_set_pdl")
+
+
+def pdl_enabled() -> bool:
+    return bool(load().grl_pdl_enabled())
diff --git a/geometry_rl_b200/csrc/grl_common.cuh b/geometry_rl_b200/csrc/grl_common.cuh
--- a/geometry_rl_b200/csrc/grl_common.cuh
+++ b/geometry_rl_b200/csrc/grl_common.cuh
@@ -1,6 +1,8 @@
 #pragma once
 #include <cuda_runtime.h>
 #include <stdint.h>
+
+#include <utility>
 
 #include "../../include/grl_b200.h"
 
@@ -30,6 +32,31 @@
       return (code);                  \
     }                                 \
   } while (0)
+
+bool pdl_enabled();
+__device__ __forceinline__ void griddep_wait() { asm volatile("griddepcontrol.wait;" ::: "memory"); }
+__device__ __forceinline__ void griddep_launch_dependents() { asm volatile("griddepcontrol.launch_dependents;" ::: "memory"); }
+
+template <typename... P, typename... A>
+int launch_pdl(const char* what, void (*kernel)(P...), dim3 grid, dim3 block, size_t smem, cudaStream_t stream, A&&... args) {
+  cudaLaunchAttribute attr;
+  attr.id = cudaLaunchAttributeProgrammaticStreamSerialization;
+  attr.val.programmaticStreamSerializationAllowed = 1;
+  cudaLaunchConfig_t cfg = {};
+  cfg.gridDim = grid;
+  cfg.blockDim = block;
+  cfg.dynamicSmemBytes = smem;
+  cfg.stream = stream;
+  cfg.attrs = &attr;
+  cfg.numAttrs = pdl_enabled() ? 1 : 0;
+  const cudaError_t e = cudaLaunchKernelEx(&cfg, kernel, std::forward<A>(args)...);
+  if (e != cudaSuccess) {
+    (void)cudaGetLastError();
+    set_error("%s: %s", what, cudaGetErrorString(e));
+    return GRL_ECUDA;
+  }
+  return check_launch(what);
+}
 
 __device__ __forceinline__ float gelu_f(float x) { return 0.5f * x * (1.0f + erff(x * 0.70710678118654752440f)); }
 __device__ __forceinline__ float gelu_grad_f(float x) {
diff --git a/geometry_rl_b200/csrc/grl_conv_node_bwd_tc.cu b/geometry_rl_b200/csrc/grl_conv_node_bwd_tc.cu
--- a/geometry_rl_b200/csrc/grl_conv_node_bwd_tc.cu
+++ b/geometry_rl_b200/csrc/grl_conv_node_bwd_tc.cu
@@ -95,6 +95,7 @@
   for (int i = tid; i < 4 * kC; i += kNB3Threads) {
     (&s.acc_gb2[0][0])[i] = 0.f; (&s.acc_glng[0][0])[i] = 0.f; (&s.acc_glnb[0][0])[i] = 0.f;
   }
+  griddep_wait();
   const float gscale = d.grad_amax ? tc::grad_scale_from_amax(__ldg(d.grad_amax)) : 1.0f;
   const float inv_gscale = 1.0f / gscale;
   const int n_tiles = (d.n_dst + kTE - 1) / kTE;
@@ -144,6 +145,7 @@
     auto pre = [&](int qq, uint32_t col) { tc::issue_mma_fast<kKb / 16>(tmem + col, a1_k, shifted(w1_k, 64u * qq * 16u), id_pre, false); };
     auto gh = [&](int qq, uint32_t col) { tc::issue_mma_fast<kC / 16>(tmem + col, gz_k, shifted(w2_mn, 8u * qq * (kC * 16u)), id_gh, false); };
     for (; tile < n_tiles; tile += gridDim.x) {
+      if (tile + (int)gridDim.x >= n_tiles) griddep_launch_dependents();
       tc::mbar_wait(&s.lnready, p_ln);
       p_ln ^= 1u;
       tc::tc_fence_after();
@@ -410,9 +412,10 @@
 
 constexpr int kFiberThreads = 512;
 constexpr int kFibTile = 4;
+constexpr int kFibStages = 4;
 struct FiberBwdSmem {
-  float G[2][kFibTile * kRow];
-  float X[2][kFibTile * kRow];
+  float G[kFibStages][kFibTile * kRow];
+  float X[kFibStages][kFibTile * kRow];
 };
 
 __device__ __forceinline__ void fiber_stage(FiberBwdSmem& s, int buf, const GrlConvDesc& d, int tile) {
@@ -431,6 +434,7 @@
   extern __shared__ __align__(128) unsigned char smem_raw[];
   FiberBwdSmem& s = *reinterpret_cast<FiberBwdSmem*>(smem_raw);
   const int tid = threadIdx.x, c = tid & 63, op = tid >> 6;
+  griddep_wait();
   unsigned long long fk2[kO], gfk2[kO];
 #pragma unroll
   for (int p = 0; p < kO; ++p) {
@@ -441,13 +445,18 @@
   float gbias = 0.f;
   const int n_tiles = (d.n_dst + kFibTile - 1) / kFibTile;
   int tile = blockIdx.x, buf = 0;
-  if (tile < n_tiles) fiber_stage(s, 0, d, tile);
-  cp_async_commit();
-  for (; tile < n_tiles; tile += gridDim.x, buf ^= 1) {
-    const int nt = tile + gridDim.x;
-    if (nt < n_tiles) fiber_stage(s, buf ^ 1, d, nt);
+#pragma unroll
+  for (int st = 0; st < kFibStages - 1; ++st) {
+    const int t = tile + st * (int)gridDim.x;
+    if (t < n_tiles) fiber_stage(s, st, d, t);
     cp_async_commit();
-    cp_async_wait<1>();
+  }
+  for (; tile < n_tiles; tile += gridDim.x, buf = (buf + 1) % kFibStages) {
+    if (tile + (int)gridDim.x >= n_tiles) griddep_launch_dependents();
+    const int nt = tile + (kFibStages - 1) * (int)gridDim.x;
+    if (nt < n_tiles) fiber_stage(s, (buf + kFibStages - 1) % kFibStages, d, nt);
+    cp_async_commit();
+    cp_async_wait<kFibStages - 1>();
     __syncthreads();
 #pragma unroll
     for (int j = 0; j < kFibTile; ++j) {
@@ -497,12 +506,12 @@
     GRL_REQUIRE(d->x2, GRL_EINVAL, "grl_fbconv_node_bwd_tc: x2 (saved by grl_fbconv_node_fwd_tc) is required");
     const int smem = (int)sizeof(grl::NodeBwd3Smem);
     if (grl::ensure_dynamic_smem((const void*)grl::fbconv_node_bwd_tc3_kernel, smem) != GRL_OK) return GRL_ECUDA;
-    grl::fbconv_node_bwd_tc3_kernel<<<d->n_partials_node, grl::kNB3Threads, smem, (cudaStream_t)stream>>>(*d);
-  }
-  int rc = grl::check_launch("grl_fbconv_node_bwd_tc (mlp)");
-  if (rc != GRL_OK) return rc;
+    const int rc = grl::launch_pdl("grl_fbconv_node_bwd_tc (mlp)", grl::fbconv_node_bwd_tc3_kernel, d->n_partials_node,
+                                   grl::kNB3Threads, smem, (cudaStream_t)stream, *d);
+    if (rc != GRL_OK) return rc;
+  }
   const int smem2 = (int)sizeof(grl::FiberBwdSmem);
   if (grl::ensure_dynamic_smem((const void*)grl::fbconv_fiber_bwd_kernel, smem2) != GRL_OK) return GRL_ECUDA;
-  grl::fbconv_fiber_bwd_kernel<<<d->n_partials_node, grl::kFiberThreads, smem2, (cudaStream_t)stream>>>(*d);
-  return grl::check_launch("grl_fbconv_node_bwd_tc (fibre)");
+  return grl::launch_pdl("grl_fbconv_node_bwd_tc (fibre)", grl::fbconv_fiber_bwd_kernel, d->n_partials_node, grl::kFiberThreads,
+                         smem2, (cudaStream_t)stream, *d);
 }
diff --git a/geometry_rl_b200/csrc/grl_conv_node_tc.cu b/geometry_rl_b200/csrc/grl_conv_node_tc.cu
--- a/geometry_rl_b200/csrc/grl_conv_node_tc.cu
+++ b/geometry_rl_b200/csrc/grl_conv_node_tc.cu
@@ -80,6 +80,7 @@
     *reinterpret_cast<uint4*>(s.W1h + ((size_t)9 * kH + n) * 8) = make_uint4(0u, 0u, 0u, 0u);
   }
   if (tid < kC) { s.b2[tid] = d.b2[tid]; s.bias[tid] = d.bias[tid]; s.lng[tid] = d.ln_g[tid]; s.lnb[tid] = d.ln_b[tid]; }
+  griddep_wait();
   const int fc = gt & 63, pq = gt >> 6;
   unsigned long long fk2[kO][2];
 #pragma unroll
@@ -107,6 +108,7 @@
   uint32_t parity = 0;
 
   for (; tile < n_tiles; tile += tile_stride) {
+    if (tile + tile_stride >= n_tiles) griddep_launch_dependents();
     const int n0 = tile * kTE;
     if (gt == 0) {
       tc::prefetch_l2(d.x_dst + (size_t)n0 * kRow, (uint32_t)min(kTE, d.n_dst - n0) * kRow * 4u);
@@ -274,7 +276,7 @@
   if (grl::make_row_tensor_map(&tm_xd, d->x_dst, d->n_dst, grl::kTM) != GRL_OK) return GRL_ECUDA;
   int grid = grl::sm_count();
   if (2 * grid > n_tiles) grid = (n_tiles + 1) / 2;
-  if (d->accumulate_out) grl::fbconv_node_fwd_tc2_kernel<true><<<grid, grl::kNF2Threads, smem2, (cudaStream_t)stream>>>(*d, tm_xd);
-  else grl::fbconv_node_fwd_tc2_kernel<false><<<grid, grl::kNF2Threads, smem2, (cudaStream_t)stream>>>(*d, tm_xd);
-  return grl::check_launch("grl_fbconv_node_fwd_tc");
-}
+  return grl::launch_pdl("grl_fbconv_node_fwd_tc",
+                         d->accumulate_out ? grl::fbconv_node_fwd_tc2_kernel<true> : grl::fbconv_node_fwd_tc2_kernel<false>, grid,
+                         grl::kNF2Threads, smem2, (cudaStream_t)stream, *d, tm_xd);
+}
diff --git a/geometry_rl_b200/csrc/grl_critic.cu b/geometry_rl_b200/csrc/grl_critic.cu
--- a/geometry_rl_b200/csrc/grl_critic.cu
+++ b/geometry_rl_b200/csrc/grl_critic.cu
@@ -68,6 +68,7 @@
 }
 
 __global__ void __launch_bounds__(kCrThreads) critic_stats_kernel(const GrlCriticDesc d) {
+  griddep_wait();
   extern __shared__ __align__(16) unsigned char smem_raw[];
   CriticSmem& s = *reinterpret_cast<CriticSmem*>(smem_raw);
   const int p = threadIdx.x >> 4, cg = threadIdx.x & 15;
@@ -100,6 +101,7 @@
 }
 
 __global__ void critic_combine_kernel(const double* __restrict__ partials, int n_slots, int n, double* __restrict__ out) {
+  griddep_wait();
   const int i = threadIdx.x;
   if (i >= n) return;
   double s = 0.0;
@@ -124,6 +126,7 @@
 }
 
 __global__ void __launch_bounds__(kCrThreads) critic_fwd_kernel(const GrlCriticDesc d) {
+  griddep_wait();
   extern __shared__ __align__(16) unsigned char smem_raw[];
   CriticSmem& s = *reinterpret_cast<CriticSmem*>(smem_raw);
   const int p = threadIdx.x >> 4, cg = threadIdx.x & 15;
@@ -162,6 +165,7 @@
 }
 
 __global__ void __launch_bounds__(kCrThreads) critic_bwd_stats_kernel(const GrlCriticDesc d) {
+  griddep_wait();
   extern __shared__ __align__(16) unsigned char smem_raw[];
   CriticSmem& s = *reinterpret_cast<CriticSmem*>(smem_raw);
   const int p = threadIdx.x >> 4, cg = threadIdx.x & 15;
@@ -229,6 +233,7 @@
 }
 
 __global__ void __launch_bounds__(kCrThreads) critic_bwd_kernel(const GrlCriticDesc d) {
+  griddep_wait();
   extern __shared__ __align__(16) unsigned char smem_raw[];
   CriticSmem& s = *reinterpret_cast<CriticSmem*>(smem_raw);
   const int p = threadIdx.x >> 4, cg = threadIdx.x & 15;
@@ -315,9 +320,10 @@
   const int smem = (int)sizeof(grl::CriticSmem);
   if (grl::ensure_dynamic_smem((const void*)grl::critic_stats_kernel, smem) != GRL_OK) return GRL_ECUDA;
   const int grid = critic_grid(d);
-  grl::critic_stats_kernel<<<grid, grl::kCrThreads, smem, (cudaStream_t)stream>>>(*d);
-  grl::critic_combine_kernel<<<1, 32, 0, (cudaStream_t)stream>>>(d->stat_partials, grid, 2, d->stats);
-  return grl::check_launch("grl_critic_inner_stats");
+  const int rc2 = grl::launch_pdl("grl_critic_inner_stats", grl::critic_stats_kernel, grid, grl::kCrThreads, smem, (cudaStream_t)stream, *d);
+  if (rc2 != GRL_OK) return rc2;
+  return grl::launch_pdl("grl_critic_inner_stats (combine)", grl::critic_combine_kernel, 1, 32, 0, (cudaStream_t)stream,
+                         d->stat_partials, grid, 2, d->stats);
 }
 
 int grl_critic_inner_fwd(const GrlCriticDesc* d, grl_stream_t stream) {
@@ -326,8 +332,7 @@
   GRL_REQUIRE(d->ysum && d->count > 0, GRL_EINVAL, "grl_critic_inner_fwd: ysum / count");
   const int smem = (int)sizeof(grl::CriticSmem);
   if (grl::ensure_dynamic_smem((const void*)grl::critic_fwd_kernel, smem) != GRL_OK) return GRL_ECUDA;
-  grl::critic_fwd_kernel<<<critic_grid(d), grl::kCrThreads, smem, (cudaStream_t)stream>>>(*d);
-  return grl::check_launch("grl_critic_inner_fwd");
+  return grl::launch_pdl("grl_critic_inner_fwd", grl::critic_fwd_kernel, critic_grid(d), grl::kCrThreads, smem, (cudaStream_t)stream, *d);
 }
 
 int grl_critic_inner_bwd_stats(const GrlCriticDesc* d, grl_stream_t stream) {
@@ -337,9 +342,11 @@
   const int smem = (int)sizeof(grl::CriticSmem);
   if (grl::ensure_dynamic_smem((const void*)grl::critic_bwd_stats_kernel, smem) != GRL_OK) return GRL_ECUDA;
   const int grid = critic_grid(d);
-  grl::critic_bwd_stats_kernel<<<grid, grl::kCrThreads, smem, (cudaStream_t)stream>>>(*d);
-  grl::critic_combine_kernel<<<1, 32, 0, (cudaStream_t)stream>>>(d->stat_partials, grid, 2, d->bstats);
-  return grl::check_launch("grl_critic_inner_bwd_stats");
+  const int rc2 = grl::launch_pdl("grl_critic_inner_bwd_stats", grl::critic_bwd_stats_kernel, grid, grl::kCrThreads, smem,
+                                  (cudaStream_t)stream, *d);
+  if (rc2 != GRL_OK) return rc2;
+  return grl::launch_pdl("grl_critic_inner_bwd_stats (combine)", grl::critic_combine_kernel, 1, 32, 0, (cudaStream_t)stream,
+                         d->stat_partials, grid, 2, d->bstats);
 }
 
 int grl_critic_inner_bwd(const GrlCriticDesc* d, grl_stream_t stream) {
@@ -348,8 +355,7 @@
   GRL_REQUIRE(d->grad_ysum && d->bstats && d->grad_partials && d->count > 0, GRL_EINVAL, "grl_critic_inner_bwd: null pointer");
   const int smem = (int)sizeof(grl::CriticSmem);
   if (grl::ensure_dynamic_smem((const void*)grl::critic_bwd_kernel, smem) != GRL_OK) return GRL_ECUDA;
-  grl::critic_bwd_kernel<<<critic_grid(d), grl::kCrThreads, smem, (cudaStream_t)stream>>>(*d);
-  return grl::check_launch("grl_critic_inner_bwd");
-}
-
-}
+  return grl::launch_pdl("grl_critic_inner_bwd", grl::critic_bwd_kernel, critic_grid(d), grl::kCrThreads, smem, (cudaStream_t)stream, *d);
+}
+
+}
diff --git a/geometry_rl_b200/csrc/grl_edge_fused.cu b/geometry_rl_b200/csrc/grl_edge_fused.cu
--- a/geometry_rl_b200/csrc/grl_edge_fused.cu
+++ b/geometry_rl_b200/csrc/grl_edge_fused.cu
@@ -118,6 +118,7 @@
   stage_w1_b1_b2(s.W1b, d.w1, d.b1, d.b2);
   tc::stage_weight_f16(s.W2h, d.w2, kC, kC, kC);
   tc::stage_weight_f16(s.Wkh, d.wk, kC, kC, kC);
+  griddep_wait();
   const long long W = 8ll * __ldg(d.rowptr + d.n_key) + d.n_key;
   const int n_lo = blockIdx.x == 0 ? 0 : fused_lower_bound(d.rowptr, d.n_key, W * blockIdx.x / gridDim.x);
   const int n_hi = blockIdx.x + 1 == gridDim.x ? d.n_key : fused_lower_bound(d.rowptr, d.n_key, W * (blockIdx.x + 1) / gridDim.x);
@@ -155,6 +156,7 @@
   int cur = n_lo;
   float4 sum = make_float4(0.f, 0.f, 0.f, 0.f);
   for (int t = 0; t < n_tiles; ++t) {
+    if (t + 1 == n_tiles) griddep_launch_dependents();
     const int slot = t & 3;
     const uint32_t par = (uint32_t)t & 1u;
     const int cnt = min(kTE, p1 - (p0 + t * kTE));
@@ -356,6 +358,7 @@
   tc::stage_weight_bf16(s.Wkb, d.wk, kC, kC, kC);
   if (tid < kC) s.b2[tid] = __ldg(d.b2 + tid);
   if (tid < 4 * kC) (&s.acc_gb2[0][0])[tid] = 0.f;
+  griddep_wait();
   const long long W = 8ll * __ldg(d.rowptr + d.n_key) + d.n_key;
   const int n_lo = blockIdx.x == 0 ? 0 : fused_lower_bound(d.rowptr, d.n_key, W * blockIdx.x / gridDim.x);
   const int n_hi = blockIdx.x + 1 == gridDim.x ? d.n_key : fused_lower_bound(d.rowptr, d.n_key, W * (blockIdx.x + 1) / gridDim.x);
@@ -384,6 +387,7 @@
     };
     load_idx(0, es, ed);
     for (int t = 0; t < n_tiles; ++t) {
+      if (t + 1 == n_tiles) griddep_launch_dependents();
       const int slot = t & 3;
       const int cnt = min(kTE, p1 - (p0 + t * kTE));
       load_idx(t + 1, es_n, ed_n);
@@ -744,8 +748,8 @@
   if (grl::ensure_dynamic_smem((const void*)grl::edge_fused_fwd_kernel, smem) != GRL_OK) return GRL_ECUDA;
   int grid = 3 * grl::sm_count();
   if (grid > d->n_key) grid = d->n_key;
-  grl::edge_fused_fwd_kernel<<<grid, grl::kThreads, smem, (cudaStream_t)stream>>>(*d, tm_xs);
-  return grl::check_launch("grl_fbconv_edge_fused_fwd");
+  return grl::launch_pdl("grl_fbconv_edge_fused_fwd", grl::edge_fused_fwd_kernel, grid, grl::kThreads, smem, (cudaStream_t)stream, *d,
+                         tm_xs);
 }
 
 int grl_fbconv_edge_fused_bwd(const GrlFusedEdgeDesc* d, grl_stream_t stream) {
@@ -761,8 +765,8 @@
   if (grl::make_row_tensor_map(&tm_in, d->grad_x_src_init ? d->grad_x_src_init : d->x_src, d->n_key) != GRL_OK) return GRL_ECUDA;
   const int smem = (int)sizeof(grl::FusedBwdWs3Smem) + 1024;
   if (grl::ensure_dynamic_smem((const void*)grl::edge_fused_bwd_ws3_kernel, smem) != GRL_OK) return GRL_ECUDA;
-  grl::edge_fused_bwd_ws3_kernel<<<d->n_partials, grl::kWs3Threads, smem, (cudaStream_t)stream>>>(*d, tm_gx, tm_xs, tm_in);
-  return grl::check_launch("grl_fbconv_edge_fused_bwd");
-}
-
-}
+  return grl::launch_pdl("grl_fbconv_edge_fused_bwd", grl::edge_fused_bwd_ws3_kernel, d->n_partials, grl::kWs3Threads, smem,
+                         (cudaStream_t)stream, *d, tm_gx, tm_xs, tm_in);
+}
+
+}
diff --git a/geometry_rl_b200/csrc/grl_embed.cu b/geometry_rl_b200/csrc/grl_embed.cu
--- a/geometry_rl_b200/csrc/grl_embed.cu
+++ b/geometry_rl_b200/csrc/grl_embed.cu
@@ -47,6 +47,7 @@
   __shared__ float sc[kEmbTile * kMaxF], vc[kEmbTile * kMaxF * 3];
   const int tid = threadIdx.x, o = tid >> 4, cg = tid & 15;
   const int F = d.n_scalars + d.n_vectors;
+  griddep_wait();
   unsigned long long w01[4 * FQ], w23[4 * FQ];
 #pragma unroll
   for (int f = 0; f < 4 * FQ; ++f) {
@@ -93,6 +94,7 @@
   __shared__ float sc[kEmbTile * kMaxF], vc[kEmbTile * kMaxF * 3];
   const int tid = threadIdx.x, o = tid >> 4, cg = tid & 15;
   const int F = d.n_scalars + d.n_vectors;
+  griddep_wait();
   unsigned long long g01[4 * FQ], g23[4 * FQ];
 #pragma unroll
   for (int f = 0; f < 4 * FQ; ++f) g01[f] = g23[f] = pack2(0.f, 0.f);
@@ -166,12 +168,11 @@
   const int fq = (d->n_scalars + d->n_vectors + 3) / 4;
   int grid = (fq <= 2 ? 8 : 6) * grl::sm_count();
   if (grid > n_tiles) grid = n_tiles;
-  cudaStream_t st = (cudaStream_t)stream;
-  if (fq == 1) grl::embed_fwd_kernel<1><<<grid, grl::kThreads, 0, st>>>(*d);
-  else if (fq == 2) grl::embed_fwd_kernel<2><<<grid, grl::kThreads, 0, st>>>(*d);
-  else if (fq == 3) grl::embed_fwd_kernel<3><<<grid, grl::kThreads, 0, st>>>(*d);
-  else grl::embed_fwd_kernel<4><<<grid, grl::kThreads, 0, st>>>(*d);
-  return grl::check_launch("grl_embed_fwd");
+  void (*kernel)(const GrlEmbedDesc) = fq == 1   ? grl::embed_fwd_kernel<1>
+                                       : fq == 2 ? grl::embed_fwd_kernel<2>
+                                       : fq == 3 ? grl::embed_fwd_kernel<3>
+                                                 : grl::embed_fwd_kernel<4>;
+  return grl::launch_pdl("grl_embed_fwd", kernel, grid, grl::kThreads, 0, (cudaStream_t)stream, *d);
 }
 
 int grl_embed_bwd(const GrlEmbedDesc* d, grl_stream_t stream) {
@@ -179,12 +180,11 @@
   if (rc != GRL_OK) return rc;
   GRL_REQUIRE(d->grad_x && d->grad_weight_partials && d->n_partials > 0, GRL_EINVAL, "grl_embed_bwd: null pointer");
   const int fq = (d->n_scalars + d->n_vectors + 3) / 4;
-  cudaStream_t st = (cudaStream_t)stream;
-  if (fq == 1) grl::embed_bwd_kernel<1><<<d->n_partials, grl::kThreads, 0, st>>>(*d);
-  else if (fq == 2) grl::embed_bwd_kernel<2><<<d->n_partials, grl::kThreads, 0, st>>>(*d);
-  else if (fq == 3) grl::embed_bwd_kernel<3><<<d->n_partials, grl::kThreads, 0, st>>>(*d);
-  else grl::embed_bwd_kernel<4><<<d->n_partials, grl::kThreads, 0, st>>>(*d);
-  return grl::check_launch("grl_embed_bwd");
+  void (*kernel)(const GrlEmbedDesc) = fq == 1   ? grl::embed_bwd_kernel<1>
+                                       : fq == 2 ? grl::embed_bwd_kernel<2>
+                                       : fq == 3 ? grl::embed_bwd_kernel<3>
+                                                 : grl::embed_bwd_kernel<4>;
+  return grl::launch_pdl("grl_embed_bwd", kernel, d->n_partials, grl::kThreads, 0, (cudaStream_t)stream, *d);
 }
 
 }
diff --git a/geometry_rl_b200/csrc/grl_readout.cu b/geometry_rl_b200/csrc/grl_readout.cu
--- a/geometry_rl_b200/csrc/grl_readout.cu
+++ b/geometry_rl_b200/csrc/grl_readout.cu
@@ -34,6 +34,7 @@
 }
 
 __global__ void __launch_bounds__(256) readout_fwd_kernel(const GrlReadoutDesc d) {
+  griddep_wait();
   __shared__ float s_ori[kO][3];
   __shared__ float s_obar[3];
   if (threadIdx.x < kO * 3) s_ori[threadIdx.x / 3][threadIdx.x % 3] = d.ori[threadIdx.x];
@@ -78,6 +79,7 @@
 }
 
 __global__ void __launch_bounds__(256) readout_bwd_kernel(const GrlReadoutDesc d) {
+  griddep_wait();
   __shared__ float s_ori[kO][3];
   __shared__ float s_obar[3];
   __shared__ float s_gw[8][kMaxJ * kC + kMaxJ];
@@ -186,15 +188,13 @@
   int grid = (d->n_nodes + 7) / 8;
   const int cap = 4 * grl::sm_count();
   if (grid > cap) grid = cap;
-  grl::readout_fwd_kernel<<<grid, 256, 0, (cudaStream_t)stream>>>(*d);
-  return grl::check_launch("grl_readout_fwd");
+  return grl::launch_pdl("grl_readout_fwd", grl::readout_fwd_kernel, grid, 256, 0, (cudaStream_t)stream, *d);
 }
 
 int grl_readout_bwd(const GrlReadoutDesc* d, grl_stream_t stream) {
   const int rc = check_readout(d, "grl_readout_bwd", true);
   if (rc != GRL_OK) return rc;
-  grl::readout_bwd_kernel<<<d->n_partials, 256, 0, (cudaStream_t)stream>>>(*d);
-  return grl::check_launch("grl_readout_bwd");
-}
-
-}
+  return grl::launch_pdl("grl_readout_bwd", grl::readout_bwd_kernel, d->n_partials, 256, 0, (cudaStream_t)stream, *d);
+}
+
+}
diff --git a/geometry_rl_b200/csrc/grl_trpl.cu b/geometry_rl_b200/csrc/grl_trpl.cu
--- a/geometry_rl_b200/csrc/grl_trpl.cu
+++ b/geometry_rl_b200/csrc/grl_trpl.cu
@@ -31,6 +31,7 @@
 }
 
 __global__ void __launch_bounds__(128) trpl_fwd_kernel(const GrlProjDesc d) {
+  griddep_wait();
   const int b = blockIdx.x * blockDim.x + threadIdx.x;
   if (b >= d.batch) return;
   const int k = d.k;
@@ -117,6 +118,7 @@
 }
 
 __global__ void __launch_bounds__(128) trpl_bwd_kernel(const GrlProjDesc d) {
+  griddep_wait();
   const int b = blockIdx.x * blockDim.x + threadIdx.x;
   if (b >= d.batch) return;
   const int k = d.k;
@@ -220,6 +222,7 @@
 constexpr double kLog2Pi = 1.8378770664093454835606594728112;
 
 __global__ void __launch_bounds__(128) trpl_loss_terms_kernel(const GrlLossDesc d) {
+  griddep_wait();
   const int b = blockIdx.x * blockDim.x + threadIdx.x;
   if (b >= d.batch) return;
   const int k = d.k;
@@ -292,6 +295,7 @@
 }
 
 __global__ void __launch_bounds__(kLossThreads) trpl_loss_stats_kernel(const GrlLossDesc d) {
+  griddep_wait();
   __shared__ double sh[32];
   const int B = d.batch, tid = threadIdx.x;
   const double* T = d.terms;
@@ -309,6 +313,7 @@
 }
 
 __global__ void __launch_bounds__(kLossThreads) trpl_loss_sums_kernel(const GrlLossDesc d) {
+  griddep_wait();
   __shared__ double sh[32];
   const int B = d.batch, tid = threadIdx.x;
   const double* T = d.terms;
@@ -348,6 +353,7 @@
 }
 
 __global__ void trpl_loss_finalize_kernel(const GrlLossDesc d) {
+  griddep_wait();
   if (threadIdx.x != 0 || blockIdx.x != 0) return;
   const double n = d.stats[2];
   const double* G = d.sums;
@@ -369,6 +375,7 @@
 }
 
 __global__ void __launch_bounds__(128) trpl_loss_bwd_kernel(const GrlLossDesc d) {
+  griddep_wait();
   const int b = blockIdx.x * blockDim.x + threadIdx.x;
   if (b >= d.batch) return;
   const int k = d.k;
@@ -420,15 +427,13 @@
 int grl_trpl_fwd(const GrlProjDesc* d, grl_stream_t stream) {
   const int rc = check_proj(d, "grl_trpl_fwd", false);
   if (rc != GRL_OK) return rc;
-  grl::trpl_fwd_kernel<<<(d->batch + 127) / 128, 128, 0, (cudaStream_t)stream>>>(*d);
-  return grl::check_launch("grl_trpl_fwd");
+  return grl::launch_pdl("grl_trpl_fwd", grl::trpl_fwd_kernel, (d->batch + 127) / 128, 128, 0, (cudaStream_t)stream, *d);
 }
 
 int grl_trpl_bwd(const GrlProjDesc* d, grl_stream_t stream) {
   const int rc = check_proj(d, "grl_trpl_bwd", true);
   if (rc != GRL_OK) return rc;
-  grl::trpl_bwd_kernel<<<(d->batch + 127) / 128, 128, 0, (cudaStream_t)stream>>>(*d);
-  return grl::check_launch("grl_trpl_bwd");
+  return grl::launch_pdl("grl_trpl_bwd", grl::trpl_bwd_kernel, (d->batch + 127) / 128, 128, 0, (cudaStream_t)stream, *d);
 }
 
 static int check_loss(const GrlLossDesc* d, const char* who, bool bwd) {
@@ -449,13 +454,16 @@
   if (rc != GRL_OK) return rc;
   GRL_REQUIRE(d->stage >= 0 && d->stage <= 3, GRL_EINVAL, "grl_trpl_loss_fwd: stage=%d", d->stage);
   cudaStream_t st = (cudaStream_t)stream;
+  int rc2 = GRL_OK;
   if (d->stage == 0 || d->stage == 1) {
-    grl::trpl_loss_terms_kernel<<<(d->batch + 127) / 128, 128, 0, st>>>(*d);
-    grl::trpl_loss_stats_kernel<<<1, grl::kLossThreads, 0, st>>>(*d);
-  }
-  if (d->stage == 0 || d->stage == 2) grl::trpl_loss_sums_kernel<<<1, grl::kLossThreads, 0, st>>>(*d);
-  if (d->stage == 0 || d->stage == 3) grl::trpl_loss_finalize_kernel<<<1, 32, 0, st>>>(*d);
-  return grl::check_launch("grl_trpl_loss_fwd");
+    rc2 = grl::launch_pdl("grl_trpl_loss_fwd (terms)", grl::trpl_loss_terms_kernel, (d->batch + 127) / 128, 128, 0, st, *d);
+    if (rc2 == GRL_OK) rc2 = grl::launch_pdl("grl_trpl_loss_fwd (stats)", grl::trpl_loss_stats_kernel, 1, grl::kLossThreads, 0, st, *d);
+  }
+  if (rc2 == GRL_OK && (d->stage == 0 || d->stage == 2))
+    rc2 = grl::launch_pdl("grl_trpl_loss_fwd (sums)", grl::trpl_loss_sums_kernel, 1, grl::kLossThreads, 0, st, *d);
+  if (rc2 == GRL_OK && (d->stage == 0 || d->stage == 3))
+    rc2 = grl::launch_pdl("grl_trpl_loss_fwd (finalize)", grl::trpl_loss_finalize_kernel, 1, 32, 0, st, *d);
+  return rc2;
 }
 
 int grl_dp_combine(const double* gathered, int world, int n, int n_sum, double* out, grl_stream_t stream) {
@@ -468,8 +476,7 @@
 int grl_trpl_loss_bwd(const GrlLossDesc* d, grl_stream_t stream) {
   const int rc = check_loss(d, "grl_trpl_loss_bwd", true);
   if (rc != GRL_OK) return rc;
-  grl::trpl_loss_bwd_kernel<<<(d->batch + 127) / 128, 128, 0, (cudaStream_t)stream>>>(*d);
-  return grl::check_launch("grl_trpl_loss_bwd");
-}
-
-}
+  return grl::launch_pdl("grl_trpl_loss_bwd", grl::trpl_loss_bwd_kernel, (d->batch + 127) / 128, 128, 0, (cudaStream_t)stream, *d);
+}
+
+}
diff --git a/geometry_rl_b200/csrc/grl_util.cu b/geometry_rl_b200/csrc/grl_util.cu
--- a/geometry_rl_b200/csrc/grl_util.cu
+++ b/geometry_rl_b200/csrc/grl_util.cu
@@ -1,5 +1,7 @@
 #include <cstdarg>
 #include <cstdio>
+#include <cstdlib>
+#include <cstring>
 #include <atomic>
 #include <mutex>
 #include <utility>
@@ -65,6 +67,13 @@
   return GRL_OK;
 }
 
+static std::atomic<int> g_pdl{[] {
+  const char* v = std::getenv("GRL_PDL");
+  return (v && std::strcmp(v, "0") == 0) ? 0 : 1;
+}()};
+
+bool pdl_enabled() { return g_pdl.load(std::memory_order_relaxed) != 0; }
+
 static std::atomic<int> g_reserved_sms{0};
 
 int sm_count() {
@@ -103,6 +112,7 @@
 __global__ void __launch_bounds__(256) reduce_partials_kernel(const float* __restrict__ partials, int n_partials, int64_t n,
                                                               float* __restrict__ out, int accumulate) {
   __shared__ float seg_sum[8][32];
+  griddep_wait();
   const int lane = threadIdx.x & 31, seg = threadIdx.x >> 5;
   const int per = (n_partials + 7) / 8;
   const int p0 = seg * per, p1 = min(n_partials, p0 + per);
@@ -133,12 +143,22 @@
 
 __global__ void __launch_bounds__(256) absmax_kernel(const float4* __restrict__ x, int64_t n4, const float* __restrict__ tail,
                                                      int n_tail, unsigned int* __restrict__ out_bits) {
+  griddep_wait();
   unsigned int m = 0u;
-  for (int64_t i = blockIdx.x * (int64_t)blockDim.x + threadIdx.x; i < n4; i += (int64_t)gridDim.x * blockDim.x) {
-    const float4 v = __ldg(x + i);
+  auto fold = [&m](float4 v) {
     const float a = fmaxf(fmaxf(fabsf(v.x), fabsf(v.y)), fmaxf(fabsf(v.z), fabsf(v.w)));
     m = max(m, __float_as_uint(a));
-  }
+  };
+  const int64_t stride = (int64_t)gridDim.x * blockDim.x;
+  int64_t i = blockIdx.x * (int64_t)blockDim.x + threadIdx.x;
+  for (; i + 3 * stride < n4; i += 4 * stride) {
+    const float4 v0 = __ldg(x + i), v1 = __ldg(x + i + stride), v2 = __ldg(x + i + 2 * stride), v3 = __ldg(x + i + 3 * stride);
+    fold(v0);
+    fold(v1);
+    fold(v2);
+    fold(v3);
+  }
+  for (; i < n4; i += stride) fold(__ldg(x + i));
   if (blockIdx.x == 0 && (int)threadIdx.x < n_tail) m = max(m, __float_as_uint(fabsf(tail[threadIdx.x])));
 #pragma unroll
   for (int o = 16; o > 0; o >>= 1) m = max(m, __shfl_xor_sync(0xffffffffu, m, o));
@@ -164,14 +184,20 @@
   grl::g_reserved_sms.store(n, std::memory_order_relaxed);
   return GRL_OK;
 }
+int grl_set_pdl(int on) {
+  GRL_REQUIRE(on == 0 || on == 1, GRL_EINVAL, "grl_set_pdl: on=%d is not 0 or 1", on);
+  grl::g_pdl.store(on, std::memory_order_relaxed);
+  return GRL_OK;
+}
+int grl_pdl_enabled(void) { return grl::pdl_enabled() ? 1 : 0; }
 
 int grl_reduce_partials(const float* partials, int n_partials, int64_t n_floats, float* out, int accumulate,
                         grl_stream_t stream) {
   GRL_REQUIRE(partials && out && n_partials > 0 && n_floats > 0, GRL_EINVAL, "grl_reduce_partials: bad arguments");
   int64_t blocks = (n_floats + 31) / 32;
   if (blocks > 16 * grl::sm_count()) blocks = 16 * grl::sm_count();
-  grl::reduce_partials_kernel<<<(int)blocks, 256, 0, (cudaStream_t)stream>>>(partials, n_partials, n_floats, out, accumulate);
-  return grl::check_launch("grl_reduce_partials");
+  return grl::launch_pdl("grl_reduce_partials", grl::reduce_partials_kernel, (int)blocks, 256, 0, (cudaStream_t)stream, partials,
+                         n_partials, n_floats, out, accumulate);
 }
 
 int grl_absmax(const float* x, int64_t n, uint32_t* out_bits, grl_stream_t stream) {
@@ -183,8 +209,8 @@
   int64_t blocks = (n4 + 255) / 256;
   if (blocks > 8 * grl::sm_count()) blocks = 8 * grl::sm_count();
   if (blocks < 1) blocks = 1;
-  grl::absmax_kernel<<<(int)blocks, 256, 0, s>>>(reinterpret_cast<const float4*>(x), n4, x + 4 * n4, (int)(n - 4 * n4), out_bits);
-  return grl::check_launch("grl_absmax");
-}
-
-}
+  return grl::launch_pdl("grl_absmax", grl::absmax_kernel, (int)blocks, 256, 0, s, reinterpret_cast<const float4*>(x), n4,
+                         x + 4 * n4, (int)(n - 4 * n4), out_bits);
+}
+
+}
diff --git a/include/grl_b200.h b/include/grl_b200.h
--- a/include/grl_b200.h
+++ b/include/grl_b200.h
@@ -25,6 +25,8 @@
 const char* grl_last_error(void);
 int grl_sm_count(void);
 int grl_reserve_sms(int n);
+int grl_set_pdl(int on);
+int grl_pdl_enabled(void);
 
 
 int grl_knn_edge_ptr(const int32_t* num_valid, int B, int P, int k, int64_t* edge_ptr, grl_stream_t stream);
```
